# TongtongSong/OpenEAT

Measured on AMD Instinct MI355X. Metric: audio-frames/sec/GPU (train) + RTF (attention-rescoring decode), 12L Conformer, higher is better.
Workload: dtype f32 (storage, accumulate, softmax, norms, losses, optimizer all fp32; every matrix product is the fp32 product to within one fp32 rounding, computed as six exact bf16 x bf16 MFMA products of three-piece operand splits h+m+l = x, dropped terms < 2^-24 |a||b| - tests hold it to the exact-fp32 mode's t; 1 GPU; configs[1]: 12L Conformer d=256 (12+3+3, h=4, ff=1024, K=15, V=3246), B=32/GPU x 10 s 16 kHz wav (T=998 frames), L=30, CTC+attention joint loss, fbank+fwd+bwd+clip+Adam, dropout 0.1; global_batch=32, parallelism=dp1, hip_graph=True

## Files before the change

include/openeat_hip.h:

```cpp
#ifndef OPENEAT_HIP_H
#define OPENEAT_HIP_H

#include <stddef.h>
#include <stdint.h>

#ifdef __cplusplus
extern "C" {
#endif

const char* oe_last_error(void);
int oe_abi_version(void);

int oe_capture_unjoined_streams(void* origin, void* const* sides, int n_sides, int* unjoined_index);

int oe_stamp(long long* buf, int slot, void* stream);

enum { OE_GATHER_NONE = 0, OE_GATHER_A = 1, OE_GATHER_B = 2 };

typedef struct oe_gemm_args {
    const float* a; long lda; int a_kmajor;
    const float* b; long ldb; int b_kmajor;
    float* c; long ldc;
    int m, n, k;
    int split_k;
    float alpha; const float* alpha_dev;
    const float* bias;
    int act;
    float* preact_out; const float* actgrad_in; long ld_aux;
    float drop_p; unsigned long long seed; const unsigned long long* seed_dev;
    const unsigned char* rowmask;
    const float* residual; long ldr; int res_row_mod; float beta;
    int accumulate; int atomic_out;
    int conv_gather; int conv_t1, conv_f1, conv_t2, conv_f2, conv_c;
    float* a_colsum;
    int precision;
    int conv_k, conv_s;
    int conv_kh;
    int out_scatter; int sc_t1, sc_f1, sc_t2, sc_f2, sc_s;
    const void* a_planes; long a_plane_stride;
    const void* b_planes; long b_plane_stride;
    void* c_planes; long c_plane_stride; long ldcp;
    int conv_korder;
    int actgrad_bf16;
    int planes_k_padded;
} oe_gemm_args;

int oe_gemm_f32(const oe_gemm_args* args, void* stream);

int oe_split_planes(const float* x, long ld, long rows, long cols, void* planes, long ldp, long plane_stride, void* stream);
long oe_gemm_pl_launches(void);
long oe_gemm_hyb_launches(void);
int oe_gemm_pl_config(int min_blocks, int tile, int bk, int waves);
int oe_gemm_pl_hybrid(int on);

typedef struct oe_ln_prologue {
    const float* dy; const float* x; const float* stats; const float* gamma; const float* add;
    float* dx; float* g; float* ws;
    float g_alpha, g_p; unsigned long long g_seed; const unsigned char* g_rowmask; const unsigned char* ln_rowmask;
    const float* beta; const float* gamma2; const float* stats2; float* ws2;
} oe_ln_prologue;

typedef struct oe_lnf_prologue {
    const float* x; const float* gamma; const float* beta; float eps;
    float* y; float* stats; const unsigned char* rowmask;
    const float* gamma2; const float* beta2; float eps2; float* u; float* stats2;
} oe_lnf_prologue;

typedef struct oe_ln_epilogue {
    const float* x; const float* stats; const float* gamma; const float* beta; int act;
    float* dx; float* ws;
} oe_ln_epilogue;

typedef struct oe_ffn_args {
    const float* x; long ldx;
    const void* w1p; const float* b1;
    const void* w2p; const float* b2;
    int rows, d, ff, act, precision;
    float drop_in; unsigned long long seed_in;
    float drop_out; unsigned long long seed_out;
    const unsigned long long* seed_dev;
    float* pre_out; float* act_out;
    const float* residual; long ldr; float beta;
    float* y; long ldy;
    oe_ln_prologue ln;
    oe_lnf_prologue lnf;
} oe_ffn_args;
size_t oe_ffn_packed_bytes(int d, int ff, int precision);
int oe_ffn_supported(int d, int ff, int precision, int act);
int oe_ffn_pack_weights(const float* w1, const float* w2, int d, int ff, int precision, void* w1p, void* w2p, void* stream);
int oe_ffn_fwd(const oe_ffn_args* args, void* stream);
int oe_ffn_pack_weights_bwd(const float* w1, const float* w2, int d, int ff, int precision, void* w2t_packed, void* w1t_packed, void* stream);
int oe_ffn_bwd(const oe_ffn_args* a, void* stream);
int oe_ffn_pack_weights_table(const void* table, int n, int max_d, int max_ff, int precision, void* stream);
int oe_ffn6_config(int mode);

typedef struct oe_rowgemm_args {
    const float* x; long ldx;
    const void* wp; const float* bias;
    int rows, k, n;
    float drop_p; unsigned long long seed; const unsigned long long* seed_dev;
    const unsigned char* rowmask;
    const float* residual; long ldr; float beta;
    float* y; long ldy;
    int act; float* preact_out; const float* actgrad_in; long ld_aux;
    oe_ln_prologue ln;
    oe_lnf_prologue lnf;
    oe_ln_epilogue lne;
} oe_rowgemm_args;
int oe_rowgemm6_supported(int k, int n);
int oe_rowgemm6_form(int rows, int k, int n);
int oe_rowgemm6(const oe_rowgemm_args* args, void* stream);
int oe_rowgemm6_pack_table(const void* table, int n, long max_pieces, void* stream);

typedef struct oe_tn_problem {
    const float* a; const float* b; float* c; float* a_colsum; const float* alpha_dev;
    long lda, ldb, ldc;
    int m, n, k;
    float alpha;
    int k_chunk, gx, gy, nz, block_start, reserved;
} oe_tn_problem;
int oe_gemm_tn_grouped_plan(oe_tn_problem* problems_host, int n, int target_blocks);
int oe_gemm_tn_grouped(const oe_tn_problem* problems_dev, int n, int total_blocks, int precision, void* stream);

int oe_colsum_f32(const float* x, long ldx, int m, int n, float alpha, const float* alpha_dev,
                  float* out, int accumulate, void* stream);

int oe_layernorm_fwd_pl(const float* x, const float* gamma, const float* beta, float eps, int rows, int d,
                        const unsigned char* rowmask, int act, float* y, float* stats, void* y_planes, long plane_stride, void* stream);
int oe_layernorm_fwd(const float* x, const float* gamma, const float* beta, float eps, int rows, int d,
                     const unsigned char* rowmask, int act, float* y, float* stats, void* stream);
size_t oe_layernorm_bwd_workspace_floats(int rows, int d);
int oe_layernorm_bwd(const float* dy, const float* x, const float* gamma, const float* beta, int act,
                     const float* stats, int rows, int d, const unsigned char* rowmask, const float* add,
                     float* dx, float* dgamma, float* dbeta, float* workspace, void* stream);
int oe_layernorm_pair_fwd(const float* x, const float* gamma1, const float* beta1, float eps1, const float* gamma2, const float* beta2,
                          float eps2, int rows, int d, float* y1, float* stats1, float* y2, float* stats2, void* stream);
int oe_layernorm_pair_bwd_dx_drop(const float* dy2, const float* x, const float* gamma1, const float* beta1, const float* stats1,
                                  const float* gamma2, const float* stats2, int rows, int d, const float* add, float* dx, float* gout,
                                  float g_alpha, float g_p, unsigned long long g_seed, const unsigned long long* g_seed_dev,
                                  const unsigned char* g_rowmask, float* workspace1, float* workspace2, void* stream);
int oe_layernorm_bwd_dx(const float* dy, const float* x, const float* gamma, const float* beta, int act, const float* stats,
                        int rows, int d, const unsigned char* rowmask, const float* add, float* dx, float* workspace,
                        void* stream);
int oe_layernorm_param_reduce(const float* workspace, int rows, int d, float* dgamma, float* dbeta, void* stream);
int oe_layernorm_param_reduce_table(const long long* table, int n, int max_rows, int max_d, void* stream);
int oe_layernorm_bwd_dx_drop(const float* dy, const float* x, const float* gamma, const float* beta, int act,
                             const float* stats, int rows, int d, const unsigned char* rowmask, const float* add, float* dx,
                             float* gout, float g_alpha, float g_p, unsigned long long g_seed,
                             const unsigned long long* g_seed_dev, const unsigned char* g_rowmask, float* workspace,
                             void* stream);
int oe_layernorm_bwd_dx_drop_pl(const float* dy, const float* x, const float* gamma, const float* beta, int act,
                                const float* stats, int rows, int d, const unsigned char* rowmask, const float* add, float* dx,
                                float* gout, float g_alpha, float g_p, unsigned long long g_seed,
                                const unsigned long long* g_seed_dev, const unsigned char* g_rowmask, float* workspace,
                                void* out_planes, long plane_stride, void* stream);

size_t oe_ctc_workspace_floats(int B, int T, int Lmax);
int oe_ctc_config(int pipe_mode, int chunks);
int oe_ctc_loss_fused_stats(const float* logits, long ldv, int B, int T, int V, const int* hlens, const int* targets,
                            int Lmax, const int* tlens, float grad_scale, const float* utt_weight, float* nll, float* loss_sum,
                            float* dlogits, float* workspace, const float* row_stats, int stats_groups, void* stream);
int oe_ctc_loss_fused(const float* logits, long ldv, int B, int T, int V, const int* hlens, const int* targets,
                      int Lmax, const int* tlens, float grad_scale, const float* utt_weight, float* nll, float* loss_sum,
                      float* dlogits, float* workspace, void* stream);

int oe_ctc_greedy(const float* logits, long ldv, int B, int T, int V, const int* hlens, int eos,
                  int* frame_best, int* out_tokens, int* out_lens, void* stream);

size_t oe_ctc_align_workspace_bytes(int B, int T, int Lmax);
int oe_ctc_align(const float* logits, long ldv, int B, int T, int V, const int* hlens, const int* targets, int Lmax,
                 const int* tlens, int* frames, int* tok_start, int* tok_end, float* tok_logp, float* score, void* workspace,
                 void* stream);

typedef struct oe_attn_args {
    const float* q; long q_bstride, q_rstride;
    const float* k; long k_bstride, k_rstride;
    const float* v; long v_bstride, v_rstride;
    float* out; long o_bstride, o_rstride;
    float* lse;
    const unsigned char* mask; long mask_bstride, mask_rstride;
    const float* keybias;
    int B, H, T1, T2, D;
    float scale;
    float drop_p; unsigned long long seed; const unsigned long long* seed_dev;
    const float* d_out;
    float* dq; float* dk; float* dv;
    float* dkeybias;
    float* delta;
    int precision;
    int causal;
} oe_attn_args;

int oe_attention_fwd(const oe_attn_args* args, void* stream);
int oe_attention_bwd(const oe_attn_args* args, void* stream);

int oe_relpos_prepare(const float* k, long k_bstride, long k_rstride, const float* p, long p_rstride,
                      const float* u, const float* v, int B, int T, int H, int D, float scale, float* kp,
                      float* keybias, void* stream);
int oe_relpos_backward(const float* dkp, const float* dkeybias, const float* k, long k_bstride, long k_rstride,
                       const float* p, long p_rstride, const float* u, const float* v, int B, int T, int H, int D,
                       float scale, float* dk, float* dp, long dp_rstride, float* du, float* dv, void* stream);

int oe_glu_fwd(const float* a, long rows, int d, float* y, void* stream);
int oe_glu_bwd(const float* a, const float* dy, long rows, int d, float* da, void* stream);

// ... 101 lines not shown
```

openeat_amd/csrc/ffn.hip:

```cpp
#include <stdlib.h>
#include "gemm_common.h"
#include "../../include/openeat_hip.h"

typedef __bf16 bf16x8 __attribute__((ext_vector_type(8)));

#define FFN_THREADS 256
#define FFN_ROWS 32

__device__ __forceinline__ int ffn_acc_row(int r, int lk) { return (r & 3) + 8 * (r >> 2) + 4 * lk; }

template <bool TRANSPOSED>
__device__ __forceinline__ void ffn_pack_piece(const float* __restrict__ w1, const float* __restrict__ w2, int d, int ff, int planes,
                                               __bf16* __restrict__ w1p, __bf16* __restrict__ w2p, long piece, int lane) {
    const int KS = d / 16, DT = d / 32, FT = ff / 32;
    const long n1 = (long)FT * KS, n2 = (long)FT * DT * 2;
    float x[8];
    __bf16* dst;
    if (piece < n1) {
        const int ft = (int)(piece / KS), ks = (int)(piece % KS);
        const int row = 32 * ft + (lane & 31), col = 16 * ks + 8 * (lane >> 5);
        if (!TRANSPOSED) {
            const float* src = w1 + (long)row * d + col;
            const float4 a = *reinterpret_cast<const float4*>(src), b = *reinterpret_cast<const float4*>(src + 4);
            x[0] = a.x; x[1] = a.y; x[2] = a.z; x[3] = a.w; x[4] = b.x; x[5] = b.y; x[6] = b.z; x[7] = b.w;
// ... 254 lines not shown
        const int pc = (c4 + 4 * row) & (D - 1);
        float4 v = *reinterpret_cast<const float4*>(&part[row * PART_PITCH + pc]);
#pragma unroll
        for (int w = 1; w < 4; ++w) {
            const float4 u = *reinterpret_cast<const float4*>(&part[w * (FFN_ROWS * PART_PITCH) + row * PART_PITCH + pc]);
            v.x += u.x; v.y += u.y; v.z += u.z; v.w += u.w;
        }
        if (p.b2) { v.x += p.b2[c4]; v.y += p.b2[c4 + 1]; v.z += p.b2[c4 + 2]; v.w += p.b2[c4 + 3]; }
        if (p.p_out > 0.f) {
            const uint2 h = drop_hash4(seed_out, ((unsigned long long)gr * D + c4) >> 2);
            v.x *= drop_field(h.x, 0, dp_out); v.y *= drop_field(h.x, 1, dp_out);
            v.z *= drop_field(h.y, 0, dp_out); v.w *= drop_field(h.y, 1, dp_out);
        }
        float4 res = make_float4(0.f, 0.f, 0.f, 0.f);
        if (p.residual) res = *reinterpret_cast<const float4*>(p.residual + gr * p.ldr + c4);
        v = make_float4(res.x + p.beta * v.x, res.y + p.beta * v.y, res.z + p.beta * v.z, res.w + p.beta * v.w);
        *reinterpret_cast<float4*>(p.y + gr * p.ldy + c4) = v;
    }
}

int oe_ffn6_supported(int d, int ff);
int oe_ffn6_run(const oe_ffn_args* a, bool bwd, void* stream);
static int ffn_planes(int precision) { return precision == 6 ? 3 : precision == 3 ? 2 : 1; }

extern "C" size_t oe_ffn_packed_bytes(int d, int ff, int precision) {
    return (size_t)d * ff * 2 * ffn_planes(precision);
}

extern "C" int oe_ffn_supported(int d, int ff, int precision, int act) {
    if (!(act == OE_ACT_NONE || act == OE_ACT_RELU || act == OE_ACT_SWISH)) return 0;
    if (precision == 6) return oe_ffn6_supported(d, ff);
    return (d == 128 || d == 256) && ff > 0 && ff % 128 == 0 && ff <= 8192 && (precision == 1 || precision == 3);
}

static int ffn_pack(const float* w1, const float* w2, int d, int ff, int precision, void* w1p, void* w2p, bool transposed, void* stream) {
    OE_REQUIRE(w1 && w2 && w1p && w2p, "oe_ffn_pack_weights: null pointer");
    OE_REQUIRE(oe_ffn_supported(d, ff, precision, 0), "oe_ffn_pack_weights: unsupported shape d=%d ff=%d precision=%d", d, ff, precision);
    OE_REQUIRE(((((uintptr_t)w1) | ((uintptr_t)w2) | ((uintptr_t)w1p) | ((uintptr_t)w2p)) & 15) == 0, "oe_ffn_pack_weights: 16-byte alignment required");
    const long pieces = (long)(ff / 32) * (d / 16) + (long)(ff / 32) * (d / 32) * 2;
    if (transposed)
        hipLaunchKernelGGL(ffn_pack_kernel<true>, dim3(oe_cdiv(pieces, 4)), dim3(256), 0, (hipStream_t)stream, w1, w2, d, ff,
                           ffn_planes(precision), (__bf16*)w1p, (__bf16*)w2p);
    else
        hipLaunchKernelGGL(ffn_pack_kernel<false>, dim3(oe_cdiv(pieces, 4)), dim3(256), 0, (hipStream_t)stream, w1, w2, d, ff,
                           ffn_planes(precision), (__bf16*)w1p, (__bf16*)w2p);
    OE_LAUNCH_CHECK("oe_ffn_pack_weights");
    return 0;
}
extern "C" int oe_ffn_pack_weights_table(const void* table, int n, int max_d, int max_ff, int precision, void* stream) {
    OE_REQUIRE(table && n > 0, "oe_ffn_pack_weights_table: empty table");
    OE_REQUIRE(max_d >= 32 && max_d % 32 == 0 && max_ff >= 32 && max_ff % 32 == 0 && (precision == 1 || precision == 3 || precision == 6),
               "oe_ffn_pack_weights_table: bad launch geometry d=%d ff=%d precision=%d", max_d, max_ff, precision);
    const long pieces = (long)(max_ff / 32) * (max_d / 16) + (long)(max_ff / 32) * (max_d / 32) * 2;
    hipLaunchKernelGGL(ffn_pack_table_kernel, dim3(oe_cdiv(pieces, 4), n, 2), dim3(256), 0, (hipStream_t)stream, (const long long*)table);
    OE_LAUNCH_CHECK("oe_ffn_pack_weights_table");
    return 0;
}
extern "C" int oe_ffn_pack_weights(const float* w1, const float* w2, int d, int ff, int precision, void* w1p, void* w2p, void* stream) {
    return ffn_pack(w1, w2, d, ff, precision, w1p, w2p, false, stream);
}
extern "C" int oe_ffn_pack_weights_bwd(const float* w1, const float* w2, int d, int ff, int precision, void* w2tp, void* w1tp, void* stream) {
    return ffn_pack(w1, w2, d, ff, precision, w2tp, w1tp, true, stream);
}

template <int D, int TERMS>
static int ffn_launch(const FfnParams& p, int nout, hipStream_t st) {
    const dim3 grid(oe_cdiv(p.rows, FFN_ROWS)), block(FFN_THREADS);
    const size_t dyn = (size_t)p.ff * sizeof(float);
    if (nout == 2) hipLaunchKernelGGL((ffn_fwd_kernel<D, TERMS, 2>), grid, block, dyn, st, p);
    else if (nout == 1) hipLaunchKernelGGL((ffn_fwd_kernel<D, TERMS, 1>), grid, block, dyn, st, p);
    else hipLaunchKernelGGL((ffn_fwd_kernel<D, TERMS, 0>), grid, block, dyn, st, p);
    OE_LAUNCH_CHECK("oe_ffn_fwd");
    return 0;
}

extern "C" int oe_ffn_fwd(const oe_ffn_args* a, void* stream) {
    OE_REQUIRE(a && a->x && a->w1p && a->w2p && a->y, "oe_ffn_fwd: null pointer");
    OE_REQUIRE(oe_ffn_supported(a->d, a->ff, a->precision, a->act), "oe_ffn_fwd: unsupported d=%d ff=%d precision=%d act=%d", a->d, a->ff,
               a->precision, a->act);
    OE_REQUIRE(a->rows > 0 && a->ldx % 4 == 0 && a->ldy % 4 == 0 && (!a->residual || a->ldr % 4 == 0), "oe_ffn_fwd: bad rows / strides");
    OE_REQUIRE(((((uintptr_t)a->x) | ((uintptr_t)a->y) | ((uintptr_t)a->residual) | ((uintptr_t)a->pre_out) | ((uintptr_t)a->act_out) |
                 ((uintptr_t)a->w1p) | ((uintptr_t)a->w2p)) & 15) == 0, "oe_ffn_fwd: 16-byte alignment required");
    OE_REQUIRE(a->drop_in >= 0.f && a->drop_in < 1.f && a->drop_out >= 0.f && a->drop_out < 1.f, "oe_ffn_fwd: dropout rate out of range");
    OE_REQUIRE(!(a->act_out && !a->pre_out), "oe_ffn_fwd: act_out needs pre_out (the store count is a compile-time constant)");
    if (a->precision == 6) return oe_ffn6_run(a, false, stream);
    FfnParams p{};
    p.x = a->x; p.ldx = a->ldx; p.w1p = (const __bf16*)a->w1p; p.b1 = a->b1; p.w2p = (const __bf16*)a->w2p; p.b2 = a->b2;
    p.pre = a->pre_out; p.act_out = a->act_out; p.residual = a->residual; p.ldr = a->ldr; p.beta = a->beta; p.y = a->y; p.ldy = a->ldy;
    p.rows = a->rows; p.ff = a->ff; p.act = a->act; p.p_in = a->drop_in; p.seed_in = a->seed_in; p.p_out = a->drop_out; p.seed_out = a->seed_out;
    p.seed_dev = a->seed_dev;
    const int nout = a->act_out ? 2 : a->pre_out ? 1 : 0;
    hipStream_t st = (hipStream_t)stream;
    if (a->d == 256) return a->precision == 3 ? ffn_launch<256, 3>(p, nout, st) : ffn_launch<256, 1>(p, nout, st);
    return a->precision == 3 ? ffn_launch<128, 3>(p, nout, st) : ffn_launch<128, 1>(p, nout, st);
}

extern "C" int oe_ffn_bwd(const oe_ffn_args* a, void* stream) {
    OE_REQUIRE(a && (a->x || a->ln.dy) && a->w1p && a->w2p && a->y && a->pre_out && a->act_out, "oe_ffn_bwd: null pointer");
    OE_REQUIRE(!a->ln.dy || a->precision == 6, "oe_ffn_bwd: the LayerNorm-backward prologue exists in precision 6 only");
    OE_REQUIRE(oe_ffn_supported(a->d, a->ff, a->precision, a->act), "oe_ffn_bwd: unsupported d=%d ff=%d precision=%d act=%d", a->d, a->ff,
               a->precision, a->act);
    OE_REQUIRE(!a->b1 && !a->b2 && !a->residual && a->drop_out == 0.f && a->beta == 1.f, "oe_ffn_bwd: bias / residual / output dropout do not apply");
    OE_REQUIRE(a->rows > 0 && a->ldx % 4 == 0 && a->ldy % 4 == 0, "oe_ffn_bwd: bad rows / strides");
    OE_REQUIRE(((((uintptr_t)a->x) | ((uintptr_t)a->y) | ((uintptr_t)a->pre_out) | ((uintptr_t)a->act_out) | ((uintptr_t)a->w1p) |
                 ((uintptr_t)a->w2p)) & 15) == 0, "oe_ffn_bwd: 16-byte alignment required");
    OE_REQUIRE(a->drop_in >= 0.f && a->drop_in < 1.f, "oe_ffn_bwd: dropout rate out of range");
    if (a->precision == 6) return oe_ffn6_run(a, true, stream);
    FfnParams p{};
    p.x = a->x; p.ldx = a->ldx; p.w1p = (const __bf16*)a->w1p; p.w2p = (const __bf16*)a->w2p;
    p.pre = a->pre_out; p.act_out = a->act_out; p.beta = 1.f; p.y = a->y; p.ldy = a->ldy;
    p.rows = a->rows; p.ff = a->ff; p.act = a->act; p.p_in = a->drop_in; p.seed_in = a->seed_in; p.seed_dev = a->seed_dev;
    const dim3 grid(oe_cdiv(p.rows, FFN_ROWS)), block(FFN_THREADS);
    const size_t dyn = (size_t)p.ff * sizeof(float);
    hipStream_t st = (hipStream_t)stream;
    if (a->d == 256) {
        if (a->precision == 3) hipLaunchKernelGGL((ffn_fwd_kernel<256, 3, 1, true>), grid, block, dyn, st, p);
        else hipLaunchKernelGGL((ffn_fwd_kernel<256, 1, 1, true>), grid, block, dyn, st, p);
    } else {
        if (a->precision == 3) hipLaunchKernelGGL((ffn_fwd_kernel<128, 3, 1, true>), grid, block, dyn, st, p);
        else hipLaunchKernelGGL((ffn_fwd_kernel<128, 1, 1, true>), grid, block, dyn, st, p);
    }
    OE_LAUNCH_CHECK("oe_ffn_bwd");
    return 0;
}
```

openeat_amd/csrc/ffn6.hip:

```cpp
#include <stdlib.h>
#include "gemm_common.h"
#include "../../include/openeat_hip.h"

#ifndef OE_F6_NSET
#define OE_F6_NSET 4
#endif
#ifndef OE_F6_FR
#define OE_F6_FR 1
#endif

typedef __bf16 bf16x8 __attribute__((ext_vector_type(8)));
typedef __bf16 bf16x4 __attribute__((ext_vector_type(4)));

struct LnPro {
    const float* dy; const float* x; const float* stats; const float* gamma; const float* add;
    float* dx; float* g; float* ws;
    float g_alpha, g_p; unsigned long long g_seed; const unsigned char* g_rowmask; const unsigned char* ln_rowmask;
    const float* beta; const float* gamma2; const float* stats2; float* ws2;
};
static LnPro ln_pro_of(const oe_ln_prologue& a) {
    LnPro q;
    q.dy = a.dy; q.x = a.x; q.stats = a.stats; q.gamma = a.gamma; q.add = a.add; q.dx = a.dx; q.g = a.g; q.ws = a.ws;
    q.g_alpha = a.g_alpha; q.g_p = a.g_p; q.g_seed = a.g_seed; q.g_rowmask = a.g_rowmask; q.ln_rowmask = a.ln_rowmask;
    q.beta = a.beta; q.gamma2 = a.gamma2; q.stats2 = a.stats2; q.ws2 = a.ws2;
    return q;
}
static const char* ln_pro_check(const oe_ln_prologue& a) {
    if (!(a.x && a.stats && a.gamma && a.dx && a.g && a.ws)) return "null pointer";
    if (((((uintptr_t)a.dy) | ((uintptr_t)a.x) | ((uintptr_t)a.gamma) | ((uintptr_t)a.add) | ((uintptr_t)a.dx) | ((uintptr_t)a.g)) & 15) != 0) return "16-byte alignment required";
    if (!(a.g_p >= 0.f && a.g_p < 1.f)) return "dropout rate out of range";
    if (a.gamma2 && !(a.beta && a.stats2 && a.ws2 && !a.ln_rowmask)) return "pair: beta / stats2 / ws2 missing (and no row mask)";
    if (((((uintptr_t)a.beta) | ((uintptr_t)a.gamma2)) & 15) != 0) return "16-byte alignment required";
    return nullptr;
}

struct LnfPro {
    const float* x; const float* gamma; const float* beta; float eps; float* y; float* stats; const unsigned char* rowmask;
    const float* gamma2; const float* beta2; float eps2; float* u; float* stats2;
};
static LnfPro lnf_pro_of(const oe_lnf_prologue& a) {
    LnfPro q;
    q.x = a.x; q.gamma = a.gamma; q.beta = a.beta; q.eps = a.eps; q.y = a.y; q.stats = a.stats; q.rowmask = a.rowmask;
    q.gamma2 = a.gamma2; q.beta2 = a.beta2; q.eps2 = a.eps2; q.u = a.u; q.stats2 = a.stats2;
    return q;
}
static const char* lnf_pro_check(const oe_lnf_prologue& a) {
    if (!(a.gamma && a.beta && a.y && a.stats)) return "null pointer";
    if (((((uintptr_t)a.x) | ((uintptr_t)a.gamma) | ((uintptr_t)a.beta) | ((uintptr_t)a.y)) & 15) != 0) return "16-byte alignment required";
    if (a.gamma2 && !(a.beta2 && a.stats2 && !a.rowmask)) return "pair: beta2 / stats2 missing (and no row mask)";
    if (((((uintptr_t)a.gamma2) | ((uintptr_t)a.beta2) | ((uintptr_t)a.u)) & 15) != 0) return "16-byte alignment required";
    return nullptr;
}

struct Ffn6Params {
    const float* x; long ldx;
    const unsigned char* w1p; const float* b1;
    const unsigned char* w2p; const float* b2;
    float* pre; float* act_out;
    const float* residual; long ldr; float beta;
    float* y; long ldy;
    int rows, ff, act;
    float p_in; unsigned long long seed_in;
    float p_out; unsigned long long seed_out;
    const unsigned long long* seed_dev;
    LnPro ln;
    LnfPro lnf;
};

__device__ __forceinline__ float f6_act_bwd(int act, float x) {
    const float s = sigmoidf_(x);
    const float sw = s * (1.f + x * (1.f - s));
    return act == OE_ACT_SWISH ? sw : (act == OE_ACT_RELU ? (x > 0.f ? 1.f : 0.f) : 1.f);
}
struct F6 { bf16x8 p[3]; };

#ifdef OE_GEMM_STAMPS
static __device__ unsigned long long* f6_stamp_buf = nullptr;
extern "C" int oe_ffn6_set_stamps(void* buf) {
    return (int)hipMemcpyToSymbol(HIP_SYMBOL(f6_stamp_buf), &buf, sizeof(buf));
}
#define F6_STAMP(slot)                                                                                                   \
    do {                                                                                                                 \
        __builtin_amdgcn_sched_barrier(0);                                                                               \
        unsigned long long t_;                                                                                           \
        asm volatile("s_memtime %0\n\ts_waitcnt lgkmcnt(0)" : "=s"(t_) :: "memory");                                    \
        __builtin_amdgcn_sched_barrier(0);                                                                               \
        if (f6_stamp_buf && (blockIdx.x == 0 || blockIdx.x == gridDim.x - 1) && (threadIdx.x & 63) == 0 && (slot) < 128)     \
            f6_stamp_buf[(blockIdx.x == 0 ? 0 : 1024) + (threadIdx.x >> 6) * 128 + (slot)] = t_;                        \
    } while (0)
#else
#define F6_STAMP(slot) do { } while (0)
#endif
__device__ __forceinline__ int f6_acc_row(int r, int lk) { return (r & 3) + 8 * (r >> 2) + 4 * lk; }
__device__ __forceinline__ void f6_lds_barrier() { asm volatile("s_waitcnt lgkmcnt(0)\n\ts_barrier" ::: "memory"); }
__device__ __forceinline__ void f6_wave_sync() {
    asm volatile("s_waitcnt lgkmcnt(0)" ::: "memory");
    __builtin_amdgcn_wave_barrier();
}

template <bool BWD, int NOUT>
__device__ __forceinline__ void f6_epilogue1(const Ffn6Params& p, const f32x16& hacc, float4 q0, float4 q1, float4 q2, float4 q3, long mrow, int ft,
                                             int lane, float* patch, unsigned long long seed_in, const DropParams& dp_in, float (&hv)[16]) {
    const int lq = lane & 31, lk = lane >> 5;
    auto store_tile = [&](float* out) {
        f6_wave_sync();
#pragma unroll
        for (int r = 0; r < 16; ++r) patch[lq * 36 + f6_acc_row(r, lk)] = hv[r];
        f6_wave_sync();
#pragma unroll
        for (int ps = 0; ps < 4; ++ps) {
            const int row = ps * 8 + (lane >> 3), c4 = (lane & 7) * 4;
            if (mrow + row < p.rows)
                *reinterpret_cast<float4*>(out + (mrow + row) * p.ff + ft * 32 + c4) = *reinterpret_cast<const float4*>(&patch[row * 36 + c4]);
        }
    };
    if (!BWD) {
        hv[0] = hacc[0] + q0.x; hv[1] = hacc[1] + q0.y; hv[2] = hacc[2] + q0.z; hv[3] = hacc[3] + q0.w;
        hv[4] = hacc[4] + q1.x; hv[5] = hacc[5] + q1.y; hv[6] = hacc[6] + q1.z; hv[7] = hacc[7] + q1.w;
        hv[8] = hacc[8] + q2.x; hv[9] = hacc[9] + q2.y; hv[10] = hacc[10] + q2.z; hv[11] = hacc[11] + q2.w;
        hv[12] = hacc[12] + q3.x; hv[13] = hacc[13] + q3.y; hv[14] = hacc[14] + q3.z; hv[15] = hacc[15] + q3.w;
        if (NOUT >= 1 && p.pre) store_tile(p.pre);
        if (p.act == OE_ACT_SWISH) {
#pragma unroll
            for (int r = 0; r < 16; ++r) hv[r] *= sigmoidf_(hv[r]);
        } else if (p.act == OE_ACT_RELU) {
#pragma unroll
            for (int r = 0; r < 16; ++r) hv[r] = fmaxf(hv[r], 0.f);
        }
    } else {
        f6_wave_sync();
        float* pr = &patch[(lane >> 3) * 36 + (lane & 7) * 4];
        *reinterpret_cast<float4*>(pr) = q0;
        *reinterpret_cast<float4*>(pr + 8 * 36) = q1;
        *reinterpret_cast<float4*>(pr + 16 * 36) = q2;
        *reinterpret_cast<float4*>(pr + 24 * 36) = q3;
        f6_wave_sync();
#pragma unroll
        for (int r = 0; r < 16; ++r) hv[r] = hacc[r] * f6_act_bwd(p.act, patch[lq * 36 + f6_acc_row(r, lk)]);
    }
    if (p.p_in > 0.f) {
        const unsigned long long e0 = (unsigned long long)(mrow + lq) * p.ff + ft * 32 + 4 * lk;
#pragma unroll
        for (int g4 = 0; g4 < 4; ++g4) {
            const uint2 h = drop_hash4(seed_in, (e0 + 8 * g4) >> 2);
            hv[4 * g4] *= drop_field(h.x, 0, dp_in); hv[4 * g4 + 1] *= drop_field(h.x, 1, dp_in);
            hv[4 * g4 + 2] *= drop_field(h.y, 0, dp_in); hv[4 * g4 + 3] *= drop_field(h.y, 1, dp_in);
        }
    }
    if ((BWD || NOUT == 2) && p.act_out) store_tile(p.act_out);
}
__device__ __forceinline__ void f6_write_planes(const float (&hv)[16], unsigned char* hdst, int s_stride, int lane) {
#pragma unroll
    for (int s = 0; s < 2; ++s) {
        float v[8];
#pragma unroll
        for (int e = 0; e < 8; ++e) v[e] = hv[8 * s + e];
        oe_bf16x8 pl[3];
        oe_split8<3>(v, pl);
#pragma unroll
        for (int pn = 0; pn < 3; ++pn) *reinterpret_cast<oe_bf16x8*>(hdst + s * s_stride + pn * 1024 + lane * 16) = pl[pn];
    }
}

template <int D, bool PAIR>
__device__ __forceinline__ void ln_fwd_rows_to_planes(const LnfPro& q, int rows, long m0, int wv, int lane, unsigned char* xs) {
    static_assert(D == 256, "one float4 per lane and row");
    constexpr int BM = 32, XP = D + 8;
    const float4 g = reinterpret_cast<const float4*>(q.gamma)[lane], bb = reinterpret_cast<const float4*>(q.beta)[lane];
    float4 g2 = g, bb2 = bb;
    if (PAIR) { g2 = reinterpret_cast<const float4*>(q.gamma2)[lane]; bb2 = reinterpret_cast<const float4*>(q.beta2)[lane]; }
    float4 v[4];
#pragma unroll
    for (int k = 0; k < 4; ++k) v[k] = reinterpret_cast<const float4*>(q.x + min(m0 + wv + 8 * k, (long)rows - 1) * D)[lane];
#pragma unroll
    for (int k = 0; k < 4; ++k) {
        const int row = wv + 8 * k;
        const long grow = m0 + row;
        const bool valid = grow < rows;
        const float mean = wave_sum(v[k].x + v[k].y + v[k].z + v[k].w) / D;
        const float a = v[k].x - mean, b = v[k].y - mean, c = v[k].z - mean, e = v[k].w - mean;
        const float rstd = rsqrtf(wave_sum(a * a + b * b + c * c + e * e) / D + q.eps);
        float4 o = make_float4(0.f, 0.f, 0.f, 0.f);
        if (!(valid && q.rowmask && !q.rowmask[grow]))
            o = make_float4((v[k].x - mean) * rstd * g.x + bb.x, (v[k].y - mean) * rstd * g.y + bb.y,
                            (v[k].z - mean) * rstd * g.z + bb.z, (v[k].w - mean) * rstd * g.w + bb.w);
        if (valid && lane == 0) { q.stats[grow * 2] = mean; q.stats[grow * 2 + 1] = rstd; }
        if (PAIR) {
            if (valid && q.u) reinterpret_cast<float4*>(q.u + grow * D)[lane] = o;
            const float mean2 = wave_sum(o.x + o.y + o.z + o.w) / D;
            const float a2 = o.x - mean2, b2 = o.y - mean2, c2 = o.z - mean2, e2 = o.w - mean2;
            const float rstd2 = rsqrtf(wave_sum(a2 * a2 + b2 * b2 + c2 * c2 + e2 * e2) / D + q.eps2);
            if (valid && lane == 0) { q.stats2[grow * 2] = mean2; q.stats2[grow * 2 + 1] = rstd2; }
            o = make_float4((o.x - mean2) * rstd2 * g2.x + bb2.x, (o.y - mean2) * rstd2 * g2.y + bb2.y,
                            (o.z - mean2) * rstd2 * g2.z + bb2.z, (o.w - mean2) * rstd2 * g2.w + bb2.w);
        }
        if (valid) reinterpret_cast<float4*>(q.y + grow * D)[lane] = o;
        const float xq[4] = {o.x, o.y, o.z, o.w};
        oe_bf16x4v pl[3];
        oe_split4<3>(xq, pl);
#pragma unroll
        for (int n = 0; n < 3; ++n) *reinterpret_cast<oe_bf16x4v*>(xs + ((size_t)(n * BM + row) * XP + 4 * lane) * 2) = pl[n];
    }
}

template <int D, bool PAIR>
__device__ __forceinline__ void ln_bwd_rows_to_planes(const LnPro& q, const unsigned long long* seed_dev, int rows, long m0, int wv, int lane,
                                                      unsigned char* xs, float* red) {
    static_assert(D == 256, "one float4 per lane and row");
    constexpr int BM = 32, XP = D + 8;
    constexpr int NV = D / 256;
    const float4* g4 = reinterpret_cast<const float4*>(q.gamma);
    float4 gam[NV], dg[2][NV], db[2][NV];
    float4 bet[PAIR ? NV : 1], gam2[PAIR ? NV : 1], dg2[2][PAIR ? NV : 1], db2[2][PAIR ? NV : 1];
#pragma unroll
    for (int j = 0; j < NV; ++j) {
        gam[j] = g4[lane + 64 * j];
        dg[0][j] = dg[1][j] = db[0][j] = db[1][j] = make_float4(0.f, 0.f, 0.f, 0.f);
        if (PAIR) {
            bet[j] = reinterpret_cast<const float4*>(q.beta)[lane + 64 * j];
            gam2[j] = reinterpret_cast<const float4*>(q.gamma2)[lane + 64 * j];
            dg2[0][j] = dg2[1][j] = db2[0][j] = db2[1][j] = make_float4(0.f, 0.f, 0.f, 0.f);
        }
    }
    const DropParams g_dpar = drop_params(q.g_p);
    const unsigned long long g_seed_eff = q.g_seed + (seed_dev ? *seed_dev * 0x9E3779B97F4A7C15ull : 0ull);
    float4 dyv[4][NV], xv[4][NV], av[4][NV];
    float mean[4], rstd[4];
#pragma unroll
    for (int k = 0; k < 4; ++k) {
        const long rc = min(m0 + wv + 8 * k, (long)rows - 1);
        mean[k] = q.stats[rc * 2];
        rstd[k] = q.stats[rc * 2 + 1];
// ... 60 lines not shown
            dgs.x += t.x * xh[j].x; dgs.y += t.y * xh[j].y; dgs.z += t.z * xh[j].z; dgs.w += t.w * xh[j].w;
            dbs.x += t.x; dbs.y += t.y; dbs.z += t.z; dbs.w += t.w;
        }
        const float c1 = wave_sum(s1) / D, c2 = wave_sum(s2) / D;
#pragma unroll
        for (int j = 0; j < NV; ++j) {
            const int i = lane + 64 * j;
            float4 o = av[k][j];
            if (live) {
                o.x += rstd[k] * (g[j].x - c1 - xh[j].x * c2);
                o.y += rstd[k] * (g[j].y - c1 - xh[j].y * c2);
                o.z += rstd[k] * (g[j].z - c1 - xh[j].z * c2);
                o.w += rstd[k] * (g[j].w - c1 - xh[j].w * c2);
            }
            float4 gq = make_float4(o.x * q.g_alpha, o.y * q.g_alpha, o.z * q.g_alpha, o.w * q.g_alpha);
            const unsigned long long e0 = (unsigned long long)grow * D + 4 * i;
            if (q.g_p > 0.f) {
                const uint4 r = drop_words8(g_seed_eff, e0 >> 3);
                const bool hi = (e0 >> 2) & 1;
                const unsigned wa = hi ? r.z : r.x, wb = hi ? r.w : r.y;
                gq.x *= drop_field(wa, 0, g_dpar); gq.y *= drop_field(wa, 1, g_dpar);
                gq.z *= drop_field(wb, 0, g_dpar); gq.w *= drop_field(wb, 1, g_dpar);
            }
            if (valid && q.g_rowmask && !q.g_rowmask[grow]) gq = make_float4(0.f, 0.f, 0.f, 0.f);
            if (valid) {
                reinterpret_cast<float4*>(q.dx + grow * D)[i] = o;
                reinterpret_cast<float4*>(q.g + grow * D)[i] = gq;
            }
            const float xq[4] = {gq.x, gq.y, gq.z, gq.w};
            oe_bf16x4v pl[3];
            oe_split4<3>(xq, pl);
#pragma unroll
            for (int n = 0; n < 3; ++n) *reinterpret_cast<oe_bf16x4v*>(xs + ((size_t)(n * BM + row) * XP + 4 * i) * 2) = pl[n];
        }
    }
#pragma unroll
    for (int sl = 0; sl < 2; ++sl)
#pragma unroll
        for (int j = 0; j < NV; ++j) {
            reinterpret_cast<float4*>(red + ((wv * 2 + sl) * 2 + 0) * D)[lane + 64 * j] = dg[sl][j];
            reinterpret_cast<float4*>(red + ((wv * 2 + sl) * 2 + 1) * D)[lane + 64 * j] = db[sl][j];
        }
    __syncthreads();
    for (int c = threadIdx.x; c < 4 * D; c += 512) {
        float sum = 0.f;
#pragma unroll
        for (int w = 0; w < 8; ++w) sum += red[w * 4 * D + c];
        const long slot = 2 * (long)blockIdx.x + c / (2 * D);
        if (slot * 16 < rows) q.ws[slot * 2 * D + (c % (2 * D))] = sum;
    }
    if (PAIR) {
        __syncthreads();
#pragma unroll
        for (int sl = 0; sl < 2; ++sl)
#pragma unroll
            for (int j = 0; j < NV; ++j) {
                reinterpret_cast<float4*>(red + ((wv * 2 + sl) * 2 + 0) * D)[lane + 64 * j] = dg2[sl][j];
                reinterpret_cast<float4*>(red + ((wv * 2 + sl) * 2 + 1) * D)[lane + 64 * j] = db2[sl][j];
            }
        __syncthreads();
        for (int c = threadIdx.x; c < 4 * D; c += 512) {
            float sum = 0.f;
#pragma unroll
            for (int w = 0; w < 8; ++w) sum += red[w * 4 * D + c];
            const long slot = 2 * (long)blockIdx.x + c / (2 * D);
            if (slot * 16 < rows) q.ws2[slot * 2 * D + (c % (2 * D))] = sum;
        }
    }
}

template <int D, int RT, bool BWD, int NOUT, int NG, int LNP = 0>
__global__ __launch_bounds__(256 * NG, (NG == 2 || (RT == 1 && D <= 256)) ? 2 : 1) void ffn6_kernel(Ffn6Params p) {
    static_assert(NG == 1 || (NG == 2 && RT == 1), "two wave groups: 32-row blocks");
    static_assert(LNP == 0 || (D == 256 && RT == 1 && NG == 2 && BWD == (LNP == 1)), "LayerNorm prologues: the eight-wave 32-row kernels at d = 256");
    constexpr int BM = 32 * RT;
    constexpr int KS = D / 16, DT = D / 32, DPW = DT / 4;
    constexpr int FR = OE_F6_FR, NSET = OE_F6_NSET;
    constexpr int NS1 = KS / FR, NS2 = DPW * 8 / FR, NSTG = NS1 + NS2;
    static_assert(DT % 4 == 0 && KS % FR == 0 && NSTG % NSET == 0, "stage split");
    constexpr int XP = D + 8;
    constexpr int X_BYTES = 3 * BM * XP * 2;
    constexpr int H_WAVE = 2 * RT * 3 * 1024;
    constexpr int H_BYTES = 4 * H_WAVE;
    static_assert(H_WAVE >= 32 * 36 * 4, "the wave's h region doubles as its 32 x 36 fp32 patch");
    constexpr int PIECE = 3 * 1024;
    constexpr int NT = RT * DPW;
    static_assert(NG == 1 || (NT % 2 == 0 && 8 * (NT / 2) * 4096 <= X_BYTES), "the groups' exchange buffer reuses the x planes");
    __shared__ __attribute__((aligned(1024))) unsigned char lds[X_BYTES + NG * H_BYTES];
    unsigned char* xs = lds;

    const int lane = threadIdx.x & 63;
    const int wv = __builtin_amdgcn_readfirstlane(threadIdx.x >> 6);
    const int grp = NG == 2 ? (wv >> 2) : 0;
    const int wave = wv & 3;
    unsigned char* hs = lds + X_BYTES + grp * H_BYTES;
    const int lq = lane & 31, lk = lane >> 5;
    const long m0 = (long)blockIdx.x * BM;
    const int nchunks = p.ff / 128;
    const int rot = blockIdx.x % nchunks;

    if constexpr (LNP == 2) {
        if (p.lnf.gamma2) ln_fwd_rows_to_planes<D, true>(p.lnf, p.rows, m0, wv, lane, xs);
        else ln_fwd_rows_to_planes<D, false>(p.lnf, p.rows, m0, wv, lane, xs);
    } else if constexpr (LNP == 1) {
        static_assert(LNP != 1 || 8 * 2 * 2 * D * 4 <= NG * H_BYTES, "the prologue's partial sums reuse the h regions");
        if (p.ln.gamma2) ln_bwd_rows_to_planes<D, true>(p.ln, p.seed_dev, p.rows, m0, wv, lane, xs, reinterpret_cast<float*>(lds + X_BYTES));
        else ln_bwd_rows_to_planes<D, false>(p.ln, p.seed_dev, p.rows, m0, wv, lane, xs, reinterpret_cast<float*>(lds + X_BYTES));
    } else {
        constexpr int C4 = D / 4;
        for (int i = threadIdx.x; i < BM * C4; i += 256 * NG) {
            const int row = i / C4, c4 = (i - row * C4) * 4;
            const long gr = min(m0 + row, (long)p.rows - 1);
            const float4 v = *reinterpret_cast<const float4*>(p.x + gr * p.ldx + c4);
            const float xv[4] = {v.x, v.y, v.z, v.w};
            oe_bf16x4v pl[3];
            oe_split4<3>(xv, pl);
#pragma unroll
            for (int n = 0; n < 3; ++n) *reinterpret_cast<oe_bf16x4v*>(xs + ((size_t)(n * BM + row) * XP + c4) * 2) = pl[n];
        }
    }

    const unsigned char* w1l = p.w1p + lane * 16 + (long)wave * KS * PIECE;
    const unsigned char* w2l = p.w2p + lane * 16 + (long)wave * DPW * 2 * PIECE;
    constexpr long W1_CHUNK = 4L * KS * PIECE, W2_CHUNK = 4L * DT * 2 * PIECE;
    auto load_stage = [&](auto w_c, int c, F6 (&f)[FR]) {
        constexpr int w = decltype(w_c)::value;
        const unsigned char* b1p = w1l + c * W1_CHUNK;
        const unsigned char* b2p = w2l + c * W2_CHUNK;
#pragma unroll
        for (int j = 0; j < FR; ++j) {
            const unsigned char* src;
            if constexpr (w < NS1) {
                src = b1p + (long)(w * FR + j) * PIECE;
            } else {
                const int fidx = (w - NS1) * FR + j;
                const int dtl = fidx >> 3, ftl = (fidx >> 1) & 3, s = fidx & 1;
                src = b2p + (long)(((ftl * DT + dtl) * 2) + s) * PIECE;
            }
            f[j].p[0] = *reinterpret_cast<const bf16x8*>(src); f[j].p[1] = *reinterpret_cast<const bf16x8*>(src + 1024);
            f[j].p[2] = *reinterpret_cast<const bf16x8*>(src + 2048);
        }
    };
    auto chunk_at = [&](int ci) {
        int c = min(ci, nchunks - 1) + rot;
        return c >= nchunks ? c - nchunks : c;
    };
    F6 fr[NSET][FR];
    {
        const int c0 = chunk_at(grp);
        static_for<0, NSET - 1>([&](auto k_c) { load_stage(k_c, c0, fr[decltype(k_c)::value]); });
    }

    f32x16 yacc[RT][DPW];
#pragma unroll
    for (int a = 0; a < RT; ++a)
#pragma unroll
        for (int t = 0; t < DPW; ++t)
#pragma unroll
            for (int r = 0; r < 16; ++r) yacc[a][t][r] = 0.f;
    const unsigned long long sd = p.seed_dev ? *p.seed_dev * 0x9E3779B97F4A7C15ull : 0ull;
    const unsigned long long seed_in = p.seed_in + sd, seed_out = p.seed_out + sd;
    const DropParams dp_in = drop_params(p.p_in), dp_out = drop_params(p.p_out);
    unsigned char* hmine = hs + wave * H_WAVE;
    float* patch = reinterpret_cast<float*>(hmine);

    auto x_frag = [&](int rt, int ks, F6& f) {
        const unsigned char* a = xs + ((size_t)(rt * 32 + lq) * XP + 16 * ks + 8 * lk) * 2;
// ... 671 lines not shown
    OE_REQUIRE(!has_act || !(a->preact_out || a->actgrad_in) || (a->ld_aux % 2 == 0 && ((((uintptr_t)a->preact_out) | ((uintptr_t)a->actgrad_in)) & 7) == 0),
               "oe_rowgemm6: pre-activation / act-grad source must be 8-byte aligned with an even row stride");
    OE_REQUIRE(a->rows > 0 && a->ldx % 4 == 0 && a->ldy % 4 == 0 && (!a->residual || a->ldr % 4 == 0), "oe_rowgemm6: bad rows / strides");
    if (a->ln.dy) {
        OE_REQUIRE(form == 1 && a->k == 256, "oe_rowgemm6: the LayerNorm-backward prologue exists in the row-block form at k = 256 only");
        const char* why = ln_pro_check(a->ln);
        OE_REQUIRE(why == nullptr, "oe_rowgemm6: LayerNorm prologue: %s", why);
    }
    if (a->lnf.x) {
        OE_REQUIRE(form == 1 && a->k == 256 && !a->ln.dy && !a->lnf.gamma2, "oe_rowgemm6: the (single) LayerNorm-forward prologue exists in the row-block form at k = 256 only");
        const char* why = lnf_pro_check(a->lnf);
        OE_REQUIRE(why == nullptr, "oe_rowgemm6: LayerNorm-forward prologue: %s", why);
    }
    OE_REQUIRE(((((uintptr_t)a->x) | ((uintptr_t)a->y) | ((uintptr_t)a->residual) | ((uintptr_t)a->wp) | ((uintptr_t)a->bias)) & 15) == 0,
               "oe_rowgemm6: 16-byte alignment required");
    OE_REQUIRE(a->drop_p >= 0.f && a->drop_p < 1.f, "oe_rowgemm6: dropout rate out of range");
    Row6Params p{};
    p.x = a->x; p.ldx = a->ldx; p.wp = (const unsigned char*)a->wp; p.bias = a->bias; p.residual = a->residual; p.ldr = a->ldr; p.beta = a->beta;
    p.rowmask = a->rowmask; p.y = a->y; p.ldy = a->ldy; p.rows = a->rows; p.no = a->n; p.p_out = a->drop_p; p.seed_out = a->seed; p.seed_dev = a->seed_dev;
    p.k = a->k; p.act = a->act; p.preact_out = a->preact_out; p.actgrad_in = a->actgrad_in; p.ld_aux = a->ld_aux;
    p.ln = ln_pro_of(a->ln);
    p.lnf = lnf_pro_of(a->lnf);
    if (a->lne.dx) {
        OE_REQUIRE(form == 1 && a->k == 256 && a->n == 256 && !a->lnf.x, "oe_rowgemm6: the LayerNorm-backward epilogue exists for 256 <- 256 in the row-block form only");
        OE_REQUIRE(a->lne.x && a->lne.stats && a->lne.gamma && a->lne.beta && a->lne.ws, "oe_rowgemm6: LayerNorm epilogue: null pointer");
        OE_REQUIRE(!a->bias && a->drop_p == 0.f && !a->rowmask && !a->residual && a->beta == 1.f, "oe_rowgemm6: LayerNorm epilogue: no other epilogue feature applies");
        OE_REQUIRE(a->lne.act == OE_ACT_NONE || a->lne.act == OE_ACT_RELU || a->lne.act == OE_ACT_SWISH, "oe_rowgemm6: LayerNorm epilogue: activation %d", a->lne.act);
        OE_REQUIRE(((((uintptr_t)a->lne.x) | ((uintptr_t)a->lne.gamma) | ((uintptr_t)a->lne.beta) | ((uintptr_t)a->lne.dx) | ((uintptr_t)a->lne.ws)) & 15) == 0,
                   "oe_rowgemm6: LayerNorm epilogue: 16-byte alignment required");
        p.le_x = a->lne.x; p.le_stats = a->lne.stats; p.le_gamma = a->lne.gamma; p.le_beta = a->lne.beta; p.le_act = a->lne.act;
        p.le_dx = a->lne.dx; p.le_ws = a->lne.ws;
    }
    if (form == 2) {
        const dim3 tgrid(oe_cdiv(a->rows, 32), a->n / 32), tblock(512);
        hipStream_t st = (hipStream_t)stream;
        switch (a->k / 128) {
            case 2: hipLaunchKernelGGL((rowtile6_kernel<2>), tgrid, tblock, 0, st, p); break;
            case 4: hipLaunchKernelGGL((rowtile6_kernel<4>), tgrid, tblock, 0, st, p); break;
            case 6: hipLaunchKernelGGL((rowtile6_kernel<6>), tgrid, tblock, 0, st, p); break;
            default: hipLaunchKernelGGL((rowtile6_kernel<8>), tgrid, tblock, 0, st, p); break;
        }
        OE_LAUNCH_CHECK("oe_rowgemm6 (tile form)");
        return 0;
    }
    const dim3 grid(oe_cdiv(a->rows, 32)), block(512);
    if (a->k > 512) hipLaunchKernelGGL(rowgemm6p_kernel, grid, block, 0, (hipStream_t)stream, p);
    else if (a->lne.dx && a->ln.dy) hipLaunchKernelGGL((rowgemm6_kernel<256, 1, true>), grid, block, 0, (hipStream_t)stream, p);
    else if (a->lne.dx) hipLaunchKernelGGL((rowgemm6_kernel<256, 0, true>), grid, block, 0, (hipStream_t)stream, p);
    else if (a->ln.dy) hipLaunchKernelGGL((rowgemm6_kernel<256, 1>), grid, block, 0, (hipStream_t)stream, p);
    else if (a->lnf.x) hipLaunchKernelGGL((rowgemm6_kernel<256, 2>), grid, block, 0, (hipStream_t)stream, p);
    else if (a->k == 512) hipLaunchKernelGGL((rowgemm6_kernel<512>), grid, block, 0, (hipStream_t)stream, p);
    else hipLaunchKernelGGL((rowgemm6_kernel<256>), grid, block, 0, (hipStream_t)stream, p);
    OE_LAUNCH_CHECK("oe_rowgemm6");
    return 0;
}

template <int D, int RT, int NG>
static int ffn6_launch(const Ffn6Params& p, bool bwd, int nout, hipStream_t st) {
    const dim3 grid(oe_cdiv(p.rows, 32 * RT)), block(256 * NG);
    if constexpr (D == 256 && RT == 1 && NG == 2) {
        if (bwd && p.ln.dy) {
            hipLaunchKernelGGL((ffn6_kernel<D, RT, true, 1, NG, 1>), grid, block, 0, st, p);
            OE_LAUNCH_CHECK("oe_ffn_bwd (precision 6, LayerNorm-backward prologue)");
            return 0;
        }
        if (!bwd && p.lnf.x) {
            if (nout == 2) hipLaunchKernelGGL((ffn6_kernel<D, RT, false, 2, NG, 2>), grid, block, 0, st, p);
            else if (nout == 1) hipLaunchKernelGGL((ffn6_kernel<D, RT, false, 1, NG, 2>), grid, block, 0, st, p);
            else hipLaunchKernelGGL((ffn6_kernel<D, RT, false, 0, NG, 2>), grid, block, 0, st, p);
            OE_LAUNCH_CHECK("oe_ffn_fwd (precision 6, LayerNorm prologue)");
            return 0;
        }
    }
    OE_REQUIRE(!p.ln.dy && !p.lnf.x, "oe_ffn: the LayerNorm prologues exist at d = 256 in the two-group block shape only");
    if (bwd) hipLaunchKernelGGL((ffn6_kernel<D, RT, true, 1, NG>), grid, block, 0, st, p);
    else if (nout == 2) hipLaunchKernelGGL((ffn6_kernel<D, RT, false, 2, NG>), grid, block, 0, st, p);
    else if (nout == 1) hipLaunchKernelGGL((ffn6_kernel<D, RT, false, 1, NG>), grid, block, 0, st, p);
    else hipLaunchKernelGGL((ffn6_kernel<D, RT, false, 0, NG>), grid, block, 0, st, p);
    OE_LAUNCH_CHECK(bwd ? "oe_ffn_bwd (precision 6)" : "oe_ffn_fwd (precision 6)");
    return 0;
}

int oe_ffn6_supported(int d, int ff) { return (d == 128 || d == 256 || d == 512) && ff > 0 && ff % 128 == 0 && ff <= 8192; }

static int ffn6_mode_v = getenv("OE_FFN6_MODE") ? atoi(getenv("OE_FFN6_MODE")) : 0;
static int ffn6_mode() { return ffn6_mode_v; }
extern "C" int oe_ffn6_config(int mode) {
    if (mode >= 0) ffn6_mode_v = mode;
    return ffn6_mode_v;
}

int oe_ffn6_run(const oe_ffn_args* a, bool bwd, void* stream) {
    Ffn6Params p{};
    p.x = a->x; p.ldx = a->ldx; p.w1p = (const unsigned char*)a->w1p; p.b1 = a->b1; p.w2p = (const unsigned char*)a->w2p; p.b2 = a->b2;
    p.pre = a->pre_out; p.act_out = a->act_out; p.residual = a->residual; p.ldr = a->ldr; p.beta = a->beta; p.y = a->y; p.ldy = a->ldy;
    p.rows = a->rows; p.ff = a->ff; p.act = a->act; p.p_in = a->drop_in; p.seed_in = a->seed_in; p.p_out = a->drop_out; p.seed_out = a->seed_out;
    p.seed_dev = a->seed_dev;
    if (a->ln.dy) {
        const char* why = ln_pro_check(a->ln);
        OE_REQUIRE(bwd && why == nullptr, "oe_ffn: LayerNorm prologue: %s", bwd ? why : "backward only");
        p.ln = ln_pro_of(a->ln);
    }
    if (a->lnf.x) {
        const char* why = lnf_pro_check(a->lnf);
        OE_REQUIRE(!bwd && why == nullptr, "oe_ffn: LayerNorm-forward prologue: %s", bwd ? "forward only" : why);
        p.lnf = lnf_pro_of(a->lnf);
    }
    const int nout = a->act_out ? 2 : a->pre_out ? 1 : 0;
    hipStream_t st = (hipStream_t)stream;
    const int mode = ffn6_mode();
    const bool two_groups = (a->ff % 256 == 0) && mode != 1 && mode != 2;
    if (a->d == 512) return two_groups ? ffn6_launch<512, 1, 2>(p, bwd, nout, st) : ffn6_launch<512, 1, 1>(p, bwd, nout, st);
    if (a->d == 256) {
        if (two_groups) return ffn6_launch<256, 1, 2>(p, bwd, nout, st);
        return mode == 2 ? ffn6_launch<256, 1, 1>(p, bwd, nout, st) : ffn6_launch<256, 2, 1>(p, bwd, nout, st);
    }
    return ffn6_launch<128, 2, 1>(p, bwd, nout, st);
}
```

openeat_amd/csrc/gemm.hip:

```cpp
#include <stdlib.h>
#include "gemm_common.h"
#include "../../include/openeat_hip.h"


#define BK 16
#define LDS_PAD 4

template <int TM, int TN, bool A_KMAJOR, bool B_KMAJOR, bool GATHER_A, bool GATHER_B>
__global__ __launch_bounds__(256) void gemm_f32_kernel(OperandDesc A, OperandDesc B, float* __restrict__ C, long ldc,
                                                        int M, int N, int K, int k_chunk, int gx, int gy, EpiParams ep) {
    int tile_x, tile_y, tile_z;
    {
        const int nblk = gridDim.x, id = blockIdx.x;
        const int q = nblk >> 3, r = nblk & 7, xcd = id & 7, j = id >> 3;
        const int swz = (xcd < r ? xcd * (q + 1) : r * (q + 1) + (xcd - r) * q) + j;
        tile_x = swz % gx;
        tile_y = (swz / gx) % gy;
        tile_z = swz / (gx * gy);
    }
    constexpr int BM = 64 * TM, BN = 64 * TN;
    constexpr int LDA = BM + LDS_PAD, LDB = BN + LDS_PAD;
    constexpr int LDS_FLOATS = (2 * BK * (LDA + LDB) > 4 * 32 * 36) ? 2 * BK * (LDA + LDB) : 4 * 32 * 36;
    __shared__ __attribute__((aligned(16))) float lds[LDS_FLOATS];
    auto As = [&](int buf) -> float* { return lds + buf * (BK * LDA); };
// ... 60 lines not shown
#pragma unroll
        for (int s = 0; s < A_SLOTS; ++s) {
            int slot = tid + s * 256;
            if (!A_KMAJOR) {
                int row = slot / 4, kq = (slot & 3) * 4;
                float* d = As(buf) + kq * LDA + row;
                d[0] = a_reg[s].x; d[LDA] = a_reg[s].y; d[2 * LDA] = a_reg[s].z; d[3 * LDA] = a_reg[s].w;
            } else {
                int k = slot / (BM / 4), rq = (slot % (BM / 4)) * 4;
                *reinterpret_cast<float4*>(As(buf) + k * LDA + rq) = a_reg[s];
            }
        }
#pragma unroll
        for (int s = 0; s < B_SLOTS; ++s) {
            int slot = tid + s * 256;
            if (!B_KMAJOR) {
                int row = slot / 4, kq = (slot & 3) * 4;
                float* d = Bs(buf) + kq * LDB + row;
                d[0] = b_reg[s].x; d[LDB] = b_reg[s].y; d[2 * LDB] = b_reg[s].z; d[3 * LDB] = b_reg[s].w;
            } else {
                int k = slot / (BN / 4), rq = (slot % (BN / 4)) * 4;
                *reinterpret_cast<float4*>(Bs(buf) + k * LDB + rq) = b_reg[s];
            }
        }
    };

    f32x16 acc[TM][TN];
#pragma unroll
    for (int i = 0; i < TM; ++i)
#pragma unroll
        for (int j = 0; j < TN; ++j)
#pragma unroll
            for (int r = 0; r < 16; ++r) acc[i][j][r] = 0.f;

    if (nk > 0) {
        load_tiles(0);
        store_tiles(0);
    }
    __syncthreads();

    const int lrow = lane & 31, lk = lane >> 5;
    for (int kt = 0; kt < nk; ++kt) {
        const int buf = kt & 1;
        if (kt + 1 < nk) load_tiles(kt + 1);
        const float* as = As(buf) + wm * (32 * TM) + lrow;
        const float* bs = Bs(buf) + wn * (32 * TN) + lrow;
#pragma unroll
        for (int kk = 0; kk < BK / 2; ++kk) {
            float a[TM], b[TN];
#pragma unroll
            for (int i = 0; i < TM; ++i) a[i] = as[(kk * 2 + lk) * LDA + i * 32];
#pragma unroll
            for (int j = 0; j < TN; ++j) b[j] = bs[(kk * 2 + lk) * LDB + j * 32];
#pragma unroll
            for (int i = 0; i < TM; ++i)
#pragma unroll
                for (int j = 0; j < TN; ++j)
                    acc[i][j] = __builtin_amdgcn_mfma_f32_32x32x2f32(a[i], b[j], acc[i][j], 0, 0, 0);
        }
        if (kt + 1 < nk) store_tiles(buf ^ 1);
        __syncthreads();
    }

    gemm_epilogue<TM, TN>(acc, lds, C, ldc, M, N, m0, n0, ep, tile_z);
}

template <int TM, int TN, bool AK, bool BKM, bool GA, bool GB>
static int launch(const OperandDesc& A, const OperandDesc& B, float* C, long ldc, int M, int N, int K, int splitk,
                  const EpiParams& ep, hipStream_t st) {
    constexpr int BM = 64 * TM, BN = 64 * TN;
    int kc = oe_cdiv(oe_cdiv(K, splitk), BK) * BK;
    if (kc <= 0) kc = BK;
    int nz = oe_cdiv(K, kc);
    if (nz < 1) nz = 1;
    const int gx = oe_cdiv(N, BN), gy = oe_cdiv(M, BM);
    hipLaunchKernelGGL((gemm_f32_kernel<TM, TN, AK, BKM, GA, GB>), dim3(gx * gy * nz), dim3(256), 0, st, A, B, C, ldc, M, N, K, kc, gx, gy, ep);
    OE_LAUNCH_CHECK("oe_gemm_f32");
    return 0;
}

static bool vec_ok(const void* p, long ld) { return ((uintptr_t)p % 16 == 0) && (ld % 4 == 0); }

extern "C" int oe_gemm_f32(const oe_gemm_args* g, void* stream) {
    OE_REQUIRE(g && g->c && (g->a || (g->a_planes && g->b_planes && g->precision == 6)) && (g->b || (g->a_planes && g->b_planes && g->precision == 6)),
               "oe_gemm_f32: null operand");
    OE_REQUIRE(g->m > 0 && g->n > 0 && g->k >= 0, "oe_gemm_f32: bad shape m=%d n=%d k=%d", g->m, g->n, g->k);
    OE_REQUIRE(g->split_k >= 1, "oe_gemm_f32: split_k must be >= 1");
    OE_REQUIRE(!(g->split_k > 1 && !g->atomic_out), "oe_gemm_f32: split_k > 1 needs atomic_out");
    OE_REQUIRE(!(g->atomic_out && (g->act || g->residual || g->preact_out || g->actgrad_in || g->drop_p > 0.f || g->beta != 1.f)),
               "oe_gemm_f32: atomic_out supports only alpha/bias epilogues");
    OE_REQUIRE(g->drop_p >= 0.f && g->drop_p < 1.f, "oe_gemm_f32: drop_p out of range");
    OE_REQUIRE(g->act == OE_ACT_NONE || g->act == OE_ACT_RELU || g->act == OE_ACT_SWISH,
               "oe_gemm_f32: only relu (1) and swish (2) are fused into the epilogue; apply act %d with oe_act_fwd / oe_act_grad", g->act);
    hipStream_t st = (hipStream_t)stream;
    OperandDesc A{}, B{};
    A.p = g->a; A.ld = g->lda; A.vec_ok = vec_ok(g->a, g->lda);
    B.p = g->b; B.ld = g->ldb; B.vec_ok = vec_ok(g->b, g->ldb);
    const bool ga = g->conv_gather == OE_GATHER_A, gb = g->conv_gather == OE_GATHER_B;
    if (ga || gb) {
        OperandDesc& X = ga ? A : B;
        X.T1 = g->conv_t1; X.F1 = g->conv_f1; X.T2 = g->conv_t2; X.F2 = g->conv_f2; X.C = g->conv_c;
        X.KS = g->conv_k > 0 ? g->conv_k : 3;
        X.S = g->conv_s > 0 ? g->conv_s : 2;
        OE_REQUIRE(X.C > 0 && X.C % 4 == 0, "oe_gemm_f32: conv gather needs C %% 4 == 0");
        const int KH = g->conv_kh > 0 ? g->conv_kh : X.KS;
        OE_REQUIRE(X.T1 >= KH && X.F1 >= X.KS && X.T2 >= 1 && X.F2 >= 1 && X.T2 <= (X.T1 - KH) / X.S + 1 && X.F2 <= (X.F1 - X.KS) / X.S + 1,
                   "oe_gemm_f32: conv gather dims inconsistent");
        OE_REQUIRE(g->conv_kh <= 0 || ga, "oe_gemm_f32: conv_kh is for a gather on A");
        OE_REQUIRE(gb ? (X.T2 == (X.T1 - KH) / X.S + 1 && X.F2 == (X.F1 - X.KS) / X.S + 1) : true, "oe_gemm_f32: conv gather dims inconsistent");
        X.vec_ok = ((uintptr_t)X.p % 16 == 0);
        OE_REQUIRE(ga ? (!g->a_kmajor && g->k == KH * X.KS * X.C) : (g->b_kmajor && g->n == X.KS * X.KS * X.C),
                   "oe_gemm_f32: conv gather layout mismatch");
    }
    EpiParams ep{};
    ep.alpha = g->alpha; ep.alpha_dev = g->alpha_dev; ep.bias = g->bias; ep.act = g->act;
    ep.preact_out = g->preact_out; ep.actgrad_in = g->actgrad_in; ep.ld_aux = g->ld_aux ? g->ld_aux : g->ldc;
    ep.actgrad_bf16 = g->actgrad_bf16;
    OE_REQUIRE(!g->actgrad_bf16 || (g->actgrad_in && g->act == OE_ACT_RELU && !g->preact_out),
               "oe_gemm_f32: actgrad_bf16 is for the ReLU mask (only the sign of the source is read), without preact_out");
    ep.drop_p = g->drop_p; ep.seed = g->seed; ep.seed_dev = g->seed_dev; ep.rowmask = g->rowmask;
    ep.residual = g->residual; ep.ldr = g->ldr ? g->ldr : g->ldc; ep.beta = g->beta; ep.res_row_mod = g->res_row_mod;
    ep.accumulate = g->accumulate; ep.atomic = g->atomic_out; ep.a_colsum = g->a_colsum;
    ep.scatter = g->out_scatter; ep.sc_t1 = g->sc_t1; ep.sc_f1 = g->sc_f1; ep.sc_t2 = g->sc_t2; ep.sc_f2 = g->sc_f2; ep.sc_s = g->sc_s;
    ep.c_planes = (__bf16*)g->c_planes; ep.c_pstride = g->c_plane_stride; ep.ld_cp = g->ldcp ? g->ldcp : g->ldc;
    OE_REQUIRE(!g->c_planes || (!g->atomic_out && !g->accumulate && !g->out_scatter && ep.ld_cp % 4 == 0 && g->c_plane_stride % 4 == 0 &&
                                (((uintptr_t)g->c_planes) & 7) == 0),
               "oe_gemm_f32: c_planes needs a plain (non-atomic, non-scattered) output, 8-byte aligned planes and strides of whole 4-element groups");
    if (g->out_scatter) {
        OE_REQUIRE(!g->atomic_out && !g->accumulate && !g->preact_out && !g->residual && !g->rowmask && g->drop_p <= 0.f,
                   "oe_gemm_f32: out_scatter supports alpha / bias / activation / act-grad epilogues only");
        OE_REQUIRE(g->sc_t2 >= 1 && g->sc_f2 >= 1 && g->sc_s >= 1 && (long)(g->sc_t2 - 1) * g->sc_s < g->sc_t1 && (long)(g->sc_f2 - 1) * g->sc_s < g->sc_f1 &&
                   g->m % ((long)g->sc_t2 * g->sc_f2) == 0, "oe_gemm_f32: out_scatter dims inconsistent");
    }
    OE_REQUIRE(!g->a_colsum || (g->precision != 0 && g->a_kmajor && g->conv_gather != OE_GATHER_A), "oe_gemm_f32: a_colsum needs the bf16 path and a k-major A");
    const int M = g->m, N = g->n, K = g->k, sk = g->split_k;
    OE_REQUIRE(g->precision == 0 || g->precision == 1 || g->precision == 3 || g->precision == 6,
               "oe_gemm_f32: precision must be 0 (fp32), 1 (bf16), 3 (bf16x3) or 6 (bf16x6)");
    OE_REQUIRE(g->conv_korder == 0 || (g->conv_korder == 1 && ga && g->precision == 6 && g->a_planes && g->b_planes && sk <= 1 && A.C % 32 == 0),
               "oe_gemm_f32: conv_korder 1 needs a gather on A, precision 6, pre-split operands, no split of the reduction and C %% 32 == 0");
    if (g->precision == 6 && g->a_planes && g->b_planes) {
        const int r = oe_gemm_pl_try(A, B, g->a_planes, g->a_plane_stride, g->b_planes, g->b_plane_stride, g->c, g->ldc, M, N, K, sk, ep,
                                     g->a_kmajor, g->b_kmajor, ga, gb, st, g->conv_korder, g->planes_k_padded != 0);
        if (r != 1) return r;
        OE_REQUIRE(g->conv_korder == 0, "oe_gemm_f32: conv_korder 1, but the pre-split kernel does not take this problem (M=%d N=%d K=%d) - "
                                        "B is laid out for it alone", M, N, K);
    }
    if (g->precision == 6 && g->b_planes && !g->a_planes && g->a && !ga && !gb && !g->a_kmajor) {
        const int r = oe_gemm_hyb_try(A, B, g->b_planes, g->b_plane_stride, g->c, g->ldc, M, N, K, sk, ep, g->b_kmajor, st);
        if (r != 1) return r;
    }
    OE_REQUIRE(g->a && g->b, "oe_gemm_f32: an operand exists as bf16 planes only, but the pre-split kernel does not take this problem "
                             "(M=%d N=%d K=%d, a_kmajor=%d b_kmajor=%d gather=%d)", M, N, K, g->a_kmajor, g->b_kmajor, g->conv_gather);
    if (g->precision) return oe_gemm_bf16_dispatch(A, B, g->c, g->ldc, M, N, K, sk, ep, g->a_kmajor, g->b_kmajor, ga, gb, g->precision, st);
    const long b22 = (long)oe_cdiv(M, 128) * oe_cdiv(N, 128) * sk, b12 = (long)oe_cdiv(M, 64) * oe_cdiv(N, 128) * sk;
    const int tile = (b22 >= 200 && M >= 128 && N >= 128) ? 22 : (b12 >= 160 && N >= 128) ? 12 : 11;
#define OE_DISPATCH(AK, BKM, GA, GB)                                                                       \
    do {                                                                                                   \
        if (tile == 22) return launch<2, 2, AK, BKM, GA, GB>(A, B, g->c, g->ldc, M, N, K, sk, ep, st);     \
        if (tile == 12) return launch<1, 2, AK, BKM, GA, GB>(A, B, g->c, g->ldc, M, N, K, sk, ep, st);     \
        return launch<1, 1, AK, BKM, GA, GB>(A, B, g->c, g->ldc, M, N, K, sk, ep, st);                     \
    } while (0)
    if (!g->a_kmajor && !g->b_kmajor) { if (ga) { OE_DISPATCH(false, false, true, false); } else { OE_DISPATCH(false, false, false, false); } }
    if (!g->a_kmajor && g->b_kmajor) { OE_DISPATCH(false, true, false, false); }
    if (g->a_kmajor && g->b_kmajor) { if (gb) { OE_DISPATCH(true, true, false, true); } else { OE_DISPATCH(true, true, false, false); } }
    OE_REQUIRE(false, "oe_gemm_f32: layout a_kmajor=1,b_kmajor=0 is not supported");
#undef OE_DISPATCH
}
```

openeat_amd/csrc/gemm_common.h:

```cpp
#pragma once
#include "oe_common.h"

#include <type_traits>

typedef float f32x16 __attribute__((ext_vector_type(16)));

template <int I, int N, class F>
__device__ __forceinline__ void static_for(F&& f) {
    if constexpr (I < N) {
        f(std::integral_constant<int, I>{});
        static_for<I + 1, N>(f);
    }
}


#ifdef OE_GEMM_STAMPS
static __device__ unsigned long long* oe_stamp_buf = nullptr;
#define OE_STAMP(slot)                                                                                     \
    do {                                                                                                   \
        __builtin_amdgcn_sched_barrier(0);                                                                 \
        unsigned long long t_;                                                                             \
        asm volatile("s_memtime %0\n\ts_waitcnt lgkmcnt(0)" : "=s"(t_) :: "memory");                       \
        __builtin_amdgcn_sched_barrier(0);                                                                 \
        if (oe_stamp_buf && threadIdx.x == 0 && blockIdx.x < 4096) oe_stamp_buf[blockIdx.x * 8 + (slot)] = t_; \
// ... 18 lines not shown
    long b = q / d.T2;
    return ((b * d.T1 + d.S * t) * (long)d.F1 + d.S * f) * d.C;
}
template <bool GATHER>
__device__ __forceinline__ long addr_col(const OperandDesc& d, long c) {
    if (!GATHER) return c;
    int seg = d.KS * d.C;
    int kh = (int)(c / seg);
    return (long)kh * d.F1 * d.C + (c - (long)kh * seg);
}

__device__ __forceinline__ float4 load4(const float* p, int n_valid, bool vec_ok) {
    float4 v = make_float4(0.f, 0.f, 0.f, 0.f);
    if (n_valid >= 4 && vec_ok) {
        v = *reinterpret_cast<const float4*>(p);
    } else {
        if (n_valid > 0) v.x = p[0];
        if (n_valid > 1) v.y = p[1];
        if (n_valid > 2) v.z = p[2];
        if (n_valid > 3) v.w = p[3];
    }
    return v;
}

struct EpiParams {
    float alpha;
    const float* alpha_dev;
    const float* bias;
    int act;
    float* preact_out;
    const float* actgrad_in;
    long ld_aux;
    float drop_p;
    unsigned long long seed;
    const unsigned long long* seed_dev;
    const unsigned char* rowmask;
    const float* residual;
    long ldr;
    int res_row_mod;
    float beta;
    int accumulate;
    int atomic;
    float* a_colsum;
    int scatter, sc_t1, sc_f1, sc_t2, sc_f2, sc_s;
    int actgrad_bf16;
    __bf16* c_planes;
    long c_pstride;
    long ld_cp;
};

__device__ __forceinline__ long scatter_row(const EpiParams& ep, long r) {
    const int f = (int)(r % ep.sc_f2);
    const long q = r / ep.sc_f2;
    const int t = (int)(q % ep.sc_t2);
    const long b = q / ep.sc_t2;
    return (b * ep.sc_t1 + (long)ep.sc_s * t) * ep.sc_f1 + (long)ep.sc_s * f;
}
__device__ __forceinline__ void pass_rows(const EpiParams& ep, long row0, long (&ro)[4]) {
    if (!ep.scatter) {
#pragma unroll
        for (int p = 0; p < 4; ++p) ro[p] = row0 + 8 * p;
        return;
    }
    int f = (int)(row0 % ep.sc_f2);
    long q = row0 / ep.sc_f2;
    int t = (int)(q % ep.sc_t2);
    long b = q / ep.sc_t2;
#pragma unroll
    for (int p = 0; p < 4; ++p) {
        ro[p] = (b * ep.sc_t1 + (long)ep.sc_s * t) * ep.sc_f1 + (long)ep.sc_s * f;
        f += 8;
        while (f >= ep.sc_f2) {
            f -= ep.sc_f2;
            if (++t == ep.sc_t2) { t = 0; ++b; }
        }
    }
}


int oe_gemm_bf16_dispatch(const OperandDesc& A, const OperandDesc& B, float* C, long ldc, int M, int N, int K, int sk,
                          const EpiParams& ep, bool a_kmajor, bool b_kmajor, bool ga, bool gb, int terms, hipStream_t st);

int oe_gemm_tn_planes_try(const OperandDesc& A, const OperandDesc& B, float* C, long ldc, int M, int N, int K, int sk, const EpiParams& ep,
                          int terms, hipStream_t st);
int oe_gemm_dma_try(const OperandDesc& A, const OperandDesc& B, float* C, long ldc, int M, int N, int K, int sk, const EpiParams& ep,
                    bool a_kmajor, bool b_kmajor, bool gather_b, int terms, int tile, hipStream_t st);
int oe_gemm_hyb_try(const OperandDesc& A, const OperandDesc& B, const void* Bp, long b_pstride, float* C, long ldc, int M, int N, int K, int sk,
                    const EpiParams& ep, bool b_kmajor, hipStream_t st);
int oe_gemm_pl_try(const OperandDesc& A, const OperandDesc& B, const void* Ap, long a_pstride, const void* Bp, long b_pstride, float* C, long ldc,
                   int M, int N, int K, int sk, const EpiParams& ep, bool a_kmajor, bool b_kmajor, bool ga, bool gb, hipStream_t st, int korder = 0,
                   bool k_padded = false);

__device__ __forceinline__ float epi_value(const EpiParams& ep, float v, float alpha, float bias, float aux, float dm, bool row_dead,
                                           float res, float& pre) {
    float x = v * alpha + bias;
    pre = x;
    if (ep.actgrad_in) x *= (ep.act == OE_ACT_RELU) ? (aux > 0.f ? 1.f : 0.f) : (ep.act == OE_ACT_SWISH) ? act_bwd(OE_ACT_SWISH, aux) : 1.f;
    else x = (ep.act == OE_ACT_RELU) ? fmaxf(x, 0.f) : (ep.act == OE_ACT_SWISH) ? x * sigmoidf_(x) : x;
    x *= dm;
    if (row_dead) x = 0.f;
    return res + ep.beta * x;
}

__device__ __forceinline__ float4 load_aux4(const EpiParams& ep, long off) {
    if (!ep.actgrad_bf16) return *reinterpret_cast<const float4*>(ep.actgrad_in + off);
    const oe_bf16x4 h = *reinterpret_cast<const oe_bf16x4*>(reinterpret_cast<const __bf16*>(ep.actgrad_in) + off);
    return make_float4((float)h[0], (float)h[1], (float)h[2], (float)h[3]);
}
__device__ __forceinline__ float load_aux1(const EpiParams& ep, long off) {
    return ep.actgrad_bf16 ? (float)reinterpret_cast<const __bf16*>(ep.actgrad_in)[off] : ep.actgrad_in[off];
}
template <int TM, int TN, int WM = 2>
__device__ __forceinline__ void gemm_epilogue(f32x16 (&acc)[TM][TN], float* lds, float* __restrict__ C, long ldc, int M, int N,
                                              long m0, long n0, const EpiParams& ep, int tile_z) {
    const int lane = threadIdx.x & 63, wave = threadIdx.x >> 6;
    const int wm = wave >> 1, wn = wave & 1;
    const int lrow = lane & 31, lk = lane >> 5;
    float alpha = ep.alpha;
    if (ep.alpha_dev) alpha *= *ep.alpha_dev;
    const DropParams dpar = drop_params(ep.drop_p);
    const unsigned long long seed = ep.seed + (ep.seed_dev ? *ep.seed_dev * 0x9E3779B97F4A7C15ull : 0ull);
    const bool first_split = (tile_z == 0);
    const bool interior = (m0 + 32 * TM * WM <= M) && (n0 + 64 * TN <= N);
    constexpr int EP_LD = 36;
    if (ep.atomic) {
#pragma unroll
        for (int i = 0; i < TM; ++i)
#pragma unroll
            for (int j = 0; j < TN; ++j) {
                const long col = n0 + wn * (32 * TN) + j * 32 + lrow;
                float bias = (col < N && ep.bias && first_split) ? ep.bias[col] : 0.f;
                asm volatile("" : "+v"(bias));
                float* base = C + (m0 + wm * (32 * TM) + i * 32 + 4 * lk) * ldc + col;
                if (interior) {
#pragma unroll
                    for (int r = 0; r < 16; ++r) atomicAdd(base + ((r & 3) + 8 * (r >> 2)) * ldc, acc[i][j][r] * alpha + bias);
                } else {
#pragma unroll
                    for (int r = 0; r < 16; ++r) {
                        const long row = m0 + wm * (32 * TM) + i * 32 + (r & 3) + 8 * (r >> 2) + 4 * lk;
                        if (row < M && col < N) atomicAdd(C + row * ldc + col, acc[i][j][r] * alpha + bias);
                    }
                }
            }
        return;
    }
    if (interior && !ep.scatter && !ep.accumulate && !ep.actgrad_in && !ep.residual && !ep.rowmask && ep.drop_p <= 0.f && ep.beta == 1.f && !ep.c_planes) {
        static_for<0, TM * TN>([&](auto tile_idx) {
            constexpr int i = decltype(tile_idx)::value / TN, j = decltype(tile_idx)::value % TN;
            const long col = n0 + wn * (32 * TN) + j * 32 + lrow;
            const float bias = (ep.bias && first_split) ? ep.bias[col] : 0.f;
            const long rbase = m0 + wm * (32 * TM) + i * 32 + 4 * lk;
            float* cbase = C + rbase * ldc + col;
            float v[16];
#pragma unroll
            for (int r = 0; r < 16; ++r) v[r] = acc[i][j][r] * alpha + bias;
            if (ep.preact_out) {
                float* pbase = ep.preact_out + rbase * ep.ld_aux + col;
#pragma unroll
                for (int r = 0; r < 16; ++r) pbase[((r & 3) + 8 * (r >> 2)) * ep.ld_aux] = v[r];
            }
            if (ep.act == OE_ACT_SWISH) {
#pragma unroll
                for (int r = 0; r < 16; ++r) v[r] *= sigmoidf_(v[r]);
            } else if (ep.act == OE_ACT_RELU) {
#pragma unroll
                for (int r = 0; r < 16; ++r) v[r] = fmaxf(v[r], 0.f);
// ... 219 lines not shown
```

openeat_amd/csrc/gemm_tn.hip:

```cpp
#include <stdlib.h>
#include "gemm_common.h"
#include "../../include/openeat_hip.h"

typedef __bf16 bf16x8 __attribute__((ext_vector_type(8)));
typedef __bf16 bf16x4 __attribute__((ext_vector_type(4)));
typedef short s16x4 __attribute__((ext_vector_type(4)));

#define TN_KROWS 32
#define TN_COLS 128
#define TN_PITCH (TN_COLS + 16)
#define TN_PLANE (TN_KROWS * TN_PITCH)
#define TN_THREADS 512

#ifdef OE_GEMM_STAMPS
static __device__ unsigned long long* tn_stamp_buf = nullptr;
extern "C" int oe_debug_set_tn_stamp_buffer(void* p) { return (int)hipMemcpyToSymbol(HIP_SYMBOL(tn_stamp_buf), &p, sizeof(p)); }
#define TN_NOW(var)                                                                          \
    do {                                                                                     \
        __builtin_amdgcn_sched_barrier(0);                                                   \
        asm volatile("s_memtime %0\n\ts_waitcnt lgkmcnt(0)" : "=s"(var) :: "memory");        \
        __builtin_amdgcn_sched_barrier(0);                                                   \
    } while (0)
#define TN_ACC(slot) do { unsigned long long t1_; TN_NOW(t1_); tn_acc[slot] += t1_ - tn_t; tn_t = t1_; } while (0)
#else
#define TN_NOW(var) do { } while (0)
#define TN_ACC(slot) do { } while (0)
#endif

template <int TERMS> struct TFrag { bf16x8 p[oe_npl<TERMS>::N]; };

template <int TERMS>
__device__ __forceinline__ void tn_frag(const __bf16* img, int col32, int s, int lane, TFrag<TERMS>& f) {
    const int i = lane & 15, grp = lane >> 4;
    const __bf16* p = img + (16 * s + 4 * (grp >> 1) + (i >> 2)) * TN_PITCH + col32 + 16 * (grp & 1) + 4 * (i & 3);
    typedef __attribute__((address_space(3))) s16x4 lds_s16x4;
#pragma unroll
    for (int n = 0; n < oe_npl<TERMS>::N; ++n) {
        union { s16x4 h[2]; bf16x8 v; } u;
        u.h[0] = __builtin_amdgcn_ds_read_tr16_b64_v4i16((lds_s16x4*)(p + n * TN_PLANE));
        u.h[1] = __builtin_amdgcn_ds_read_tr16_b64_v4i16((lds_s16x4*)(p + n * TN_PLANE + 8 * TN_PITCH));
        f.p[n] = u.v;
    }
}

template <int TERMS>
__device__ __forceinline__ f32x16 tn_mma(const TFrag<TERMS>& a, const TFrag<TERMS>& b, f32x16 c) {
    return oe_mma_terms<TERMS>(a, b, c);
}

struct TnRegs { float4 v[2]; };
__device__ __forceinline__ void tn_load(TnRegs& t, const float* base, long ld, int k0, int k_last) {
#pragma unroll
    for (int i = 0; i < 2; ++i) {
        const int k = min(k0 + (int)(threadIdx.x >> 5) + 16 * i, k_last);
        t.v[i] = *reinterpret_cast<const float4*>(base + (long)k * ld);
    }
}
template <int TERMS>
__device__ __forceinline__ void tn_store(const TnRegs& t, __bf16* img, int k0, int k_end) {
#pragma unroll
    for (int i = 0; i < 2; ++i) {
        const int row = (int)(threadIdx.x >> 5) + 16 * i;
        const bool live = k0 + row < k_end;
        const float x[4] = {live ? t.v[i].x : 0.f, live ? t.v[i].y : 0.f, live ? t.v[i].z : 0.f, live ? t.v[i].w : 0.f};
        constexpr int NPL = oe_npl<TERMS>::N;
        bf16x4 pl[NPL];
#pragma unroll
        for (int e = 0; e < 4; ++e) {
            __bf16 q[NPL];
            oe_split_bf16<NPL>(x[e], q);
#pragma unroll
            for (int n = 0; n < NPL; ++n) pl[n][e] = q[n];
        }
        __bf16* d = img + row * TN_PITCH + 4 * (threadIdx.x & 31);
#pragma unroll
        for (int n = 0; n < NPL; ++n) *reinterpret_cast<bf16x4*>(d + n * TN_PLANE) = pl[n];
    }
}

template <int TERMS>
__device__ __forceinline__ void tn_block(const float* __restrict__ Ap, long lda, const float* __restrict__ Bp, long ldb,
                                         float* __restrict__ C, long ldc, int M, int N, int Mr, int Nr, int K, int k_chunk,
                                         int tile_x, int tile_y, int tile_z, const EpiParams& ep) {
    constexpr int NPL = oe_npl<TERMS>::N;
    constexpr int OP_ELEMS = NPL * TN_PLANE;
    constexpr int BUF_ELEMS = 2 * OP_ELEMS;
    constexpr int XCH_BYTES = 4 * 2 * 32 * 64 * 4;
    constexpr int IMG_ELEMS = (2 * BUF_ELEMS * 2 >= XCH_BYTES) ? 2 * BUF_ELEMS : XCH_BYTES / 2;
    __shared__ __attribute__((aligned(16))) __bf16 img[IMG_ELEMS];
    __shared__ float csum_s[TN_COLS];

    const int lane = threadIdx.x & 63;
    const int wave = __builtin_amdgcn_readfirstlane(threadIdx.x >> 6);
    const int grp = wave >> 2, wm = (wave >> 1) & 1, wn = wave & 1;
    const long m0 = (long)tile_y * TN_COLS, n0 = (long)tile_x * TN_COLS;
    const int k_begin = tile_z * k_chunk;
    const int k_end = min(K, k_begin + k_chunk);
    const int nchunks = (k_end - k_begin + TN_KROWS - 1) / TN_KROWS;

    const int c4 = 4 * (threadIdx.x & 31);
    const float* a_src = Ap + min(m0 + c4, (long)Mr - 4);
    const float* b_src = Bp + min(n0 + c4, (long)Nr - 4);
    const bool do_csum = ep.a_colsum != nullptr && tile_x == 0;
    float cs[4] = {0.f, 0.f, 0.f, 0.f};

    f32x16 acc[2][2];
#pragma unroll
    for (int i = 0; i < 2; ++i)
#pragma unroll
        for (int j = 0; j < 2; ++j)
#pragma unroll
            for (int r = 0; r < 16; ++r) acc[i][j][r] = 0.f;

#ifdef OE_GEMM_STAMPS
    unsigned long long tn_acc[8] = {0, 0, 0, 0, 0, 0, 0, 0}, tn_t, tn_t0;
    TN_NOW(tn_t);
    tn_t0 = tn_t;
#endif
    TnRegs ra, rb;
    if (nchunks > 0) {
        tn_load(ra, a_src, lda, k_begin, k_end - 1);
        tn_load(rb, b_src, ldb, k_begin, k_end - 1);
        if (do_csum) {
#pragma unroll
            for (int i = 0; i < 2; ++i)
                if (k_begin + (int)(threadIdx.x >> 5) + 16 * i < k_end) { cs[0] += ra.v[i].x; cs[1] += ra.v[i].y; cs[2] += ra.v[i].z; cs[3] += ra.v[i].w; }
        }
        tn_store<TERMS>(ra, img, k_begin, k_end);
        tn_store<TERMS>(rb, img + OP_ELEMS, k_begin, k_end);
    }
    __syncthreads();
    TN_ACC(0);
    for (int c = 0; c < nchunks; ++c) {
        const int kn = k_begin + (c + 1) * TN_KROWS;
        const bool more = c + 1 < nchunks;
        if (more) {
            tn_load(ra, a_src, lda, kn, k_end - 1);
            tn_load(rb, b_src, ldb, kn, k_end - 1);
        }
        TN_ACC(1);
        const __bf16* ia = img + (c & 1) * BUF_ELEMS;
        const __bf16* ib = ia + OP_ELEMS;
        TFrag<TERMS> fa[2], fb[2];
        tn_frag<TERMS>(ia, wm * 64, grp, lane, fa[0]);
        tn_frag<TERMS>(ia, wm * 64 + 32, grp, lane, fa[1]);
        tn_frag<TERMS>(ib, wn * 64, grp, lane, fb[0]);
        tn_frag<TERMS>(ib, wn * 64 + 32, grp, lane, fb[1]);
#pragma unroll
        for (int i = 0; i < 2; ++i)
#pragma unroll
            for (int j = 0; j < 2; ++j) acc[i][j] = tn_mma<TERMS>(fa[i], fb[j], acc[i][j]);
        TN_ACC(2);
#ifdef OE_GEMM_STAMPS
        asm volatile("s_waitcnt vmcnt(0)" ::: "memory");
        TN_ACC(3);
#endif
        if (more) {
            if (do_csum) {
#pragma unroll
                for (int i = 0; i < 2; ++i)
                    if (kn + (int)(threadIdx.x >> 5) + 16 * i < k_end) { cs[0] += ra.v[i].x; cs[1] += ra.v[i].y; cs[2] += ra.v[i].z; cs[3] += ra.v[i].w; }
            }
            __bf16* nx = img + ((c + 1) & 1) * BUF_ELEMS;
            tn_store<TERMS>(ra, nx, kn, k_end);
            tn_store<TERMS>(rb, nx + OP_ELEMS, kn, k_end);
        }
        TN_ACC(4);
        __syncthreads();
        TN_ACC(5);
    }

    float alpha = ep.alpha;
    if (ep.alpha_dev) alpha *= *ep.alpha_dev;

    if (do_csum) {
        if (threadIdx.x < TN_COLS) csum_s[threadIdx.x] = 0.f;
        __syncthreads();
#pragma unroll
        for (int e = 0; e < 4; ++e) {
            const float v = cs[e] + __shfl_xor(cs[e], 32, 64);
            if (lane < 32) atomicAdd(&csum_s[4 * lane + e], v);
        }
        __syncthreads();
        if (threadIdx.x < TN_COLS && m0 + threadIdx.x < M) atomicAdd(ep.a_colsum + m0 + threadIdx.x, csum_s[threadIdx.x] * alpha);
    }

    float* xch = reinterpret_cast<float*>(img);
    const int q = wave & 3;
    {
        float* mine = xch + ((q * 2 + grp) * 32) * 64 + lane;
#pragma unroll
        for (int j = 0; j < 2; ++j)
#pragma unroll
            for (int r = 0; r < 16; ++r) mine[(j * 16 + r) * 64] = grp == 0 ? acc[1][j][r] : acc[0][j][r];
    }
    __syncthreads();
    f32x16 fin[2];
    {
        const float* theirs = xch + ((q * 2 + (1 - grp)) * 32) * 64 + lane;
#pragma unroll
        for (int j = 0; j < 2; ++j)
#pragma unroll
            for (int r = 0; r < 16; ++r) fin[j][r] = (grp == 0 ? acc[0][j][r] : acc[1][j][r]) + theirs[(j * 16 + r) * 64];
    }
    const int lrow = lane & 31, lk = lane >> 5;
    const bool interior = (m0 + TN_COLS <= M) && (n0 + TN_COLS <= N);
#pragma unroll
    for (int j = 0; j < 2; ++j) {
        const long col = n0 + wn * 64 + j * 32 + lrow;
        const long row0 = m0 + wm * 64 + grp * 32 + 4 * lk;
        float* base = C + row0 * ldc + col;
#pragma unroll
        for (int r = 0; r < 16; ++r) {
            const int dr = (r & 3) + 8 * (r >> 2);
            if (!interior && !(row0 + dr < M && col < N)) continue;
            const float v = fin[j][r] * alpha;
            if (ep.atomic) atomicAdd(base + dr * ldc, v);
            else if (ep.accumulate) base[dr * ldc] += v;
            else base[dr * ldc] = v;
        }
    }
#ifdef OE_GEMM_STAMPS
    TN_ACC(6);
    if (tn_stamp_buf && threadIdx.x == 0 && blockIdx.x < 2048) {
        for (int i = 0; i < 7; ++i) tn_stamp_buf[blockIdx.x * 8 + i] = tn_acc[i];
        tn_stamp_buf[blockIdx.x * 8 + 7] = tn_t - tn_t0;
    }
#endif
}

__device__ __forceinline__ int tn_swizzle(int id, int nblk) {
    const int q = nblk >> 3, r = nblk & 7, xcd = id & 7, j = id >> 3;
    return (xcd < r ? xcd * (q + 1) : r * (q + 1) + (xcd - r) * q) + j;
}

template <int TERMS>
__global__ __launch_bounds__(TN_THREADS) void gemm_tn_planes_kernel(const float* __restrict__ Ap, long lda, const float* __restrict__ Bp, long ldb,
                                                                   float* __restrict__ C, long ldc, int M, int N, int Mr, int Nr, int K, int k_chunk,
                                                                   int gx, int gy, EpiParams ep) {
    const int swz = tn_swizzle(blockIdx.x, gridDim.x);
    tn_block<TERMS>(Ap, lda, Bp, ldb, C, ldc, M, N, Mr, Nr, K, k_chunk, swz % gx, (swz / gx) % gy, swz / (gx * gy), ep);
}

template <int TERMS>
__global__ __launch_bounds__(TN_THREADS) void gemm_tn_grouped_kernel(const oe_tn_problem* __restrict__ tab, int n_problems) {
    const int swz = tn_swizzle(blockIdx.x, gridDim.x);
    int p = 0;
    while (p + 1 < n_problems && tab[p + 1].block_start <= swz) ++p;
    const oe_tn_problem pr = tab[p];
    const int local = swz - pr.block_start;
    EpiParams ep{};
    ep.alpha = pr.alpha; ep.alpha_dev = pr.alpha_dev; ep.beta = 1.f; ep.atomic = 1; ep.a_colsum = pr.a_colsum;
    tn_block<TERMS>(pr.a, pr.lda, pr.b, pr.ldb, pr.c, pr.ldc, pr.m, pr.n, (pr.m + 3) / 4 * 4, (pr.n + 3) / 4 * 4, pr.k, pr.k_chunk,
                    local % pr.gx, (local / pr.gx) % pr.gy, local / (pr.gx * pr.gy), ep);
}

extern "C" int oe_gemm_tn_grouped_plan(oe_tn_problem* problems, int n, int target_blocks) {
    OE_REQUIRE(problems && n > 0 && target_blocks > 0, "oe_gemm_tn_grouped_plan: bad arguments");
    long tiles = 0;
    for (int i = 0; i < n; ++i) {
        oe_tn_problem& p = problems[i];
        OE_REQUIRE(p.a && p.b && p.c && p.m >= 4 && p.n >= 4 && p.k >= 1, "oe_gemm_tn_grouped_plan: problem %d: bad shape / null pointer", i);
        OE_REQUIRE((((uintptr_t)p.a | (uintptr_t)p.b) & 15) == 0 && p.lda % 4 == 0 && p.ldb % 4 == 0 && p.lda >= (p.m + 3) / 4 * 4 &&
                       p.ldb >= (p.n + 3) / 4 * 4 && p.ldc >= p.n,
                   "oe_gemm_tn_grouped_plan: problem %d: operands not 16-byte aligned / leading dimensions too short", i);
        p.gx = oe_cdiv(p.n, TN_COLS);
        p.gy = oe_cdiv(p.m, TN_COLS);
        tiles += (long)p.gx * p.gy;
    }
    const int split = (int)min(16L, max(1L, (target_blocks + tiles / 2) / tiles));
    int blocks = 0;
    for (int i = 0; i < n; ++i) {
        oe_tn_problem& p = problems[i];
        int nz = min(split, max(1, p.k / 128));
        p.k_chunk = oe_cdiv(oe_cdiv(p.k, nz), TN_KROWS) * TN_KROWS;
        p.nz = oe_cdiv(p.k, p.k_chunk);
        p.block_start = blocks;
        blocks += p.gx * p.gy * p.nz;
    }
    return blocks;
}

extern "C" int oe_gemm_tn_grouped(const oe_tn_problem* problems_dev, int n, int total_blocks, int precision, void* stream) {
    OE_REQUIRE(problems_dev && n > 0 && total_blocks > 0, "oe_gemm_tn_grouped: bad arguments");
    OE_REQUIRE(precision == 1 || precision == 3 || precision == 6, "oe_gemm_tn_grouped: precision must be 1 (bf16), 3 (bf16x3) or 6 (bf16x6)");
    if (precision == 6)
        hipLaunchKernelGGL((gemm_tn_grouped_kernel<6>), dim3(total_blocks), dim3(TN_THREADS), 0, (hipStream_t)stream, problems_dev, n);
    else if (precision == 3)
        hipLaunchKernelGGL((gemm_tn_grouped_kernel<3>), dim3(total_blocks), dim3(TN_THREADS), 0, (hipStream_t)stream, problems_dev, n);
    else
        hipLaunchKernelGGL((gemm_tn_grouped_kernel<1>), dim3(total_blocks), dim3(TN_THREADS), 0, (hipStream_t)stream, problems_dev, n);
    OE_LAUNCH_CHECK("oe_gemm_tn_grouped");
    return 0;
}

int oe_gemm_tn_planes_try(const OperandDesc& A, const OperandDesc& B, float* C, long ldc, int M, int N, int K, int sk, const EpiParams& ep,
                          int terms, hipStream_t st) {
    static const int mode = getenv("OE_GEMM_TN_PLANES") ? atoi(getenv("OE_GEMM_TN_PLANES")) : 1;
    if (!mode) return 1;
    const int Mr = (M + 3) / 4 * 4, Nr = (N + 3) / 4 * 4;
    if (!A.vec_ok || !B.vec_ok || A.ld < Mr || B.ld < Nr || M < 4 || N < 4 || K < 1) return 1;
    if (ep.bias || ep.act || ep.preact_out || ep.actgrad_in || ep.residual || ep.rowmask || ep.drop_p > 0.f || ep.beta != 1.f || ep.scatter) return 1;
    if (sk > 1 && !ep.atomic) return 1;
    const int gx = oe_cdiv(N, TN_COLS), gy = oe_cdiv(M, TN_COLS);
    if (mode == 1 && (gx * gy < 12 || K < 2048)) return 1;
    int nz = 1;
    static const int blocks_target = getenv("OE_TN_BLOCKS") ? atoi(getenv("OE_TN_BLOCKS")) : 256;
    if (ep.atomic) {
        nz = max(1, blocks_target / (gx * gy));
        nz = min(nz, max(1, K / 128));
    }
    int kc = oe_cdiv(oe_cdiv(K, nz), TN_KROWS) * TN_KROWS;
    nz = oe_cdiv(K, kc);
    if (terms == 6)
        hipLaunchKernelGGL((gemm_tn_planes_kernel<6>), dim3(gx * gy * nz), dim3(TN_THREADS), 0, st, A.p, A.ld, B.p, B.ld, C, ldc, M, N, Mr, Nr, K, kc, gx, gy, ep);
    else if (terms == 3)
        hipLaunchKernelGGL((gemm_tn_planes_kernel<3>), dim3(gx * gy * nz), dim3(TN_THREADS), 0, st, A.p, A.ld, B.p, B.ld, C, ldc, M, N, Mr, Nr, K, kc, gx, gy, ep);
    else
        hipLaunchKernelGGL((gemm_tn_planes_kernel<1>), dim3(gx * gy * nz), dim3(TN_THREADS), 0, st, A.p, A.ld, B.p, B.ld, C, ldc, M, N, Mr, Nr, K, kc, gx, gy, ep);
    OE_LAUNCH_CHECK("oe_gemm (bf16 mfma, k-major planes)");
    return 0;
}
```

openeat_amd/hip.py:

```python
from __future__ import annotations

import ctypes as C
import os
from typing import Optional

import torch

PROFILE = None

GEMM_PRECISION = int(os.environ.get("OE_GEMM_PRECISION", "0"))

_LIB_PATH = os.environ.get("OE_HIP_LIB") or os.path.join(os.path.dirname(os.path.abspath(__file__)), "lib", "libopeneat_hip.so")
_lib = None

ACT = {"none": 0, None: 0, "relu": 1, "swish": 2, "tanh": 3, "hardtanh": 4, "selu": 5, "gelu": 6}
GATHER_NONE, GATHER_A, GATHER_B = 0, 1, 2

c_fp = C.c_void_p


class GemmArgs(C.Structure):
    _fields_ = [
        ("a", c_fp), ("lda", C.c_long), ("a_kmajor", C.c_int),
        ("b", c_fp), ("ldb", C.c_long), ("b_kmajor", C.c_int),
# ... 1 lines not shown
        ("m", C.c_int), ("n", C.c_int), ("k", C.c_int),
        ("split_k", C.c_int),
        ("alpha", C.c_float), ("alpha_dev", c_fp),
        ("bias", c_fp),
        ("act", C.c_int),
        ("preact_out", c_fp), ("actgrad_in", c_fp), ("ld_aux", C.c_long),
        ("drop_p", C.c_float), ("seed", C.c_ulonglong), ("seed_dev", c_fp),
        ("rowmask", c_fp),
        ("residual", c_fp), ("ldr", C.c_long), ("res_row_mod", C.c_int), ("beta", C.c_float),
        ("accumulate", C.c_int), ("atomic_out", C.c_int),
        ("conv_gather", C.c_int), ("conv_t1", C.c_int), ("conv_f1", C.c_int), ("conv_t2", C.c_int),
        ("conv_f2", C.c_int), ("conv_c", C.c_int),
        ("a_colsum", c_fp),
        ("precision", C.c_int),
        ("conv_k", C.c_int), ("conv_s", C.c_int),
        ("conv_kh", C.c_int),
        ("out_scatter", C.c_int), ("sc_t1", C.c_int), ("sc_f1", C.c_int), ("sc_t2", C.c_int), ("sc_f2", C.c_int), ("sc_s", C.c_int),
        ("a_planes", c_fp), ("a_plane_stride", C.c_long), ("b_planes", c_fp), ("b_plane_stride", C.c_long),
        ("c_planes", c_fp), ("c_plane_stride", C.c_long), ("ldcp", C.c_long),
        ("conv_korder", C.c_int),
        ("actgrad_bf16", C.c_int),
        ("planes_k_padded", C.c_int),
    ]


class AttnArgs(C.Structure):
    _fields_ = [
        ("q", c_fp), ("q_bstride", C.c_long), ("q_rstride", C.c_long),
        ("k", c_fp), ("k_bstride", C.c_long), ("k_rstride", C.c_long),
        ("v", c_fp), ("v_bstride", C.c_long), ("v_rstride", C.c_long),
        ("out", c_fp), ("o_bstride", C.c_long), ("o_rstride", C.c_long),
        ("lse", c_fp),
        ("mask", c_fp), ("mask_bstride", C.c_long), ("mask_rstride", C.c_long),
        ("keybias", c_fp),
        ("B", C.c_int), ("H", C.c_int), ("T1", C.c_int), ("T2", C.c_int), ("D", C.c_int),
        ("scale", C.c_float),
        ("drop_p", C.c_float), ("seed", C.c_ulonglong), ("seed_dev", c_fp),
        ("d_out", c_fp), ("dq", c_fp), ("dk", c_fp), ("dv", c_fp), ("dkeybias", c_fp), ("delta", c_fp),
        ("precision", C.c_int), ("causal", C.c_int),
    ]


class LnPrologue(C.Structure):
    _fields_ = [
        ("dy", c_fp), ("x", c_fp), ("stats", c_fp), ("gamma", c_fp), ("add", c_fp),
        ("dx", c_fp), ("g", c_fp), ("ws", c_fp),
        ("g_alpha", C.c_float), ("g_p", C.c_float), ("g_seed", C.c_ulonglong), ("g_rowmask", c_fp), ("ln_rowmask", c_fp),
        ("beta", c_fp), ("gamma2", c_fp), ("stats2", c_fp), ("ws2", c_fp),
    ]

    def fill(self, ln):
        dp = lambda t: None if t is None else t.data_ptr()
        self.dy, self.x, self.stats, self.gamma, self.add = dp(ln["dy"]), dp(ln["x"]), dp(ln["stats"]), dp(ln["gamma"]), dp(ln.get("add"))
        self.dx, self.g, self.ws = dp(ln["dx"]), dp(ln["g"]), dp(ln["ws"])
        self.g_alpha, self.g_p, self.g_seed = ln["alpha"], ln["p"], ln["seed"]
        self.g_rowmask, self.ln_rowmask = dp(ln.get("rowmask")), dp(ln.get("ln_rowmask"))
        self.beta, self.gamma2, self.stats2, self.ws2 = dp(ln.get("beta")), dp(ln.get("gamma2")), dp(ln.get("stats2")), dp(ln.get("ws2"))


class LnfPrologue(C.Structure):
    _fields_ = [("x", c_fp), ("gamma", c_fp), ("beta", c_fp), ("eps", C.c_float), ("y", c_fp), ("stats", c_fp), ("rowmask", c_fp),
                ("gamma2", c_fp), ("beta2", c_fp), ("eps2", C.c_float), ("u", c_fp), ("stats2", c_fp)]

    def fill(self, q):
        dp = lambda t: None if t is None else t.data_ptr()
        self.x, self.gamma, self.beta, self.eps = dp(q["x"]), dp(q["gamma"]), dp(q["beta"]), float(q["eps"])
        self.y, self.stats, self.rowmask = dp(q["y"]), dp(q["stats"]), dp(q.get("rowmask"))
        self.gamma2, self.beta2, self.eps2 = dp(q.get("gamma2")), dp(q.get("beta2")), float(q.get("eps2") or 0.0)
        self.u, self.stats2 = dp(q.get("u")), dp(q.get("stats2"))


class LnEpilogue(C.Structure):
    _fields_ = [("x", c_fp), ("stats", c_fp), ("gamma", c_fp), ("beta", c_fp), ("act", C.c_int), ("dx", c_fp), ("ws", c_fp)]


class FfnArgs(C.Structure):
    _fields_ = [
        ("x", c_fp), ("ldx", C.c_long),
        ("w1p", c_fp), ("b1", c_fp), ("w2p", c_fp), ("b2", c_fp),
        ("rows", C.c_int), ("d", C.c_int), ("ff", C.c_int), ("act", C.c_int), ("precision", C.c_int),
        ("drop_in", C.c_float), ("seed_in", C.c_ulonglong), ("drop_out", C.c_float), ("seed_out", C.c_ulonglong),
        ("seed_dev", c_fp),
        ("pre_out", c_fp), ("act_out", c_fp),
        ("residual", c_fp), ("ldr", C.c_long), ("beta", C.c_float),
        ("y", c_fp), ("ldy", C.c_long),
        ("ln", LnPrologue), ("lnf", LnfPrologue),
    ]


class RowGemmArgs(C.Structure):
    _fields_ = [
        ("x", c_fp), ("ldx", C.c_long),
        ("wp", c_fp), ("bias", c_fp),
        ("rows", C.c_int), ("k", C.c_int), ("n", C.c_int),
        ("drop_p", C.c_float), ("seed", C.c_ulonglong), ("seed_dev", c_fp),
        ("rowmask", c_fp),
        ("residual", c_fp), ("ldr", C.c_long), ("beta", C.c_float),
        ("y", c_fp), ("ldy", C.c_long),
        ("act", C.c_int), ("preact_out", c_fp), ("actgrad_in", c_fp), ("ld_aux", C.c_long),
        ("ln", LnPrologue), ("lnf", LnfPrologue), ("lne", LnEpilogue),
    ]


class HipLibraryMissing(RuntimeError):
    pass


def lib():
    global _lib
    if _lib is None:
        if not os.path.exists(_LIB_PATH):
            raise HipLibraryMissing(
                f"{_LIB_PATH} not found - build it with `python -c 'import __graft_entry__ as g; g.build()'` "
                "(openeat_amd has no CPU fallback)")
        _lib = C.CDLL(_LIB_PATH)
        _declare(_lib)
    return _lib


def exported_symbols():
    return list(_SIGNATURES)


class TnProblem(C.Structure):
    _fields_ = [("a", C.c_void_p), ("b", C.c_void_p), ("c", C.c_void_p), ("a_colsum", C.c_void_p), ("alpha_dev", C.c_void_p),
                ("lda", C.c_long), ("ldb", C.c_long), ("ldc", C.c_long), ("m", C.c_int), ("n", C.c_int), ("k", C.c_int),
                ("alpha", C.c_float), ("k_chunk", C.c_int), ("gx", C.c_int), ("gy", C.c_int), ("nz", C.c_int),
                ("block_start", C.c_int), ("reserved", C.c_int)]


I, L, F, P, U64, SZ = C.c_int, C.c_long, C.c_float, c_fp, C.c_ulonglong, C.c_size_t
_SIGNATURES = {
    "oe_last_error": (C.c_char_p, []),
    "oe_abi_version": (I, []),
    "oe_capture_unjoined_streams": (I, [P, C.POINTER(C.c_void_p), I, C.POINTER(I)]),
    "oe_stamp": (I, [P, I, P]),
    "oe_gemm_f32": (I, [C.POINTER(GemmArgs), P]),
    "oe_split_planes": (I, [P, L, L, L, P, L, L, P]),
    "oe_gemm_pl_launches": (L, []),
    "oe_gemm_hyb_launches": (L, []),
    "oe_gemm_pl_config": (I, [I, I, I, I]),
    "oe_gemm_pl_hybrid": (I, [I]),
    "oe_gemm_tn_grouped_plan": (I, [C.POINTER(TnProblem), I, I]),
    "oe_gemm_tn_grouped": (I, [P, I, I, I, P]),
    "oe_ffn_packed_bytes": (SZ, [I, I, I]),
    "oe_ffn_supported": (I, [I, I, I, I]),
    "oe_ffn_pack_weights": (I, [P, P, I, I, I, P, P, P]),
    "oe_ffn_pack_weights_bwd": (I, [P, P, I, I, I, P, P, P]),
    "oe_ffn_pack_weights_table": (I, [P, I, I, I, I, P]),
    "oe_ffn_fwd": (I, [C.POINTER(FfnArgs), P]),
    "oe_ffn_bwd": (I, [C.POINTER(FfnArgs), P]),
    "oe_ffn6_config": (I, [I]),
    "oe_rowgemm6_supported": (I, [I, I]),
    "oe_rowgemm6": (I, [C.POINTER(RowGemmArgs), P]),
    "oe_rowgemm6_pack_table": (I, [P, I, L, P]),
    "oe_rowgemm6_form": (I, [I, I, I]),
    "oe_colsum_f32": (I, [P, L, I, I, F, P, P, I, P]),
    "oe_layernorm_fwd": (I, [P, P, P, F, I, I, P, I, P, P, P]),
    "oe_layernorm_fwd_pl": (I, [P, P, P, F, I, I, P, I, P, P, P, L, P]),
    "oe_layernorm_bwd_workspace_floats": (SZ, [I, I]),
    "oe_layernorm_pair_fwd": (I, [P, P, P, F, P, P, F, I, I, P, P, P, P, P]),
    "oe_layernorm_pair_bwd_dx_drop": (I, [P, P, P, P, P, P, P, I, I, P, P, P, F, F, U64, P, P, P, P, P]),
    "oe_layernorm_bwd": (I, [P, P, P, P, I, P, I, I, P, P, P, P, P, P, P]),
    "oe_layernorm_bwd_dx": (I, [P, P, P, P, I, P, I, I, P, P, P, P, P]),
    "oe_layernorm_param_reduce": (I, [P, I, I, P, P, P]),
    "oe_layernorm_param_reduce_table": (I, [P, I, I, I, P]),
    "oe_layernorm_bwd_dx_drop": (I, [P, P, P, P, I, P, I, I, P, P, P, P, F, F, U64, P, P, P, P]),
    "oe_layernorm_bwd_dx_drop_pl": (I, [P, P, P, P, I, P, I, I, P, P, P, P, F, F, U64, P, P, P, P, L, P]),
    "oe_ctc_workspace_floats": (SZ, [I, I, I]),
    "oe_ctc_config": (I, [I, I]),
    "oe_ctc_loss_fused": (I, [P, L, I, I, I, P, P, I, P, F, P, P, P, P, P, P]),
    "oe_ctc_loss_fused_stats": (I, [P, L, I, I, I, P, P, I, P, F, P, P, P, P, P, P, I, P]),
    "oe_ctc_greedy": (I, [P, L, I, I, I, P, I, P, P, P, P]),
    "oe_ctc_align_workspace_bytes": (SZ, [I, I, I]),
    "oe_ctc_align": (I, [P, L, I, I, I, P, P, I, P, P, P, P, P, P, P, P]),
    "oe_attention_fwd": (I, [C.POINTER(AttnArgs), P]),
    "oe_attention_bwd": (I, [C.POINTER(AttnArgs), P]),
    "oe_relpos_prepare": (I, [P, L, L, P, L, P, P, I, I, I, I, F, P, P, P]),
    "oe_relpos_backward": (I, [P, P, P, L, L, P, L, P, P, I, I, I, I, F, P, P, L, P, P, P]),
    "oe_glu_fwd": (I, [P, L, I, P, P]),
    "oe_glu_bwd": (I, [P, P, L, I, P, P]),
    "oe_dropout_scale": (I, [P, L, I, F, F, U64, P, P, P, P]),
    "oe_embed_fwd": (I, [P, P, P, L, I, I, I, F, P, P]),
    "oe_embed_bwd": (I, [P, P, L, I, I, F, P, P]),
    "oe_swap_last2": (I, [P, L, I, I, P, I, P]),
    "oe_pad1_nhwc": (I, [P, I, I, I, I, P, P]),
    "oe_pad1_nhwc_planes": (I, [P, I, I, I, I, P, P, L, P]),
    "oe_conv_dgrad_k3s2_weights": (I, [P, I, P, P]),
    "oe_axpby": (I, [P, P, L, F, F, P, P, P]),
    "oe_loss_combine": (I, [P, P, P, F, F, F, P, P]),
    "oe_loss_combine_bwd": (I, [P, F, F, F, P, P, P, P]),
    "oe_act_fwd": (I, [P, L, I, P, P]),
    "oe_act_grad": (I, [P, P, L, I, P, P]),
    "oe_log_softmax": (I, [P, L, I, P, P]),
    "oe_topk_rows": (I, [P, L, I, I, I, P, P, P]),
    "oe_logprob_gather": (I, [P, L, I, P, I, P, P, P]),
    "oe_att_inputs": (I, [P, P, I, I, I, I, I, P, P, P, P, P, P]),
    "oe_masked_softmax_fwd": (I, [P, P, L, L, I, I, I, I, F, U64, P, P, P, P]),
    "oe_masked_softmax_bwd": (I, [P, P, L, I, F, U64, P, P, P]),
    "oe_global_cmvn": (I, [P, P, P, L, I, P, P]),
    "oe_conv1_fwd": (I, [P, P, P, I, I, I, I, P, P]),
    "oe_conv1_fwd_pl": (I, [P, P, P, I, I, I, I, P, P, L, P]),
    "oe_conv1_wgrad": (I, [P, P, I, I, I, I, P, P, P]),
    "oe_col2im_relu": (I, [P, P, I, I, I, I, P, P]),
    "oe_col2im_relu_ks": (I, [P, P, I, I, I, I, I, I, P, P]),
    "oe_dwconv_glu_fwd": (I, [P, P, P, P, I, I, I, I, I, P, P]),
    "oe_dwconv_glu_ln_fwd": (I, [P, P, P, P, I, I, I, I, I, P, P, P, F, I, P, P, P]),
    "oe_dwconv_glu_bwd_workspace_floats": (SZ, [I, I, I, I]),
    "oe_dwconv_glu_bwd": (I, [P, P, P, P, I, I, I, I, I, P, P, P, P, P, P]),
    "oe_lsm_workspace_bytes": (SZ, [L]),
    "oe_lsm_loss_fused": (I, [P, L, L, I, P, I, F, I, F, F, I, P, P, P]),
    "oe_fbank": (I, [P, P, I, L, I, I, I, I, F, F, P, P, P, P, P, F, P, P, P, P]),
    "oe_fbank_dither": (I, [P, P, I, L, I, I, I, I, F, F, P, P, P, P, P, F, P, P, F, U64, P, P]),
    "oe_utt_normalize": (I, [P, P, I, I, I, P]),
    "oe_spec_augment": (I, [P, P, I, I, I, P, I, P, I, F, P]),
    "oe_spec_substitute": (I, [P, I, I, I, P, I, I, P]),
    "oe_feature_dither": (I, [P, P, I, I, I, F, U64, P]),
    "oe_speed_perturb": (I, [P, L, P, P, I, I, P, L, P, P]),
    "oe_ctc_prefix_beam_workspace_bytes": (SZ, [I, I, I]),
    "oe_ctc_prefix_beam": (I, [P, P, I, I, P, I, I, P, P, P, P, P]),
    "oe_ctc_prefix_beam_host": (I, [P, P, I, I, I, P, P, P]),
    "oe_ctc_prefix_beam_host_batch": (I, [P, P, I, I, P, I, I, P, P, P, I]),
    "oe_ngram_score": (I, [P, I, P, L, I, I, I, I, I, P, I, P, L, P, I, I, I, P, P, P, P]),
    "oe_grad_norm_workspace_floats": (SZ, []),
    "oe_grad_norm": (I, [P, L, P, P, P]),
    "oe_adam_step": (I, [P, P, P, P, L, P, F, F, F, F, F, P, P, P]),
}


def _declare(l):
    for name, (res, args) in _SIGNATURES.items():
        fn = getattr(l, name)
        fn.restype = res
        fn.argtypes = args


def check(rc: int, what: str):
    if rc != 0:
        msg = lib().oe_last_error().decode("utf-8", "replace")
        raise RuntimeError(f"{what} failed (rc={rc}): {msg}")


def capture_unjoined_streams(origin: "torch.cuda.Stream", sides):
    sides = [s for s in sides if s is not None]
    arr = (C.c_void_p * max(len(sides), 1))(*[s.cuda_stream for s in sides])
    first = I(-1)
    n = lib().oe_capture_unjoined_streams(C.c_void_p(origin.cuda_stream), arr, len(sides), C.byref(first))
    if n < 0:
        check(n, "oe_capture_unjoined_streams")
    return n, (sides[first.value] if n > 0 else None)


def ptr(t: Optional[torch.Tensor]):
    return None if t is None else C.c_void_p(t.data_ptr())


def stream():
    return C.c_void_p(torch.cuda.current_stream().cuda_stream)


def _dev_f32(t: torch.Tensor, name: str):
    if not (t.is_cuda and t.dtype == torch.float32):
        raise TypeError(f"{name}: expected a float32 CUDA tensor, got {t.dtype} on {t.device}")


def gemm(a, b, c, m, n, k, *, lda, ldb, ldc, a_kmajor=False, b_kmajor=False, split_k=1, alpha=1.0, alpha_dev=None,
         bias=None, act=0, preact_out=None, actgrad_in=None, ld_aux=0, drop_p=0.0, seed=0, seed_dev=None, rowmask=None,
         residual=None, ldr=0, res_row_mod=0, beta=1.0, accumulate=False, atomic_out=False, conv=None, conv_gather=GATHER_NONE, precision=None, a_colsum=None,
         conv_kh=0, scatter=None, a_planes=None, b_planes=None, c_planes=None, conv_korder=0, actgrad_bf16=False):
    g = GemmArgs()
    g.a, g.lda, g.a_kmajor = (None if a is None else a.data_ptr()), lda, int(a_kmajor)
    g.b, g.ldb, g.b_kmajor = (None if b is None else b.data_ptr()), ldb, int(b_kmajor)
    g.c, g.ldc = c.data_ptr(), ldc
    g.m, g.n, g.k, g.split_k = m, n, k, split_k
    g.alpha = alpha
    g.alpha_dev = None if alpha_dev is None else alpha_dev.data_ptr()
    g.bias = None if bias is None else bias.data_ptr()
    g.act = act
    g.preact_out = None if preact_out is None else preact_out.data_ptr()
    g.actgrad_in = None if actgrad_in is None else actgrad_in.data_ptr()
    g.actgrad_bf16 = int(actgrad_bf16)
    g.ld_aux = ld_aux
    g.drop_p, g.seed = drop_p, seed
    g.seed_dev = None if seed_dev is None else seed_dev.data_ptr()
    g.rowmask = None if rowmask is None else rowmask.data_ptr()
    g.residual = None if residual is None else residual.data_ptr()
    g.ldr, g.beta, g.res_row_mod = ldr, beta, res_row_mod
    g.accumulate, g.atomic_out = int(accumulate), int(atomic_out)
    g.conv_gather = conv_gather
    g.precision = GEMM_PRECISION if precision is None else precision
    g.a_colsum = None if (a_colsum is None or g.precision == 0) else a_colsum.data_ptr()
    g.conv_kh = conv_kh
    g.conv_korder = conv_korder
    if g.precision == 6:
        if a_planes is not None and b_planes is not None:
            g.a_planes, g.a_plane_stride = a_planes.ptr, a_planes.stride
            g.b_planes, g.b_plane_stride = b_planes.ptr, b_planes.stride
            g.planes_k_padded = int(a_kmajor and b_kmajor and getattr(a_planes, "kpad", False) and getattr(b_planes, "kpad", False))
        elif b_planes is not None and a is not None:
            g.b_planes, g.b_plane_stride = b_planes.ptr, b_planes.stride
        if c_planes is not None:
            g.c_planes, g.c_plane_stride, g.ldcp = c_planes.ptr, c_planes.stride, c_planes.ld
    if scatter is not None:
        g.out_scatter = 1
        g.sc_t1, g.sc_f1, g.sc_t2, g.sc_f2, g.sc_s = scatter
    if conv is not None:
        g.conv_t1, g.conv_f1, g.conv_t2, g.conv_f2, g.conv_c = conv[:5]
        g.conv_k, g.conv_s = (conv[5], conv[6]) if len(conv) > 5 else (0, 0)
    if PROFILE is not None:
        e0, e1 = torch.cuda.Event(enable_timing=True), torch.cuda.Event(enable_timing=True)
        e0.record()
        check(lib().oe_gemm_f32(C.byref(g), stream()), "oe_gemm_f32")
        e1.record()
        PROFILE.append((e0, e1, 2.0 * m * n * k, (m, n, k, int(a_kmajor), int(b_kmajor), int(conv_gather), int(split_k))))
        return
    check(lib().oe_gemm_f32(C.byref(g), stream()), "oe_gemm_f32")


def tn_grouped_plan(problems, target_blocks: int = 384):
    n = len(problems)
    arr = (TnProblem * n)()
    dp = lambda t: None if t is None else t.data_ptr()
    for i, q in enumerate(problems):
        dy, x, out = q["dy"], q["x"], q["out"]
        p = arr[i]
        p.a, p.b, p.c, p.a_colsum, p.alpha_dev = dy.data_ptr(), x.data_ptr(), out.data_ptr(), dp(q.get("bias_out")), dp(q.get("alpha_dev"))
        p.lda, p.ldb, p.ldc = dy.stride(0), x.stride(0), out.stride(0)
        p.m, p.n, p.k, p.alpha = dy.shape[1], x.shape[1], dy.shape[0], float(q.get("alpha", 1.0))
    total = lib().oe_gemm_tn_grouped_plan(arr, n, int(target_blocks))
    if total < 0:
        return None
    return bytes(arr), total


def tn_grouped_launch(table_dev: torch.Tensor, n: int, total_blocks: int, precision=None, flops: float = 0.0):
    if PROFILE is not None:
        e0, e1 = torch.cuda.Event(enable_timing=True), torch.cuda.Event(enable_timing=True)
        e0.record()
        check(lib().oe_gemm_tn_grouped(C.c_void_p(table_dev.data_ptr()), n, total_blocks, GEMM_PRECISION if precision is None else precision,
                                       stream()), "oe_gemm_tn_grouped")
        e1.record()
        PROFILE.append((e0, e1, flops, ("tn_grouped", n, total_blocks, 0, 1, 1, 0)))
        return
    check(lib().oe_gemm_tn_grouped(C.c_void_p(table_dev.data_ptr()), n, total_blocks, GEMM_PRECISION if precision is None else precision,
                                   stream()), "oe_gemm_tn_grouped")


def ffn_fwd(x2, w1p, b1, w2p, b2, rows, d, ff, act, *, drop_in=0.0, seed_in=0, drop_out=0.0, seed_out=0, seed_dev=None, pre_out=None,
            act_out=None, residual=None, ldr=0, beta=1.0, y=None, precision=None, lnf=None):
    a = FfnArgs()
    dp = lambda t: None if t is None else t.data_ptr()
    a.x, a.ldx = x2.data_ptr(), x2.stride(0)
    if lnf is not None:
        a.lnf.fill(lnf)
    a.w1p, a.b1, a.w2p, a.b2 = w1p.data_ptr(), dp(b1), w2p.data_ptr(), dp(b2)
    a.rows, a.d, a.ff, a.act = rows, d, ff, act
    a.precision = GEMM_PRECISION if precision is None else precision
    a.drop_in, a.seed_in, a.drop_out, a.seed_out, a.seed_dev = drop_in, seed_in, drop_out, seed_out, dp(seed_dev)
    a.pre_out, a.act_out, a.residual, a.ldr, a.beta = dp(pre_out), dp(act_out), dp(residual), ldr, beta
    a.y, a.ldy = y.data_ptr(), y.stride(0)
    if PROFILE is not None:
        e0, e1 = torch.cuda.Event(enable_timing=True), torch.cuda.Event(enable_timing=True)
        e0.record()
        check(lib().oe_ffn_fwd(C.byref(a), stream()), "oe_ffn_fwd")
        e1.record()
        PROFILE.append((e0, e1, 4.0 * rows * d * ff, ("ffn_fwd", rows, d, ff, 0, 0, 1)))
        return
    check(lib().oe_ffn_fwd(C.byref(a), stream()), "oe_ffn_fwd")


def ffn_bwd(dy2, w2tp, w1tp, rows, d, ff, act, *, drop_in=0.0, seed_in=0, seed_dev=None, pre=None, dh=None, dx=None, precision=None, ln=None):
    a = FfnArgs()
    dp = lambda t: None if t is None else t.data_ptr()
    a.x, a.ldx = dy2.data_ptr(), dy2.stride(0)
    if ln is not None:
        a.ln.fill(ln)
    a.w1p, a.b1, a.w2p, a.b2 = w2tp.data_ptr(), None, w1tp.data_ptr(), None
    a.rows, a.d, a.ff, a.act = rows, d, ff, act
    a.precision = GEMM_PRECISION if precision is None else precision
    a.drop_in, a.seed_in, a.drop_out, a.seed_out, a.seed_dev = drop_in, seed_in, 0.0, 0, dp(seed_dev)
    a.pre_out, a.act_out, a.residual, a.ldr, a.beta = pre.data_ptr(), dh.data_ptr(), None, 0, 1.0
    a.y, a.ldy = dx.data_ptr(), dx.stride(0)
    if PROFILE is not None:
        e0, e1 = torch.cuda.Event(enable_timing=True), torch.cuda.Event(enable_timing=True)
        e0.record()
        check(lib().oe_ffn_bwd(C.byref(a), stream()), "oe_ffn_bwd")
        e1.record()
        PROFILE.append((e0, e1, 4.0 * rows * d * ff, ("ffn_bwd", rows, d, ff, 0, 0, 1)))
        return
    check(lib().oe_ffn_bwd(C.byref(a), stream()), "oe_ffn_bwd")


def rowgemm6(x, wp, y, rows, k, n, *, bias=None, drop_p=0.0, seed=0, seed_dev=None, rowmask=None, residual=None, ldr=0, beta=1.0,
             act=0, preact_out=None, actgrad_in=None, ld_aux=0, ln=None, lnf=None, lne=None):
    a = RowGemmArgs()
    dp = lambda t: None if t is None else t.data_ptr()
    a.x, a.ldx, a.wp, a.bias = (0 if x is None else x.data_ptr()), (k if x is None else x.stride(0)), wp.data_ptr(), dp(bias)
    a.rows, a.k, a.n = rows, k, n
    a.drop_p, a.seed, a.seed_dev, a.rowmask = drop_p, seed, dp(seed_dev), dp(rowmask)
    a.residual, a.ldr, a.beta = dp(residual), ldr, beta
    a.y, a.ldy = y.data_ptr(), y.stride(0)
    a.act, a.preact_out, a.actgrad_in, a.ld_aux = act, dp(preact_out), dp(actgrad_in), ld_aux
    if ln is not None:
        a.ln.fill(ln)
    if lnf is not None:
        a.lnf.fill(lnf)
    if lne is not None:
        a.lne.x, a.lne.stats, a.lne.gamma, a.lne.beta = dp(lne["x"]), dp(lne["stats"]), dp(lne["gamma"]), dp(lne["beta"])
        a.lne.act, a.lne.dx, a.lne.ws = int(lne["act"]), dp(lne["dx"]), dp(lne["ws"])
    if PROFILE is not None:
        e0, e1 = torch.cuda.Event(enable_timing=True), torch.cuda.Event(enable_timing=True)
        e0.record()
        check(lib().oe_rowgemm6(C.byref(a), stream()), "oe_rowgemm6")
        e1.record()
        PROFILE.append((e0, e1, 2.0 * rows * k * n, ("rowgemm6", rows, n, k, 0, 0, 1)))
        return
    check(lib().oe_rowgemm6(C.byref(a), stream()), "oe_rowgemm6")


def call(name, *args):
    conv = []
    for a in args:
        if isinstance(a, torch.Tensor):
            conv.append(C.c_void_p(a.data_ptr()))
        else:
            conv.append(a)
    check(getattr(lib(), name)(*conv, stream()), name)


def attn_args(q, k, v, out, lse, B, H, T1, T2, D, scale, *, q_strides, k_strides, v_strides, o_strides, mask=None,
              mask_strides=(0, 0), keybias=None, drop_p=0.0, seed=0, seed_dev=None, d_out=None, dq=None, dk=None, dv=None,
              dkeybias=None, delta=None, precision=None, causal=False):
    a = AttnArgs()
    a.precision = GEMM_PRECISION if precision is None else precision
    dp = lambda t: None if t is None else t.data_ptr()
    a.q, (a.q_bstride, a.q_rstride) = dp(q), q_strides
    a.k, (a.k_bstride, a.k_rstride) = dp(k), k_strides
    a.v, (a.v_bstride, a.v_rstride) = dp(v), v_strides
    a.out, (a.o_bstride, a.o_rstride) = dp(out), o_strides
    a.lse = dp(lse)
    a.mask, (a.mask_bstride, a.mask_rstride) = dp(mask), mask_strides
    a.keybias = dp(keybias)
    a.B, a.H, a.T1, a.T2, a.D = B, H, T1, T2, D
    a.scale, a.drop_p, a.seed = scale, drop_p, seed
    a.seed_dev = dp(seed_dev)
    a.d_out, a.dq, a.dk, a.dv, a.dkeybias, a.delta = dp(d_out), dp(dq), dp(dk), dp(dv), dp(dkeybias), dp(delta)
    a.causal = int(bool(causal))
    return a


def attention_fwd(a: AttnArgs):
    check(lib().oe_attention_fwd(C.byref(a), stream()), "oe_attention_fwd")


def attention_bwd(a: AttnArgs):
    check(lib().oe_attention_bwd(C.byref(a), stream()), "oe_attention_bwd")


def ctc_prefix_beam_device(top_logp: torch.Tensor, top_idx: torch.Tensor, lens: Optional[torch.Tensor], beam: int, raw: bool = False):
    if not (top_logp.is_cuda and top_idx.is_cuda and top_logp.dtype == torch.float32 and top_idx.dtype == torch.int64):
        raise TypeError("ctc_prefix_beam_device: float32 / int64 CUDA tensors required")
    top_logp, top_idx = top_logp.contiguous(), top_idx.contiguous()
    B, T = top_logp.shape[0], top_logp.shape[1]
    ml = max(T, 1)
# ... 47 lines not shown
```

openeat_amd/ops.py:

```python
from __future__ import annotations

import itertools
import os
import math
import weakref
from typing import Optional

import torch

from . import hip
from . import arena as _arena
from . import planes as _planes

ACT_NONE, ACT_RELU, ACT_SWISH, ACT_TANH, ACT_HARDTANH, ACT_SELU, ACT_GELU = 0, 1, 2, 3, 4, 5, 6
ACT_IDS = {"relu": ACT_RELU, "swish": ACT_SWISH, "tanh": ACT_TANH, "hardtanh": ACT_HARDTANH, "selu": ACT_SELU, "gelu": ACT_GELU,
           "none": ACT_NONE}
GEMM_FUSED_ACTS = (ACT_NONE, ACT_RELU, ACT_SWISH)


_seed_counter = itertools.count(0x5EED0001)
_seed_dev: Optional[torch.Tensor] = None


def next_seed() -> int:
# ... 438 lines not shown


def join_side_stream():
    flush_wgrads()
    if _side_stream is not None:
        torch.cuda.current_stream().wait_stream(_side_stream)
    if _decoder_stream is not None:
        torch.cuda.current_stream().wait_stream(_decoder_stream)
    if _ctc_stream is not None:
        torch.cuda.current_stream().wait_stream(_ctc_stream)


PARALLEL_DECODERS = False
_decoder_stream = None


_ctc_stream = None


def ctc_stream():
    global _ctc_stream
    if _ctc_stream is None:
        _ctc_stream = torch.cuda.Stream()
    return _ctc_stream


def decoder_stream():
    global _decoder_stream
    if _decoder_stream is None:
        _decoder_stream = torch.cuda.Stream()
    return _decoder_stream


class _Side:

    def __init__(self, *tensors):
        self.tensors = [t for t in tensors if isinstance(t, torch.Tensor)]

    def __enter__(self):
        side = side_stream()
        side.wait_stream(torch.cuda.current_stream())
        self.cm = torch.cuda.stream(side)
        self.cm.__enter__()

    def __exit__(self, *exc):
        self.cm.__exit__(*exc)
        for t in self.tensors:
            t.record_stream(_side_stream)
        return False


class _Inline:
    def __enter__(self):
        return None

    def __exit__(self, *exc):
        return False


def _wgrad_ctx(to_arena: bool, *tensors):
    return _Side(*tensors) if (ASYNC_WGRAD and to_arena) else _Inline()


WGRAD_DEFER = 0
_deferred = []


def _run_wgrad(to_arena: bool, tensors, fn, desc=None):
    if WGRAD_DEFER > 0 and to_arena:
        _deferred.append((fn, [t for t in tensors if isinstance(t, torch.Tensor)], torch.cuda.current_stream(), desc))
        if len(_deferred) >= WGRAD_DEFER:
            flush_wgrads()
        return
    with _wgrad_ctx(to_arena, *tensors):
        fn()


WGRAD_GROUPED = os.environ.get("OE_WGRAD_GROUPED", "1") == "1"
WGRAD_GROUP_MAX_TILES = int(os.environ.get("OE_WGRAD_GROUP_MAX_TILES", "12"))
WGRAD_GROUP_BLOCKS = int(os.environ.get("OE_WGRAD_GROUP_BLOCKS", "512"))
_TN_TABLES = []


def _group_wgrads(descs):
    if hip.GEMM_PRECISION == 0:
        return set()
    idx = []
    for i, d in enumerate(descs):
        if d is None:
            continue
        dy, x, out = d["dy"], d["x"], d["out"]
        tiles = -(-dy.shape[1] // 128) * -(-x.shape[1] // 128)
        ok = (dy.dim() == 2 and x.dim() == 2 and out.dim() == 2 and dy.stride(1) == 1 and x.stride(1) == 1 and out.stride(1) == 1 and
              dy.shape[0] == x.shape[0] and dy.shape[0] >= 128 and tiles <= WGRAD_GROUP_MAX_TILES and dy.shape[1] >= 4 and x.shape[1] >= 4 and
              dy.stride(0) % 4 == 0 and x.stride(0) % 4 == 0 and dy.data_ptr() % 16 == 0 and x.data_ptr() % 16 == 0 and
              dy.stride(0) >= -(-dy.shape[1] // 4) * 4 and x.stride(0) >= -(-x.shape[1] // 4) * 4)
        if ok:
            idx.append(i)
    if len(idx) < 2:
        return set()
    plan = hip.tn_grouped_plan([descs[i] for i in idx], WGRAD_GROUP_BLOCKS)
    if plan is None:
        return set()
    host, total = plan
    table = torch.empty(len(host), dtype=torch.uint8, device=descs[idx[0]]["dy"].device)
    if LN_TABLE is not None and not LN_TABLE.eager:
        LN_TABLE.uploads.append((table, host))
    else:
        pinned = torch.frombuffer(bytearray(host), dtype=torch.uint8).pin_memory()
        table.copy_(pinned, non_blocking=True)
        _TN_TABLES.append((table, pinned))
        del _TN_TABLES[:-64]
    hip.tn_grouped_launch(table, len(idx), total,
                          flops=sum(2.0 * descs[i]["dy"].shape[0] * descs[i]["dy"].shape[1] * descs[i]["x"].shape[1] for i in idx))
    return set(idx)


def drop_deferred():
    global _deferred
    _deferred = []


WGRAD_FLUSH_INLINE = False


def flush_wgrads():
    global _deferred
    if not _deferred:
        return
    if WGRAD_FLUSH_INLINE:
        grouped = _group_wgrads([d for _, _, _, d in _deferred]) if WGRAD_GROUPED else set()
        for i, (fn, _, _, _) in enumerate(_deferred):
            if i not in grouped:
                fn()
        _deferred = []
        return
    side = side_stream()
    origins = []
    for _, _, st, _ in _deferred:
        if all(st != o for o in origins):
            origins.append(st)
    for st in origins:
        side.wait_stream(st)
    with torch.cuda.stream(side):
        grouped = _group_wgrads([d for _, _, _, d in _deferred]) if WGRAD_GROUPED else set()
        for i, (fn, _, _, _) in enumerate(_deferred):
            if i not in grouped:
                fn()
    for _, ts, _, _ in _deferred:
        for t in ts:
            t.record_stream(side)
    _deferred = []


def wgrad(param, dy, x, alpha=1.0, alpha_dev=None):
    tgt = _arena.grad_target(param)
    if tgt is None:
        return gemm_tn(dy, x, alpha=alpha, alpha_dev=alpha_dev).view(param.shape)
    out = tgt.view(dy.shape[1], x.shape[1])
    pl = wgrad_planes(dy, x)
    _run_wgrad(True, (dy, x, alpha_dev) + _pl_tensors(pl), lambda: gemm_tn(dy, x, out=out, alpha=alpha, alpha_dev=alpha_dev, planes=pl),
               desc=dict(dy=dy, x=x, out=out, alpha=alpha, alpha_dev=alpha_dev, bias_out=None))
    return None


def _pl_tensors(pl):
    return tuple(q.t for q in pl if q is not None) if pl is not None else ()


def _sink_swapped(param, src, A, Bd, Cd):
    tgt = _arena.grad_target(param)
    if tgt is None:
        out = torch.empty_like(param)
        hip.call("oe_swap_last2", src, A, Bd, Cd, out, 0)
        return out
    hip.call("oe_swap_last2", src, A, Bd, Cd, tgt, 1)
    return None


def wgrad_bias(w, b, dy, x, alpha=1.0, alpha_dev=None):
    if b is None:
        return wgrad(w, dy, x, alpha, alpha_dev), None
    N, K = dy.shape[1], x.shape[1]
    tw, tb = _arena.grad_target(w), _arena.grad_target(b)
    ow = tw.view(N, K) if tw is not None else _new(N, K, like=dy, zero=True)
    ob = tb if tb is not None else _new(N, like=dy, zero=True)
    pl = wgrad_planes(dy, x)
    _run_wgrad(tw is not None and tb is not None, (dy, x, alpha_dev) + _pl_tensors(pl),
               lambda: gemm_tn(dy, x, out=ow, alpha=alpha, alpha_dev=alpha_dev, bias_out=ob, planes=pl),
               desc=dict(dy=dy, x=x, out=ow, alpha=alpha, alpha_dev=alpha_dev, bias_out=ob))
    return (None if tw is not None else ow.view(w.shape)), (None if tb is not None else ob)


def bgrad(param, dy, alpha=1.0, alpha_dev=None, n=None):
    if param is None:
        return None
    tgt = _arena.grad_target(param)
    if tgt is None:
        return colsum(dy, alpha, alpha_dev, n)
    colsum(dy, alpha, alpha_dev, n, out=tgt)
    return None


def grad_sink(param):
    tgt = _arena.grad_target(param)
    if tgt is None:
        z = torch.zeros_like(param)
        return z, z
    return tgt.view(param.shape), None


def _fused_rows(parts, cat_dim0=True):
    a = _arena.active()
    if a is not None and a.enabled and a.adjacent(*parts):
        rows = sum(p.shape[0] for p in parts)
        return torch.as_strided(parts[0], (rows,) + tuple(parts[0].shape[1:]), parts[0].stride()), True
    return torch.cat(list(parts), 0), False


def dropout_scale(x, alpha=1.0, p=0.0, seed=0, rowmask=None, cols=None):
    out = torch.empty_like(x)
    cols = x.shape[-1] if cols is None else cols
    hip.call("oe_dropout_scale", x, x.numel(), cols, alpha, p, seed, _seed_dev, rowmask, out)
    return out


def _ln_ws(like, rows, d):
    return _new(hip.lib().oe_layernorm_bwd_workspace_floats(rows, d), like=like)


def _ln_fwd(x, gamma, beta, eps, rows, d, rowmask, act, y, stats, planes_out=True):
    pl = _planes.new_output(y.view(rows, d)) if (planes_out and _planes.active() and rows * d >= _planes.MIN_SPLIT_ELEMS) else None
    if pl is None:
        hip.call("oe_layernorm_fwd", x, gamma, beta, eps, rows, d, rowmask, act, y, stats)
    else:
        hip.call("oe_layernorm_fwd_pl", x, gamma, beta, eps, rows, d, rowmask, act, y, stats, pl.t, pl.stride)


LN_TABLE_CAPACITY = 512


class _LnTable:
    __slots__ = ("dev", "eager", "entries", "keep", "max_rows", "max_d", "launched", "uploads")

    def __init__(self, dev, eager):
        self.dev, self.eager, self.entries, self.keep, self.uploads = dev, eager, [], [], []
        self.max_rows, self.max_d, self.launched = 1, 4, 0

    def add(self, ws, rows, d, dg, db):
        self.entries.append((ws.data_ptr(), rows, d, dg.data_ptr(), db.data_ptr()))
        self.keep.append(ws)
        self.max_rows, self.max_d = max(self.max_rows, rows), max(self.max_d, d)


LN_TABLE = None
LN_EAGER_TABLE = os.environ.get("OE_LN_EAGER_TABLE", "1") == "1"
_LN_EAGER_DEV = {}
_LN_EAGER_PINNED = []


def ln_table_begin(device, eager=False):
    global LN_TABLE
    if eager:
        dev = _LN_EAGER_DEV.get(device)
        if dev is None:
            dev = _LN_EAGER_DEV[device] = torch.zeros(LN_TABLE_CAPACITY, 5, dtype=torch.int64, device=device)
    else:
        dev = torch.zeros(LN_TABLE_CAPACITY, 5, dtype=torch.int64, device=device)
    LN_TABLE = _LnTable(dev, eager)
    return LN_TABLE


def ln_table_flush():
    t = LN_TABLE
# ... 379 lines not shown
    def forward(ctx, x, y):
        x, y = _chk(x, "add"), _chk(y, "add")
        out = torch.empty_like(x)
        hip.call("oe_axpby", x, y, x.numel(), 1.0, 1.0, None, out)
        return out

    @staticmethod
    def backward(ctx, d):
        return d, d


def add(x, y):
    return AddFn.apply(x, y)


class LossCombineFn(torch.autograd.Function):

    @staticmethod
    def forward(ctx, loss_att, loss_att_r, loss_ctc, ctc_weight, reverse_weight):
        f = lambda t: None if t is None else _chk(t.reshape(1), "loss")
        la, lr, lc = f(loss_att), f(loss_att_r), f(loss_ctc)
        out = _new(1, like=la)
        hip.call("oe_loss_combine", lc, la, lr, float(ctc_weight), float(reverse_weight), 1.0, out)
        ctx.cfg = (float(ctc_weight), float(reverse_weight), lr is not None, lc is not None)
        return out.view(())

    @staticmethod
    def backward(ctx, g):
        wc, r, has_r, has_c = ctx.cfg
        g = g.contiguous().reshape(1)
        d = _new(3, like=g)
        hip.call("oe_loss_combine_bwd", g, wc, r, 1.0, d[0:1] if has_c else None, d[1:2], d[2:3] if has_r else None)
        return d[1].view(()), (d[2].view(()) if has_r else None), (d[0].view(()) if has_c else None), None, None


def combine_losses(loss_att, loss_att_r=None, loss_ctc=None, ctc_weight=0.0, reverse_weight=0.0):
    return LossCombineFn.apply(loss_att, loss_att_r, loss_ctc, ctc_weight, reverse_weight)


class CmvnFn(torch.autograd.Function):
    @staticmethod
    def forward(ctx, x, mean, istd):
        x = _chk(x, "cmvn")
        y = torch.empty_like(x)
        hip.call("oe_global_cmvn", x, mean, istd, x.numel(), x.shape[-1], y)
        return y

    @staticmethod
    def backward(ctx, dy):
        raise NotImplementedError("GlobalCMVN is applied to input features, which carry no gradient")


def global_cmvn(x, mean, istd):
    return CmvnFn.apply(x, mean, istd)


FUSED_FFN = os.environ.get("OE_FUSED_FFN", "1") == "1"
FUSED_FFN_MIN_ROWS = int(os.environ.get("OE_FUSED_FFN_MIN_ROWS", "4096"))
FUSED_FFN_BWD = {"1": True, "0": False}.get(os.environ.get("OE_FUSED_FFN_BWD", ""), None)


def _ffn_bwd_fused() -> bool:
    return (hip.GEMM_PRECISION == 6) if FUSED_FFN_BWD is None else bool(FUSED_FFN_BWD)


def _ffn6_takes_ln(d, ff):
    return hip.GEMM_PRECISION == 6 and d == 256 and ff % 256 == 0 and hip.lib().oe_ffn6_config(-1) in (0, 3)


def _ffn_fused_ok(x2, w1, w2, act, res2):
    d, ff = w1.shape[1], w1.shape[0]
    if hip.GEMM_PRECISION == 0 or x2.shape[0] < FUSED_FFN_MIN_ROWS or not hip.lib().oe_ffn_supported(d, ff, hip.GEMM_PRECISION, act):
        return False
    ok = lambda t: t is None or (t.data_ptr() % 16 == 0 and t.stride(-1) == 1)
    return (w1.is_contiguous() and w2.is_contiguous() and ok(x2) and ok(res2) and x2.stride(0) % 4 == 0 and
            (res2 is None or res2.stride(0) % 4 == 0) and w1.data_ptr() % 16 == 0 and w2.data_ptr() % 16 == 0)



_FFN = _PackTable(9)
FFN_PACK_TABLE = os.environ.get("OE_FFN_PACK_TABLE", "1") == "1"
FFN_FWD_FUSED_LAUNCHES = 0
FFN_BWD_FUSED_LAUNCHES = 0


def _ffn_dead(key, ent):
    w1, w2 = ent["w1"](), ent["w2"]()
    return w1 is None or w2 is None or w1.data_ptr() != key[0] or w2.data_ptr() != key[1]


def ffn_packs_clear():
    _FFN.clear()
    row_packs_clear()


def pack_tables_sweep():
    if torch.cuda.is_available() and not torch.cuda.is_current_stream_capturing():
        _FFN.sweep(_ffn_dead)
        _FFN.upload()
        _ROW.sweep(_row_dead)
        _ROW.upload()


def _ffn_packed(w1, w2, d, ff, bwd=False):
    prec = hip.GEMM_PRECISION
    nbytes = hip.lib().oe_ffn_packed_bytes(d, ff, prec)
    capturing = torch.cuda.is_current_stream_capturing()
    key = (w1.data_ptr(), w2.data_ptr(), prec)
    ent = _FFN.entries.get(key) if FFN_PACK_TABLE else None
    if ent is not None and ((ent["d"], ent["ff"]) != (d, ff) or ent["w1"]() is not w1 or ent["w2"]() is not w2 or _ffn_dead(key, ent)):
        if capturing:
            ent = False
        else:
            _FFN.drop(key)
            ent = None
    if ent is None and FFN_PACK_TABLE and not capturing and isinstance(w1, torch.nn.Parameter) and isinstance(w2, torch.nn.Parameter):
        bufs = [torch.empty(nbytes, dtype=torch.uint8, device=w1.device) for _ in range(4)]
        ent = dict(w1=weakref.ref(w1), w2=weakref.ref(w2), bufs=bufs, d=d, ff=ff, gen=[-1, -1], ver=[None, None])
        if not _FFN.add(key, [key[0], key[1]] + [b.data_ptr() for b in bufs] + [d, ff, {6: 3, 3: 2}.get(prec, 1)], ent, w1.device):
            ent = None
    if not ent:
        a = torch.empty(nbytes, dtype=torch.uint8, device=w1.device)
        b = torch.empty(nbytes, dtype=torch.uint8, device=w1.device)
        hip.call("oe_ffn_pack_weights_bwd" if bwd else "oe_ffn_pack_weights", w1, w2, d, ff, prec, a, b)
        return a, b
    gen, ver, kind = _planes.weights_generation(), (w1._version, w2._version), int(bwd)
    if ent["gen"][kind] != gen or ent["ver"][kind] != ver:
        if not capturing:
            _FFN.sweep(_ffn_dead)
            _FFN.upload()
        if not _FFN.dirty and len(_FFN.entries) > 1 and ent["gen"][0] != gen and ent["gen"][1] != gen:
            alive = _FFN.entries.values()
            hip.call("oe_ffn_pack_weights_table", _FFN.dev, _FFN.n, max(e["d"] for e in alive), max(e["ff"] for e in alive), prec)
            _pack_done(_FFN)
            for e in alive:
                w1e, w2e = e["w1"](), e["w2"]()
                v = (w1e._version, w2e._version) if (w1e is not None and w2e is not None) else None
                e["gen"], e["ver"] = [gen, gen], [v, v]
        else:
            _pack_wait(_FFN)
            hip.call("oe_ffn_pack_weights_bwd" if bwd else "oe_ffn_pack_weights", w1, w2, d, ff, prec, ent["bufs"][2 * kind], ent["bufs"][2 * kind + 1])
            _pack_done(_FFN)
            ent["gen"][kind], ent["ver"][kind] = gen, ver
    else:
        _pack_wait(_FFN)
    return ent["bufs"][2 * kind], ent["bufs"][2 * kind + 1]


class FeedForwardFn(torch.autograd.Function):

    @staticmethod
    def forward(ctx, x, w1, b1, w2, b2, act, p_in, residual, out_scale, p_out):
        x = _chk(x, "feed_forward", keep_pending=True)
        d = x.shape[-1]
        x2 = x.reshape(-1, d)
        M, ff = x2.shape[0], w1.shape[0]
        s_in, s_out = (next_seed() if p_in > 0 else 0), (next_seed() if p_out > 0 else 0)
        res2 = None if residual is None else _chk(residual, "residual").reshape(-1, w2.shape[0])
        lnf_p = _PENDING_LNF.take(x2)
        fused_now = FUSED_FFN and _ffn_fused_ok(x2, w1, w2, act, res2)
        lnf = None
        if lnf_p is not None:
            if (fused_now and _ffn6_takes_ln(d, ff) and x2.is_contiguous() and M == lnf_p.rows and
                    (lnf_p.gamma2 is None or (res2 is not None and lnf_p.u is not None and res2.data_ptr() == lnf_p.u.data_ptr()))):
                lnf = lnf_p.prologue()
            else:
                lnf_p.resolve()
        if fused_now:
            need = any(ctx.needs_input_grad)
            pre = _new(M, ff, like=x) if need else None
            a = _new(M, ff, like=x) if need else None
            w1p, w2p = _ffn_packed(w1, w2, d, ff)
            y = _new(M, d, like=x)
            hip.ffn_fwd(x2, w1p, b1, w2p, b2, M, d, ff, act, drop_in=p_in, seed_in=s_in, drop_out=p_out, seed_out=s_out,
                        seed_dev=_seed_dev, pre_out=pre, act_out=a, residual=res2, ldr=0 if res2 is None else res2.stride(0),
                        beta=out_scale, y=y, lnf=lnf)
            global FFN_FWD_FUSED_LAUNCHES
            FFN_FWD_FUSED_LAUNCHES += 1
            if lnf is not None:
                lnf_p.fused()
            ctx.save_for_backward(x2, w1, w2, pre, a)
            ctx.biases = (b1, b2)
            ctx.cfg = (act, p_in, s_in, out_scale, p_out, s_out, residual is not None, x.shape)
            ctx.fused = True
            ln_fuse = LN_BWD_FUSE and FUSE_OUT_DROP and _ln_rows_fusable(M, d) and _ffn_bwd_fused() and _ffn6_takes_ln(d, ff)
            return _tag_out_drop(y.view(*x.shape[:-1], w2.shape[0]), out_scale, p_out, s_out, ln_fuse=ln_fuse)
        ctx.fused = False
        pre = _new(M, ff, like=x)
        if act in GEMM_FUSED_ACTS:
            a = gemm_nt(x2, w1, b1, act=act, preact_out=pre, ld_aux=ff, drop_p=p_in, seed=s_in, seed_dev=_seed_dev, out_planes=True)
        else:
            gemm_nt(x2, w1, b1, out=pre)
            a = torch.empty_like(pre)
            hip.call("oe_act_fwd", pre, pre.numel(), act, a)
            if p_in > 0:
                a = dropout_scale(a, 1.0, p_in, s_in)
        y = gemm_nt(a, w2, b2, drop_p=p_out, seed=s_out, seed_dev=_seed_dev, residual=res2,
                    ldr=0 if res2 is None else res2.stride(0), beta=out_scale)
        ctx.save_for_backward(x2, w1, w2, pre, a)
        ctx.biases = (b1, b2)
        ctx.cfg = (act, p_in, s_in, out_scale, p_out, s_out, residual is not None, x.shape)
        return _tag_out_drop(y.view(*x.shape[:-1], w2.shape[0]), out_scale, p_out, s_out)

    @staticmethod
    def backward(ctx, dy):
        x2, w1, w2, pre, a = ctx.saved_tensors
        act, p_in, s_in, out_scale, p_out, s_out, has_res, in_shape = ctx.cfg
        dy = dy.contiguous()
        dy2 = dy.view(-1, w2.shape[0])
        g2 = dy2 if (p_out == 0 and out_scale == 1.0) else _out_drop_grad(dy2, out_scale, p_out, s_out)
        b1, b2 = ctx.biases
        pend = _PENDING_LN.take(g2)
        if ctx.fused and _ffn_bwd_fused() and g2.stride(0) % 4 == 0:
            M, d, ff = g2.shape[0], w2.shape[0], w1.shape[0]
            w2tp, w1tp = _ffn_packed(w1, w2, d, ff, bwd=True)
            dh, dx = _new(M, ff, like=g2), _new(M, d, like=g2)
            ln = None
            if pend is not None and not pend.done:
                if _ffn6_takes_ln(d, ff) and g2.is_contiguous() and g2.data_ptr() == pend.g.data_ptr() and M == pend.rows:
                    ln = pend.prologue()
                else:
                    pend.resolve()
            hip.ffn_bwd(g2, w2tp, w1tp, M, d, ff, act, drop_in=p_in, seed_in=s_in, seed_dev=_seed_dev, pre=pre, dh=dh, dx=dx, ln=ln)
            global FFN_BWD_FUSED_LAUNCHES
            FFN_BWD_FUSED_LAUNCHES += 1
            if ln is not None:
                pend.fused()
            dw2, db2 = wgrad_bias(w2, b2, g2, a)
            dw1, db1 = wgrad_bias(w1, b1, dh, x2)
            return dx.view(in_shape), dw1, db1, dw2, db2, None, None, (dy if has_res else None), None, None
        if pend is not None:
            pend.resolve()
        dw2, db2 = wgrad_bias(w2, b2, g2, a)
        if act in GEMM_FUSED_ACTS:
            dh = gemm_nn(g2, w2, act=act, actgrad_in=pre, ld_aux=pre.stride(0), drop_p=p_in, seed=s_in, seed_dev=_seed_dev, out_planes=True)
        else:
            dh = gemm_nn(g2, w2)
            if p_in > 0:
                dh = dropout_scale(dh, 1.0, p_in, s_in)
            dh = _act_grad(dh, pre, act)
        dw1, db1 = wgrad_bias(w1, b1, dh, x2)
        dx = gemm_nn(dh, w1).view(in_shape)
        return dx, dw1, db1, dw2, db2, None, None, (dy if has_res else None), None, None


def feed_forward(x, w1, b1, w2, b2, act, p_in=0.0, residual=None, out_scale=1.0, p_out=0.0):
    return FeedForwardFn.apply(x, w1, b1, w2, b2, act, p_in, residual, out_scale, p_out)


def mask_bytes(mask: torch.Tensor) -> torch.Tensor:
    if mask.dtype == torch.bool:
        return mask.contiguous().view(torch.uint8)
    return (mask if mask.dtype == torch.uint8 else mask.to(torch.uint8)).contiguous()


def _mask_u8(mask: Optional[torch.Tensor]):
    if mask is None:
        return None, (0, 0)
    m = mask_bytes(mask)
    assert m.dim() == 3, "mask must be (B, 1|T1, T2)"
    return m, (m.shape[1] * m.shape[2], 0 if m.shape[1] == 1 else m.shape[2])


CAUSAL_SELF_ATTENTION = False


class causal_self_attention:
    def __enter__(self):
        global CAUSAL_SELF_ATTENTION
        self.old, CAUSAL_SELF_ATTENTION = CAUSAL_SELF_ATTENTION, True

    def __exit__(self, *exc):
        global CAUSAL_SELF_ATTENTION
        CAUSAL_SELF_ATTENTION = self.old
        return False


class AttentionFn(torch.autograd.Function):

    @staticmethod
    def forward(ctx, xq, xkv, wq, bq, wk, bk, wv, bv, wo, bo, mask, pos_emb, wpos, pu, pv, H, p_attn, residual, p_out, pp_in=None):
        xq = _chk(xq, "attention query", keep_pending=True)
        self_attn = xkv is None
        B, T1, d = xq.shape
        D = d // H
        scale = 1.0 / math.sqrt(D)
        xq2 = xq.view(-1, d)
        if self_attn:
            T2 = T1
            wqkv, _ = _fused_rows((wq, wk, wv))
            bqkv, _ = _fused_rows((bq, bk, bv))
            qkv = gemm_nt(xq2, wqkv, bqkv)
            q, k, v = qkv[:, :d], qkv[:, d:2 * d], qkv[:, 2 * d:]
            qs = ks = vs = (T1 * 3 * d, 3 * d)
            xkv2 = xq2
        else:
            xkv = _chk(xkv, "attention key/value")
            T2 = xkv.shape[1]
            xkv2 = xkv.view(-1, d)
            q = gemm_nt(xq2, wq, bq)
            wkv, _ = _fused_rows((wk, wv))
            bkv, _ = _fused_rows((bk, bv))
            kv = gemm_nt(xkv2, wkv, bkv)
            k, v = kv[:, :d], kv[:, d:]
            qs, ks, vs = (T1 * d, d), (T2 * 2 * d, 2 * d), (T2 * 2 * d, 2 * d)
            qkv = None
        rel = pos_emb is not None
        kp = keybias = pp = None
        k_att, k_att_s = k, ks
        if rel:
            assert self_attn and pos_emb.shape[-2] == T2
            pe2 = _chk(pos_emb, "pos_emb").reshape(-1, d)
            pp = pp_in if pp_in is not None else gemm_nt(pe2, wpos)
            kp = _new(B, T2, d, like=xq)
            keybias = _new(B, H, T2, like=xq)
# ... 670 lines not shown
```

openeat_amd/planes.py:

```python
from __future__ import annotations

import os
from typing import Optional

import torch

from . import hip

POLICY = os.environ.get("OE_PLANES", "conv")
MIN_SPLIT_ELEMS = int(os.environ.get("OE_PLANES_MIN", str(1 << 19)))


_DEBUG = bool(os.environ.get("OE_PLANES_DEBUG"))


def available() -> bool:
    return POLICY != "0" and hip.GEMM_PRECISION == 6


def active() -> bool:
    return POLICY in ("all", "ln") and hip.GEMM_PRECISION == 6


WEIGHT_PLANES = os.environ.get("OE_WEIGHT_PLANES", "1") == "1"
HYB_MIN_ROWS = int(os.environ.get("OE_HYB_MIN_ROWS", "12288"))


def weights_presplit() -> bool:
    return hip.GEMM_PRECISION == 6 and (POLICY in ("all", "ln") or (WEIGHT_PLANES and POLICY != "0"))


def arena_weight(w2d: torch.Tensor) -> Optional[Planes]:
    if not weights_presplit() or w2d.dim() != 2 or w2d.stride(1) != 1 or w2d.stride(0) % 8 or w2d.shape[1] % 8:
        return None
    from . import arena as _arena
    a = _arena.active()
    if a is None:
        return None
    ptr = w2d.data_ptr()
    off = (ptr - a.flat.data_ptr()) // 4
    if not (0 <= off < a.numel) or ptr % 32:
        return None
    a.step_planes()
    return Planes(a.planes, a.planes.data_ptr() + 2 * off, a.planes_stride, w2d.stride(0), w2d.shape[0], w2d.shape[1])


def split_activations() -> bool:
    return POLICY == "all" and hip.GEMM_PRECISION == 6


class Planes:
    __slots__ = ("t", "ptr", "stride", "ld", "rows", "cols", "kpad")

    def __init__(self, t: torch.Tensor, ptr: int, stride: int, ld: int, rows: int, cols: int, kpad: bool = False):
        self.t, self.ptr, self.stride, self.ld, self.rows, self.cols = t, ptr, stride, ld, rows, cols
        self.kpad = kpad


def alloc(rows: int, cols: int, device) -> Planes:
    rp = (rows + 15) // 16 * 16
    t = torch.empty(3, rp, cols, dtype=torch.bfloat16, device=device)
    if rp != rows:
        t[:, rows:].zero_()
    return Planes(t, t.data_ptr(), rp * cols, cols, rows, cols, kpad=True)


import contextlib
from collections import OrderedDict

_REG: "OrderedDict[int, tuple]" = OrderedDict()
_NO_GRAD_KEEP = 64
_CAPTURE_DEPTH = 0
ISOLATE_CAPTURES = True


def clear():
    _REG.clear()
    new_pass()


def clear_all():
    _WCACHE.clear()
    clear()
    try:
        from . import ops as _ops
        _ops.ffn_packs_clear()
    except ImportError:
        pass


@contextlib.contextmanager
def capture_scope():
    global _REG, _CAPTURE_DEPTH
    if not ISOLATE_CAPTURES:
        yield
        return
    from . import arena as _arena
    a = _arena.active()
    if a is not None and weights_presplit():
        a.alloc_planes()
    outer, _REG = _REG, OrderedDict()
    _CAPTURE_DEPTH += 1
    try:
        yield
    finally:
        _CAPTURE_DEPTH -= 1
        _REG = outer
        bump_generation()
        if a is not None:
            a.mark_step()
        from . import ops as _ops
        _ops.pack_events_forget()


_GEN = 0


def weights_generation() -> int:
    return _GEN


def bump_generation():
    global _GEN
    _GEN += 1


def new_pass():
    bump_generation()
    from . import arena as _arena
    from . import ops as _ops
    _ops.pack_tables_sweep()
    a = _arena.active()
    if a is not None:
        a.mark_step()


def _dense2d(t: torch.Tensor) -> bool:
    return t.dim() == 2 and t.stride(1) == 1 and t.stride(0) == t.shape[1] and t.shape[1] % 8 == 0 and t.data_ptr() % 16 == 0


def register(t2d: torch.Tensor, pl: Planes):
    _REG[t2d.data_ptr()] = (pl, t2d, t2d._version)
    if not torch.is_grad_enabled():
        while len(_REG) > _NO_GRAD_KEEP:
            _REG.popitem(last=False)


# ... 70 lines not shown
```

Baseline: 1.993 million audio-frames/s.

## Emit FFN activation and hidden-gradient as bf16 planes and group weight-gradient GEMMs

The fused FFN forward now writes the activation directly as three bf16 split planes, and the fused backward writes dh the same way, in place of fp32 tensors. The weight-gradient TN GEMMs then read these pre-split planes without re-splitting, and the two FFN weight gradients go out as one grouped launch. This cuts fp32 activation traffic and the split work inside the wgrad kernels, and saves a launch. In exchange it adds plane stores through LDS in the FFN epilogue, 1.5x storage for the saved activation, and a new planes path in the TN kernel.

After: 1.943 million audio-frames/s. 0.975x the previous value.

```diff
diff --git a/include/openeat_hip.h b/include/openeat_hip.h
--- a/include/openeat_hip.h
+++ b/include/openeat_hip.h
@@ -80,6 +80,7 @@
     float drop_out; unsigned long long seed_out;
     const unsigned long long* seed_dev;
     float* pre_out; float* act_out;
+    void* act_planes; long act_plane_stride;
     const float* residual; long ldr; float beta;
     float* y; long ldy;
     oe_ln_prologue ln;
@@ -87,6 +88,7 @@
 } oe_ffn_args;
 size_t oe_ffn_packed_bytes(int d, int ff, int precision);
 int oe_ffn_supported(int d, int ff, int precision, int act);
+int oe_ffn_planes_out_supported(int d, int ff, int precision);
 int oe_ffn_pack_weights(const float* w1, const float* w2, int d, int ff, int precision, void* w1p, void* w2p, void* stream);
 int oe_ffn_fwd(const oe_ffn_args* args, void* stream);
 int oe_ffn_pack_weights_bwd(const float* w1, const float* w2, int d, int ff, int precision, void* w2t_packed, void* w1t_packed, void* stream);
@@ -118,9 +120,12 @@
     int m, n, k;
     float alpha;
     int k_chunk, gx, gy, nz, block_start, reserved;
+    const void* a_planes; long a_plane_stride;
+    const void* b_planes; long b_plane_stride;
 } oe_tn_problem;
 int oe_gemm_tn_grouped_plan(oe_tn_problem* problems_host, int n, int target_blocks);
 int oe_gemm_tn_grouped(const oe_tn_problem* problems_dev, int n, int total_blocks, int precision, void* stream);
+int oe_gemm_tn_grouped_planes(const oe_tn_problem* problems_dev, int n, int total_blocks, void* stream);
 
 int oe_colsum_f32(const float* x, long ldx, int m, int n, float alpha, const float* alpha_dev,
                   float* out, int accumulate, void* stream);
diff --git a/openeat_amd/csrc/ffn.hip b/openeat_amd/csrc/ffn.hip
--- a/openeat_amd/csrc/ffn.hip
+++ b/openeat_amd/csrc/ffn.hip
@@ -360,7 +360,8 @@
     OE_REQUIRE(((((uintptr_t)a->x) | ((uintptr_t)a->y) | ((uintptr_t)a->residual) | ((uintptr_t)a->pre_out) | ((uintptr_t)a->act_out) |
                  ((uintptr_t)a->w1p) | ((uintptr_t)a->w2p)) & 15) == 0, "oe_ffn_fwd: 16-byte alignment required");
     OE_REQUIRE(a->drop_in >= 0.f && a->drop_in < 1.f && a->drop_out >= 0.f && a->drop_out < 1.f, "oe_ffn_fwd: dropout rate out of range");
-    OE_REQUIRE(!(a->act_out && !a->pre_out), "oe_ffn_fwd: act_out needs pre_out (the store count is a compile-time constant)");
+    OE_REQUIRE(!((a->act_out || a->act_planes) && !a->pre_out), "oe_ffn_fwd: act_out needs pre_out (the store count is a compile-time constant)");
+    OE_REQUIRE(!a->act_planes || a->precision == 6, "oe_ffn_fwd: act_planes exists in precision 6 only (oe_ffn_planes_out_supported)");
     if (a->precision == 6) return oe_ffn6_run(a, false, stream);
     FfnParams p{};
     p.x = a->x; p.ldx = a->ldx; p.w1p = (const __bf16*)a->w1p; p.b1 = a->b1; p.w2p = (const __bf16*)a->w2p; p.b2 = a->b2;
@@ -374,7 +375,8 @@
 }
 
 extern "C" int oe_ffn_bwd(const oe_ffn_args* a, void* stream) {
-    OE_REQUIRE(a && (a->x || a->ln.dy) && a->w1p && a->w2p && a->y && a->pre_out && a->act_out, "oe_ffn_bwd: null pointer");
+    OE_REQUIRE(a && (a->x || a->ln.dy) && a->w1p && a->w2p && a->y && a->pre_out && (a->act_out || a->act_planes), "oe_ffn_bwd: null pointer");
+    OE_REQUIRE(!a->act_planes || a->precision == 6, "oe_ffn_bwd: act_planes exists in precision 6 only (oe_ffn_planes_out_supported)");
     OE_REQUIRE(!a->ln.dy || a->precision == 6, "oe_ffn_bwd: the LayerNorm-backward prologue exists in precision 6 only");
     OE_REQUIRE(oe_ffn_supported(a->d, a->ff, a->precision, a->act), "oe_ffn_bwd: unsupported d=%d ff=%d precision=%d act=%d", a->d, a->ff,
                a->precision, a->act);
diff --git a/openeat_amd/csrc/ffn6.hip b/openeat_amd/csrc/ffn6.hip
--- a/openeat_amd/csrc/ffn6.hip
+++ b/openeat_amd/csrc/ffn6.hip
@@ -57,6 +57,7 @@
     const unsigned char* w1p; const float* b1;
     const unsigned char* w2p; const float* b2;
     float* pre; float* act_out;
+    unsigned char* act_planes; long act_pbytes;
     const float* residual; long ldr; float beta;
     float* y; long ldy;
     int rows, ff, act;
@@ -148,6 +149,37 @@
         }
     }
     if ((BWD || NOUT == 2) && p.act_out) store_tile(p.act_out);
+    if ((BWD || NOUT == 2) && p.act_planes && mrow < p.rows) {
+        unsigned char* pp = reinterpret_cast<unsigned char*>(patch);
+        const int sw = (lq >> 2) & 3;
+        f6_wave_sync();
+#pragma unroll
+        for (int s = 0; s < 2; ++s) {
+            float v[8];
+#pragma unroll
+            for (int e = 0; e < 8; ++e) v[e] = hv[8 * s + e];
+            oe_bf16x8 hp[3];
+            oe_split8<3>(v, hp);
+#pragma unroll
+            for (int pn = 0; pn < 3; ++pn) {
+                unsigned char* d = pp + pn * 2048 + lq * 64 + lk * 8;
+                *reinterpret_cast<bf16x4*>(d + ((2 * s) ^ sw) * 16) = __builtin_shufflevector(hp[pn], hp[pn], 0, 1, 2, 3);
+                *reinterpret_cast<bf16x4*>(d + ((2 * s + 1) ^ sw) * 16) = __builtin_shufflevector(hp[pn], hp[pn], 4, 5, 6, 7);
+            }
+        }
+        f6_wave_sync();
+#pragma unroll
+        for (int ps = 0; ps < 2; ++ps) {
+            const int row = ps * 16 + (lane >> 2), j = lane & 3;
+            const bool live = mrow + row < p.rows;
+#pragma unroll
+            for (int pn = 0; pn < 3; ++pn) {
+                uint4 v = *reinterpret_cast<const uint4*>(pp + pn * 2048 + row * 64 + (j ^ ((row >> 2) & 3)) * 16);
+                if (!live) v = make_uint4(0u, 0u, 0u, 0u);
+                *reinterpret_cast<uint4*>(p.act_planes + pn * p.act_pbytes + (((mrow + row) * p.ff + ft * 32 + 8 * j) << 1)) = v;
+            }
+        }
+    }
 }
 __device__ __forceinline__ void f6_write_planes(const float (&hv)[16], unsigned char* hdst, int s_stride, int lane) {
 #pragma unroll
@@ -374,7 +406,7 @@
     constexpr int X_BYTES = 3 * BM * XP * 2;
     constexpr int H_WAVE = 2 * RT * 3 * 1024;
     constexpr int H_BYTES = 4 * H_WAVE;
-    static_assert(H_WAVE >= 32 * 36 * 4, "the wave's h region doubles as its 32 x 36 fp32 patch");
+    static_assert(H_WAVE >= 32 * 36 * 4 && H_WAVE >= 3 * 32 * 64, "the wave's h region doubles as its 32 x 36 fp32 patch / its three 32 x 32 bf16 plane patches");
     constexpr int PIECE = 3 * 1024;
     constexpr int NT = RT * DPW;
     static_assert(NG == 1 || (NT % 2 == 0 && 8 * (NT / 2) * 4096 <= X_BYTES), "the groups' exchange buffer reuses the x planes");
@@ -1212,6 +1244,7 @@
 }
 
 int oe_ffn6_supported(int d, int ff) { return (d == 128 || d == 256 || d == 512) && ff > 0 && ff % 128 == 0 && ff <= 8192; }
+extern "C" int oe_ffn_planes_out_supported(int d, int ff, int precision) { return precision == 6 && oe_ffn6_supported(d, ff); }
 
 static int ffn6_mode_v = getenv("OE_FFN6_MODE") ? atoi(getenv("OE_FFN6_MODE")) : 0;
 static int ffn6_mode() { return ffn6_mode_v; }
@@ -1226,6 +1259,12 @@
     p.pre = a->pre_out; p.act_out = a->act_out; p.residual = a->residual; p.ldr = a->ldr; p.beta = a->beta; p.y = a->y; p.ldy = a->ldy;
     p.rows = a->rows; p.ff = a->ff; p.act = a->act; p.p_in = a->drop_in; p.seed_in = a->seed_in; p.p_out = a->drop_out; p.seed_out = a->seed_out;
     p.seed_dev = a->seed_dev;
+    if (a->act_planes) {
+        OE_REQUIRE((((uintptr_t)a->act_planes) & 15) == 0 && a->act_plane_stride % 8 == 0 &&
+                       a->act_plane_stride >= (long)oe_cdiv(a->rows, 32) * 32 * a->ff,
+                   "oe_ffn: act_planes needs 16-byte alignment and a plane stride of whole 8-element groups that covers ceil(rows / 32) * 32 rows");
+        p.act_planes = (unsigned char*)a->act_planes; p.act_pbytes = a->act_plane_stride * 2;
+    }
     if (a->ln.dy) {
         const char* why = ln_pro_check(a->ln);
         OE_REQUIRE(bwd && why == nullptr, "oe_ffn: LayerNorm prologue: %s", bwd ? why : "backward only");
@@ -1236,7 +1275,7 @@
         OE_REQUIRE(!bwd && why == nullptr, "oe_ffn: LayerNorm-forward prologue: %s", bwd ? "forward only" : why);
         p.lnf = lnf_pro_of(a->lnf);
     }
-    const int nout = a->act_out ? 2 : a->pre_out ? 1 : 0;
+    const int nout = (a->act_out || a->act_planes) ? 2 : a->pre_out ? 1 : 0;
     hipStream_t st = (hipStream_t)stream;
     const int mode = ffn6_mode();
     const bool two_groups = (a->ff % 256 == 0) && mode != 1 && mode != 2;
diff --git a/openeat_amd/csrc/gemm.hip b/openeat_amd/csrc/gemm.hip
--- a/openeat_amd/csrc/gemm.hip
+++ b/openeat_amd/csrc/gemm.hip
@@ -166,7 +166,9 @@
 static bool vec_ok(const void* p, long ld) { return ((uintptr_t)p % 16 == 0) && (ld % 4 == 0); }
 
 extern "C" int oe_gemm_f32(const oe_gemm_args* g, void* stream) {
-    OE_REQUIRE(g && g->c && (g->a || (g->a_planes && g->b_planes && g->precision == 6)) && (g->b || (g->a_planes && g->b_planes && g->precision == 6)),
+    const bool wg_pl = g && g->precision == 6 && g->planes_k_padded == 2 && (g->a_planes || g->b_planes);
+    OE_REQUIRE(g && g->c && (g->a || (g->a_planes && (g->b_planes || wg_pl) && g->precision == 6)) &&
+                   (g->b || (g->b_planes && (g->a_planes || wg_pl) && g->precision == 6)),
                "oe_gemm_f32: null operand");
     OE_REQUIRE(g->m > 0 && g->n > 0 && g->k >= 0, "oe_gemm_f32: bad shape m=%d n=%d k=%d", g->m, g->n, g->k);
     OE_REQUIRE(g->split_k >= 1, "oe_gemm_f32: split_k must be >= 1");
@@ -222,6 +224,11 @@
                "oe_gemm_f32: precision must be 0 (fp32), 1 (bf16), 3 (bf16x3) or 6 (bf16x6)");
     OE_REQUIRE(g->conv_korder == 0 || (g->conv_korder == 1 && ga && g->precision == 6 && g->a_planes && g->b_planes && sk <= 1 && A.C % 32 == 0),
                "oe_gemm_f32: conv_korder 1 needs a gather on A, precision 6, pre-split operands, no split of the reduction and C %% 32 == 0");
+    if (wg_pl) {
+        OE_REQUIRE(g->a_kmajor && g->b_kmajor && !ga && !gb && g->conv_korder == 0 && !g->c_planes,
+                   "oe_gemm_f32: planes_k_padded = 2 is for plain weight gradients (a_kmajor, b_kmajor, no gather, no planes output)");
+        return oe_gemm_tn_planes_try(A, B, g->c, g->ldc, M, N, K, sk, ep, 6, st, g->a_planes, g->a_plane_stride, g->b_planes, g->b_plane_stride);
+    }
     if (g->precision == 6 && g->a_planes && g->b_planes) {
         const int r = oe_gemm_pl_try(A, B, g->a_planes, g->a_plane_stride, g->b_planes, g->b_plane_stride, g->c, g->ldc, M, N, K, sk, ep,
                                      g->a_kmajor, g->b_kmajor, ga, gb, st, g->conv_korder, g->planes_k_padded != 0);
diff --git a/openeat_amd/csrc/gemm_common.h b/openeat_amd/csrc/gemm_common.h
--- a/openeat_amd/csrc/gemm_common.h
+++ b/openeat_amd/csrc/gemm_common.h
@@ -124,7 +124,8 @@
                           const EpiParams& ep, bool a_kmajor, bool b_kmajor, bool ga, bool gb, int terms, hipStream_t st);
 
 int oe_gemm_tn_planes_try(const OperandDesc& A, const OperandDesc& B, float* C, long ldc, int M, int N, int K, int sk, const EpiParams& ep,
-                          int terms, hipStream_t st);
+                          int terms, hipStream_t st, const void* a_planes = nullptr, long a_pstride = 0, const void* b_planes = nullptr,
+                          long b_pstride = 0);
 int oe_gemm_dma_try(const OperandDesc& A, const OperandDesc& B, float* C, long ldc, int M, int N, int K, int sk, const EpiParams& ep,
                     bool a_kmajor, bool b_kmajor, bool gather_b, int terms, int tile, hipStream_t st);
 int oe_gemm_hyb_try(const OperandDesc& A, const OperandDesc& B, const void* Bp, long b_pstride, float* C, long ldc, int M, int N, int K, int sk,
diff --git a/openeat_amd/csrc/gemm_tn.hip b/openeat_amd/csrc/gemm_tn.hip
--- a/openeat_amd/csrc/gemm_tn.hip
+++ b/openeat_amd/csrc/gemm_tn.hip
@@ -78,17 +78,45 @@
     }
 }
 
-template <int TERMS>
-__device__ __forceinline__ void tn_block(const float* __restrict__ Ap, long lda, const float* __restrict__ Bp, long ldb,
-                                         float* __restrict__ C, long ldc, int M, int N, int Mr, int Nr, int K, int k_chunk,
-                                         int tile_x, int tile_y, int tile_z, const EpiParams& ep) {
-    constexpr int NPL = oe_npl<TERMS>::N;
-    constexpr int OP_ELEMS = NPL * TN_PLANE;
-    constexpr int BUF_ELEMS = 2 * OP_ELEMS;
-    constexpr int XCH_BYTES = 4 * 2 * 32 * 64 * 4;
-    constexpr int IMG_ELEMS = (2 * BUF_ELEMS * 2 >= XCH_BYTES) ? 2 * BUF_ELEMS : XCH_BYTES / 2;
-    __shared__ __attribute__((aligned(16))) __bf16 img[IMG_ELEMS];
-    __shared__ float csum_s[TN_COLS];
+typedef unsigned tn_u32x4 __attribute__((ext_vector_type(4)));
+struct TnPlRegs { tn_u32x4 p0, p1, p2; };
+__device__ __forceinline__ void tn_load_pl(TnPlRegs& t, const __bf16* p, long pstride) {
+    t.p0 = *reinterpret_cast<const tn_u32x4*>(p);
+    t.p1 = *reinterpret_cast<const tn_u32x4*>(p + pstride);
+    t.p2 = *reinterpret_cast<const tn_u32x4*>(p + 2 * pstride);
+}
+__device__ __forceinline__ void tn_store_pl(const TnPlRegs& t, __bf16* img) {
+    __bf16* d = img + (int)(threadIdx.x >> 4) * TN_PITCH + 8 * (threadIdx.x & 15);
+    *reinterpret_cast<tn_u32x4*>(d) = t.p0;
+    *reinterpret_cast<tn_u32x4*>(d + TN_PLANE) = t.p1;
+    *reinterpret_cast<tn_u32x4*>(d + 2 * TN_PLANE) = t.p2;
+}
+__device__ __forceinline__ void tn_csum_pl(const TnPlRegs& t, float (&cs)[8]) {
+    const unsigned w0[4] = {t.p0.x, t.p0.y, t.p0.z, t.p0.w}, w1[4] = {t.p1.x, t.p1.y, t.p1.z, t.p1.w}, w2[4] = {t.p2.x, t.p2.y, t.p2.z, t.p2.w};
+#pragma unroll
+    for (int i = 0; i < 4; ++i) {
+        cs[2 * i] += (__uint_as_float(w1[i] << 16) + __uint_as_float(w2[i] << 16)) + __uint_as_float(w0[i] << 16);
+        cs[2 * i + 1] += (__uint_as_float(w1[i] & 0xffff0000u) + __uint_as_float(w2[i] & 0xffff0000u)) + __uint_as_float(w0[i] & 0xffff0000u);
+    }
+}
+
+struct TnOp { const float* f; const __bf16* pl; long ld; long ps; };
+template <bool PL> struct TnStage { TnRegs r; };
+template <> struct TnStage<true> { TnPlRegs r; };
+
+template <int TERMS> struct TnLds {
+    static constexpr int OP_ELEMS = oe_npl<TERMS>::N * TN_PLANE;
+    static constexpr int BUF_ELEMS = 2 * OP_ELEMS;
+    static constexpr int XCH_BYTES = 4 * 2 * 32 * 64 * 4;
+    static constexpr int IMG_ELEMS = (2 * BUF_ELEMS * 2 >= XCH_BYTES) ? 2 * BUF_ELEMS : XCH_BYTES / 2;
+};
+
+template <int TERMS, bool APL, bool BPL>
+__device__ __forceinline__ void tn_block(const TnOp& Ao, const TnOp& Bo, float* __restrict__ C, long ldc, int M, int N, int Mr, int Nr,
+                                         int K, int k_chunk, int tile_x, int tile_y, int tile_z, const EpiParams& ep, __bf16* img, float* csum_s) {
+    static_assert(!(APL || BPL) || TERMS == 6, "planes operands are the three pieces of precision 6");
+    constexpr int OP_ELEMS = TnLds<TERMS>::OP_ELEMS, BUF_ELEMS = TnLds<TERMS>::BUF_ELEMS;
+    constexpr int NCS = APL ? 8 : 4;
 
     const int lane = threadIdx.x & 63;
     const int wave = __builtin_amdgcn_readfirstlane(threadIdx.x >> 6);
@@ -98,11 +126,37 @@
     const int k_end = min(K, k_begin + k_chunk);
     const int nchunks = (k_end - k_begin + TN_KROWS - 1) / TN_KROWS;
 
-    const int c4 = 4 * (threadIdx.x & 31);
-    const float* a_src = Ap + min(m0 + c4, (long)Mr - 4);
-    const float* b_src = Bp + min(n0 + c4, (long)Nr - 4);
+    const int c4 = 4 * (threadIdx.x & 31), c8 = 8 * (threadIdx.x & 15);
+    const float* a_src = APL ? nullptr : Ao.f + min(m0 + c4, (long)Mr - 4);
+    const float* b_src = BPL ? nullptr : Bo.f + min(n0 + c4, (long)Nr - 4);
+    const long lda = Ao.ld, ldb = Bo.ld;
+    const __bf16* a_pl = APL ? Ao.pl + min(m0 + c8, (long)M - 8) + (long)(k_begin + (int)(threadIdx.x >> 4)) * lda : nullptr;
+    const __bf16* b_pl = BPL ? Bo.pl + min(n0 + c8, (long)N - 8) + (long)(k_begin + (int)(threadIdx.x >> 4)) * ldb : nullptr;
     const bool do_csum = ep.a_colsum != nullptr && tile_x == 0;
-    float cs[4] = {0.f, 0.f, 0.f, 0.f};
+    float cs[NCS];
+#pragma unroll
+    for (int e = 0; e < NCS; ++e) cs[e] = 0.f;
+    auto load_a = [&](TnStage<APL>& t, int k0) {
+        if constexpr (APL) { tn_load_pl(t.r, a_pl, Ao.ps); a_pl += TN_KROWS * lda; } else tn_load(t.r, a_src, lda, k0, k_end - 1);
+    };
+    auto load_b = [&](TnStage<BPL>& t, int k0) {
+        if constexpr (BPL) { tn_load_pl(t.r, b_pl, Bo.ps); b_pl += TN_KROWS * ldb; } else tn_load(t.r, b_src, ldb, k0, k_end - 1);
+    };
+    auto store_a = [&](const TnStage<APL>& t, __bf16* dst, int k0) {
+        if constexpr (APL) tn_store_pl(t.r, dst); else tn_store<TERMS>(t.r, dst, k0, k_end);
+    };
+    auto store_b = [&](const TnStage<BPL>& t, __bf16* dst, int k0) {
+        if constexpr (BPL) tn_store_pl(t.r, dst); else tn_store<TERMS>(t.r, dst, k0, k_end);
+    };
+    auto csum_a = [&](const TnStage<APL>& t, int k0) {
+        if constexpr (APL) {
+            tn_csum_pl(t.r, cs);
+        } else {
+#pragma unroll
+            for (int i = 0; i < 2; ++i)
+                if (k0 + (int)(threadIdx.x >> 5) + 16 * i < k_end) { cs[0] += t.r.v[i].x; cs[1] += t.r.v[i].y; cs[2] += t.r.v[i].z; cs[3] += t.r.v[i].w; }
+        }
+    };
 
     f32x16 acc[2][2];
 #pragma unroll
@@ -117,17 +171,14 @@
     TN_NOW(tn_t);
     tn_t0 = tn_t;
 #endif
-    TnRegs ra, rb;
+    TnStage<APL> ra;
+    TnStage<BPL> rb;
     if (nchunks > 0) {
-        tn_load(ra, a_src, lda, k_begin, k_end - 1);
-        tn_load(rb, b_src, ldb, k_begin, k_end - 1);
-        if (do_csum) {
-#pragma unroll
-            for (int i = 0; i < 2; ++i)
-                if (k_begin + (int)(threadIdx.x >> 5) + 16 * i < k_end) { cs[0] += ra.v[i].x; cs[1] += ra.v[i].y; cs[2] += ra.v[i].z; cs[3] += ra.v[i].w; }
-        }
-        tn_store<TERMS>(ra, img, k_begin, k_end);
-        tn_store<TERMS>(rb, img + OP_ELEMS, k_begin, k_end);
+        load_a(ra, k_begin);
+        load_b(rb, k_begin);
+        if (do_csum) csum_a(ra, k_begin);
+        store_a(ra, img, k_begin);
+        store_b(rb, img + OP_ELEMS, k_begin);
     }
     __syncthreads();
     TN_ACC(0);
@@ -135,8 +186,8 @@
         const int kn = k_begin + (c + 1) * TN_KROWS;
         const bool more = c + 1 < nchunks;
         if (more) {
-            tn_load(ra, a_src, lda, kn, k_end - 1);
-            tn_load(rb, b_src, ldb, kn, k_end - 1);
+            load_a(ra, kn);
+            load_b(rb, kn);
         }
         TN_ACC(1);
         const __bf16* ia = img + (c & 1) * BUF_ELEMS;
@@ -156,14 +207,10 @@
         TN_ACC(3);
 #endif
         if (more) {
-            if (do_csum) {
-#pragma unroll
-                for (int i = 0; i < 2; ++i)
-                    if (kn + (int)(threadIdx.x >> 5) + 16 * i < k_end) { cs[0] += ra.v[i].x; cs[1] += ra.v[i].y; cs[2] += ra.v[i].z; cs[3] += ra.v[i].w; }
-            }
+            if (do_csum) csum_a(ra, kn);
             __bf16* nx = img + ((c + 1) & 1) * BUF_ELEMS;
-            tn_store<TERMS>(ra, nx, kn, k_end);
-            tn_store<TERMS>(rb, nx + OP_ELEMS, kn, k_end);
+            store_a(ra, nx, kn);
+            store_b(rb, nx + OP_ELEMS, kn);
         }
         TN_ACC(4);
         __syncthreads();
@@ -176,10 +223,19 @@
     if (do_csum) {
         if (threadIdx.x < TN_COLS) csum_s[threadIdx.x] = 0.f;
         __syncthreads();
-#pragma unroll
-        for (int e = 0; e < 4; ++e) {
-            const float v = cs[e] + __shfl_xor(cs[e], 32, 64);
-            if (lane < 32) atomicAdd(&csum_s[4 * lane + e], v);
+        if constexpr (APL) {
+#pragma unroll
+            for (int e = 0; e < 8; ++e) {
+                float v = cs[e] + __shfl_xor(cs[e], 32, 64);
+                v += __shfl_xor(v, 16, 64);
+                if (lane < 16) atomicAdd(&csum_s[8 * lane + e], v);
+            }
+        } else {
+#pragma unroll
+            for (int e = 0; e < 4; ++e) {
+                const float v = cs[e] + __shfl_xor(cs[e], 32, 64);
+                if (lane < 32) atomicAdd(&csum_s[4 * lane + e], v);
+            }
         }
         __syncthreads();
         if (threadIdx.x < TN_COLS && m0 + threadIdx.x < M) atomicAdd(ep.a_colsum + m0 + threadIdx.x, csum_s[threadIdx.x] * alpha);
@@ -234,16 +290,19 @@
     return (xcd < r ? xcd * (q + 1) : r * (q + 1) + (xcd - r) * q) + j;
 }
 
-template <int TERMS>
-__global__ __launch_bounds__(TN_THREADS) void gemm_tn_planes_kernel(const float* __restrict__ Ap, long lda, const float* __restrict__ Bp, long ldb,
-                                                                   float* __restrict__ C, long ldc, int M, int N, int Mr, int Nr, int K, int k_chunk,
-                                                                   int gx, int gy, EpiParams ep) {
+template <int TERMS, bool APL = false, bool BPL = false>
+__global__ __launch_bounds__(TN_THREADS) void gemm_tn_planes_kernel(TnOp A, TnOp B, float* __restrict__ C, long ldc, int M, int N, int Mr, int Nr, int K,
+                                                                   int k_chunk, int gx, int gy, EpiParams ep) {
+    __shared__ __attribute__((aligned(16))) __bf16 img[TnLds<TERMS>::IMG_ELEMS];
+    __shared__ float csum_s[TN_COLS];
     const int swz = tn_swizzle(blockIdx.x, gridDim.x);
-    tn_block<TERMS>(Ap, lda, Bp, ldb, C, ldc, M, N, Mr, Nr, K, k_chunk, swz % gx, (swz / gx) % gy, swz / (gx * gy), ep);
-}
-
-template <int TERMS>
+    tn_block<TERMS, APL, BPL>(A, B, C, ldc, M, N, Mr, Nr, K, k_chunk, swz % gx, (swz / gx) % gy, swz / (gx * gy), ep, img, csum_s);
+}
+
+template <int TERMS, bool PL = false>
 __global__ __launch_bounds__(TN_THREADS) void gemm_tn_grouped_kernel(const oe_tn_problem* __restrict__ tab, int n_problems) {
+    __shared__ __attribute__((aligned(16))) __bf16 img[TnLds<TERMS>::IMG_ELEMS];
+    __shared__ float csum_s[TN_COLS];
     const int swz = tn_swizzle(blockIdx.x, gridDim.x);
     int p = 0;
     while (p + 1 < n_problems && tab[p + 1].block_start <= swz) ++p;
@@ -251,8 +310,19 @@
     const int local = swz - pr.block_start;
     EpiParams ep{};
     ep.alpha = pr.alpha; ep.alpha_dev = pr.alpha_dev; ep.beta = 1.f; ep.atomic = 1; ep.a_colsum = pr.a_colsum;
-    tn_block<TERMS>(pr.a, pr.lda, pr.b, pr.ldb, pr.c, pr.ldc, pr.m, pr.n, (pr.m + 3) / 4 * 4, (pr.n + 3) / 4 * 4, pr.k, pr.k_chunk,
-                    local % pr.gx, (local / pr.gx) % pr.gy, local / (pr.gx * pr.gy), ep);
+    const int Mr = (pr.m + 3) / 4 * 4, Nr = (pr.n + 3) / 4 * 4;
+    const int tx = local % pr.gx, ty = (local / pr.gx) % pr.gy, tz = local / (pr.gx * pr.gy);
+    if constexpr (PL) {
+        const TnOp A{pr.a_planes ? nullptr : pr.a, (const __bf16*)pr.a_planes, pr.lda, pr.a_plane_stride};
+        const TnOp B{pr.b_planes ? nullptr : pr.b, (const __bf16*)pr.b_planes, pr.ldb, pr.b_plane_stride};
+        if (pr.a_planes && pr.b_planes) tn_block<TERMS, true, true>(A, B, pr.c, pr.ldc, pr.m, pr.n, Mr, Nr, pr.k, pr.k_chunk, tx, ty, tz, ep, img, csum_s);
+        else if (pr.a_planes) tn_block<TERMS, true, false>(A, B, pr.c, pr.ldc, pr.m, pr.n, Mr, Nr, pr.k, pr.k_chunk, tx, ty, tz, ep, img, csum_s);
+        else if (pr.b_planes) tn_block<TERMS, false, true>(A, B, pr.c, pr.ldc, pr.m, pr.n, Mr, Nr, pr.k, pr.k_chunk, tx, ty, tz, ep, img, csum_s);
+        else tn_block<TERMS, false, false>(A, B, pr.c, pr.ldc, pr.m, pr.n, Mr, Nr, pr.k, pr.k_chunk, tx, ty, tz, ep, img, csum_s);
+    } else {
+        const TnOp A{pr.a, nullptr, pr.lda, 0}, B{pr.b, nullptr, pr.ldb, 0};
+        tn_block<TERMS, false, false>(A, B, pr.c, pr.ldc, pr.m, pr.n, Mr, Nr, pr.k, pr.k_chunk, tx, ty, tz, ep, img, csum_s);
+    }
 }
 
 extern "C" int oe_gemm_tn_grouped_plan(oe_tn_problem* problems, int n, int target_blocks) {
@@ -260,10 +330,14 @@
     long tiles = 0;
     for (int i = 0; i < n; ++i) {
         oe_tn_problem& p = problems[i];
-        OE_REQUIRE(p.a && p.b && p.c && p.m >= 4 && p.n >= 4 && p.k >= 1, "oe_gemm_tn_grouped_plan: problem %d: bad shape / null pointer", i);
-        OE_REQUIRE((((uintptr_t)p.a | (uintptr_t)p.b) & 15) == 0 && p.lda % 4 == 0 && p.ldb % 4 == 0 && p.lda >= (p.m + 3) / 4 * 4 &&
-                       p.ldb >= (p.n + 3) / 4 * 4 && p.ldc >= p.n,
-                   "oe_gemm_tn_grouped_plan: problem %d: operands not 16-byte aligned / leading dimensions too short", i);
+        OE_REQUIRE((p.a || p.a_planes) && (p.b || p.b_planes) && p.c && p.m >= 4 && p.n >= 4 && p.k >= 1,
+                   "oe_gemm_tn_grouped_plan: problem %d: bad shape / null pointer", i);
+        const bool a_ok = p.a_planes ? ((((uintptr_t)p.a_planes) & 15) == 0 && p.m % 8 == 0 && p.lda % 8 == 0 && p.lda >= p.m && p.a_plane_stride % 8 == 0)
+                                     : ((((uintptr_t)p.a) & 15) == 0 && p.lda % 4 == 0 && p.lda >= (p.m + 3) / 4 * 4);
+        const bool b_ok = p.b_planes ? ((((uintptr_t)p.b_planes) & 15) == 0 && p.n % 8 == 0 && p.ldb % 8 == 0 && p.ldb >= p.n && p.b_plane_stride % 8 == 0)
+                                     : ((((uintptr_t)p.b) & 15) == 0 && p.ldb % 4 == 0 && p.ldb >= (p.n + 3) / 4 * 4);
+        OE_REQUIRE(a_ok && b_ok && p.ldc >= p.n,
+                   "oe_gemm_tn_grouped_plan: problem %d: operands not 16-byte aligned / leading dimensions too short (planes: whole 8-element groups)", i);
         p.gx = oe_cdiv(p.n, TN_COLS);
         p.gy = oe_cdiv(p.m, TN_COLS);
         tiles += (long)p.gx * p.gy;
@@ -294,12 +368,31 @@
     return 0;
 }
 
+extern "C" int oe_gemm_tn_grouped_planes(const oe_tn_problem* problems_dev, int n, int total_blocks, void* stream) {
+    OE_REQUIRE(problems_dev && n > 0 && total_blocks > 0, "oe_gemm_tn_grouped_planes: bad arguments");
+    hipLaunchKernelGGL((gemm_tn_grouped_kernel<6, true>), dim3(total_blocks), dim3(TN_THREADS), 0, (hipStream_t)stream, problems_dev, n);
+    OE_LAUNCH_CHECK("oe_gemm_tn_grouped_planes");
+    return 0;
+}
+
 int oe_gemm_tn_planes_try(const OperandDesc& A, const OperandDesc& B, float* C, long ldc, int M, int N, int K, int sk, const EpiParams& ep,
-                          int terms, hipStream_t st) {
-    static const int mode = getenv("OE_GEMM_TN_PLANES") ? atoi(getenv("OE_GEMM_TN_PLANES")) : 1;
+                          int terms, hipStream_t st, const void* apl, long a_ps, const void* bpl, long b_ps) {
+    static const int mode_env = getenv("OE_GEMM_TN_PLANES") ? atoi(getenv("OE_GEMM_TN_PLANES")) : 1;
+    const bool pl = apl || bpl;
+    const int mode = pl ? 2 : mode_env;
     if (!mode) return 1;
+    if (pl) {
+        OE_REQUIRE(terms == 6, "oe_gemm (planes operand of a weight gradient): precision 6 only");
+        OE_REQUIRE((apl || A.vec_ok) && (bpl || B.vec_ok) && K >= 1 &&
+                       (!apl || (M % 8 == 0 && M >= 8 && A.ld % 8 == 0 && A.ld >= M && a_ps % 8 == 0 && ((uintptr_t)apl & 15) == 0)) &&
+                       (!bpl || (N % 8 == 0 && N >= 8 && B.ld % 8 == 0 && B.ld >= N && b_ps % 8 == 0 && ((uintptr_t)bpl & 15) == 0)) &&
+                       (apl || (A.ld >= (M + 3) / 4 * 4 && M >= 4)) && (bpl || (B.ld >= (N + 3) / 4 * 4 && N >= 4)),
+                   "oe_gemm (planes operand of a weight gradient): 16-byte aligned operands, row lengths and strides of whole 8-element groups");
+        OE_REQUIRE(!(ep.bias || ep.act || ep.preact_out || ep.actgrad_in || ep.residual || ep.rowmask || ep.drop_p > 0.f || ep.beta != 1.f || ep.scatter) &&
+                       !(sk > 1 && !ep.atomic), "oe_gemm (planes operand of a weight gradient): alpha / column-sum epilogues only");
+    }
     const int Mr = (M + 3) / 4 * 4, Nr = (N + 3) / 4 * 4;
-    if (!A.vec_ok || !B.vec_ok || A.ld < Mr || B.ld < Nr || M < 4 || N < 4 || K < 1) return 1;
+    if (!pl && (!A.vec_ok || !B.vec_ok || A.ld < Mr || B.ld < Nr || M < 4 || N < 4 || K < 1)) return 1;
     if (ep.bias || ep.act || ep.preact_out || ep.actgrad_in || ep.residual || ep.rowmask || ep.drop_p > 0.f || ep.beta != 1.f || ep.scatter) return 1;
     if (sk > 1 && !ep.atomic) return 1;
     const int gx = oe_cdiv(N, TN_COLS), gy = oe_cdiv(M, TN_COLS);
@@ -312,12 +405,14 @@
     }
     int kc = oe_cdiv(oe_cdiv(K, nz), TN_KROWS) * TN_KROWS;
     nz = oe_cdiv(K, kc);
-    if (terms == 6)
-        hipLaunchKernelGGL((gemm_tn_planes_kernel<6>), dim3(gx * gy * nz), dim3(TN_THREADS), 0, st, A.p, A.ld, B.p, B.ld, C, ldc, M, N, Mr, Nr, K, kc, gx, gy, ep);
-    else if (terms == 3)
-        hipLaunchKernelGGL((gemm_tn_planes_kernel<3>), dim3(gx * gy * nz), dim3(TN_THREADS), 0, st, A.p, A.ld, B.p, B.ld, C, ldc, M, N, Mr, Nr, K, kc, gx, gy, ep);
-    else
-        hipLaunchKernelGGL((gemm_tn_planes_kernel<1>), dim3(gx * gy * nz), dim3(TN_THREADS), 0, st, A.p, A.ld, B.p, B.ld, C, ldc, M, N, Mr, Nr, K, kc, gx, gy, ep);
+    const TnOp Ao{apl ? nullptr : A.p, (const __bf16*)apl, A.ld, a_ps}, Bo{bpl ? nullptr : B.p, (const __bf16*)bpl, B.ld, b_ps};
+    const dim3 grid(gx * gy * nz), block(TN_THREADS);
+    if (apl && bpl) hipLaunchKernelGGL((gemm_tn_planes_kernel<6, true, true>), grid, block, 0, st, Ao, Bo, C, ldc, M, N, Mr, Nr, K, kc, gx, gy, ep);
+    else if (apl) hipLaunchKernelGGL((gemm_tn_planes_kernel<6, true, false>), grid, block, 0, st, Ao, Bo, C, ldc, M, N, Mr, Nr, K, kc, gx, gy, ep);
+    else if (bpl) hipLaunchKernelGGL((gemm_tn_planes_kernel<6, false, true>), grid, block, 0, st, Ao, Bo, C, ldc, M, N, Mr, Nr, K, kc, gx, gy, ep);
+    else if (terms == 6) hipLaunchKernelGGL((gemm_tn_planes_kernel<6>), grid, block, 0, st, Ao, Bo, C, ldc, M, N, Mr, Nr, K, kc, gx, gy, ep);
+    else if (terms == 3) hipLaunchKernelGGL((gemm_tn_planes_kernel<3>), grid, block, 0, st, Ao, Bo, C, ldc, M, N, Mr, Nr, K, kc, gx, gy, ep);
+    else hipLaunchKernelGGL((gemm_tn_planes_kernel<1>), grid, block, 0, st, Ao, Bo, C, ldc, M, N, Mr, Nr, K, kc, gx, gy, ep);
     OE_LAUNCH_CHECK("oe_gemm (bf16 mfma, k-major planes)");
     return 0;
 }
diff --git a/openeat_amd/hip.py b/openeat_amd/hip.py
--- a/openeat_amd/hip.py
+++ b/openeat_amd/hip.py
@@ -107,6 +107,7 @@
         ("drop_in", C.c_float), ("seed_in", C.c_ulonglong), ("drop_out", C.c_float), ("seed_out", C.c_ulonglong),
         ("seed_dev", c_fp),
         ("pre_out", c_fp), ("act_out", c_fp),
+        ("act_planes", c_fp), ("act_plane_stride", C.c_long),
         ("residual", c_fp), ("ldr", C.c_long), ("beta", C.c_float),
         ("y", c_fp), ("ldy", C.c_long),
         ("ln", LnPrologue), ("lnf", LnfPrologue),
@@ -151,7 +152,8 @@
     _fields_ = [("a", C.c_void_p), ("b", C.c_void_p), ("c", C.c_void_p), ("a_colsum", C.c_void_p), ("alpha_dev", C.c_void_p),
                 ("lda", C.c_long), ("ldb", C.c_long), ("ldc", C.c_long), ("m", C.c_int), ("n", C.c_int), ("k", C.c_int),
                 ("alpha", C.c_float), ("k_chunk", C.c_int), ("gx", C.c_int), ("gy", C.c_int), ("nz", C.c_int),
-                ("block_start", C.c_int), ("reserved", C.c_int)]
+                ("block_start", C.c_int), ("reserved", C.c_int),
+                ("a_planes", C.c_void_p), ("a_plane_stride", C.c_long), ("b_planes", C.c_void_p), ("b_plane_stride", C.c_long)]
 
 
 I, L, F, P, U64, SZ = C.c_int, C.c_long, C.c_float, c_fp, C.c_ulonglong, C.c_size_t
@@ -168,8 +170,10 @@
     "oe_gemm_pl_hybrid": (I, [I]),
     "oe_gemm_tn_grouped_plan": (I, [C.POINTER(TnProblem), I, I]),
     "oe_gemm_tn_grouped": (I, [P, I, I, I, P]),
+    "oe_gemm_tn_grouped_planes": (I, [P, I, I, P]),
     "oe_ffn_packed_bytes": (SZ, [I, I, I]),
     "oe_ffn_supported": (I, [I, I, I, I]),
+    "oe_ffn_planes_out_supported": (I, [I, I, I]),
     "oe_ffn_pack_weights": (I, [P, P, I, I, I, P, P, P]),
     "oe_ffn_pack_weights_bwd": (I, [P, P, I, I, I, P, P, P]),
     "oe_ffn_pack_weights_table": (I, [P, I, I, I, I, P]),
@@ -317,7 +321,16 @@
     g.a_colsum = None if (a_colsum is None or g.precision == 0) else a_colsum.data_ptr()
     g.conv_kh = conv_kh
     g.conv_korder = conv_korder
-    if g.precision == 6:
+    if g.precision == 6 and a_kmajor and b_kmajor and any(getattr(q, "pad32", False) for q in (a_planes, b_planes)):
+        for q in (a_planes, b_planes):
+            if q is not None and not q.pad32:
+                raise ValueError("gemm: a weight gradient takes planes of the 32-row padded kind (planes.alloc32) on both sides, or fp32")
+        if a_planes is not None:
+            g.a_planes, g.a_plane_stride = a_planes.ptr, a_planes.stride
+        if b_planes is not None:
+            g.b_planes, g.b_plane_stride = b_planes.ptr, b_planes.stride
+        g.planes_k_padded = 2
+    elif g.precision == 6:
         if a_planes is not None and b_planes is not None:
             g.a_planes, g.a_plane_stride = a_planes.ptr, a_planes.stride
             g.b_planes, g.b_plane_stride = b_planes.ptr, b_planes.stride
@@ -349,16 +362,32 @@
     for i, q in enumerate(problems):
         dy, x, out = q["dy"], q["x"], q["out"]
         p = arr[i]
-        p.a, p.b, p.c, p.a_colsum, p.alpha_dev = dy.data_ptr(), x.data_ptr(), out.data_ptr(), dp(q.get("bias_out")), dp(q.get("alpha_dev"))
-        p.lda, p.ldb, p.ldc = dy.stride(0), x.stride(0), out.stride(0)
-        p.m, p.n, p.k, p.alpha = dy.shape[1], x.shape[1], dy.shape[0], float(q.get("alpha", 1.0))
+        p.a, p.b, p.c, p.a_colsum, p.alpha_dev = dp(dy), dp(x), out.data_ptr(), dp(q.get("bias_out")), dp(q.get("alpha_dev"))
+        ap, bp = q.get("dy_planes"), q.get("x_planes")
+        if ap is not None:
+            p.a_planes, p.a_plane_stride = ap.ptr, ap.stride
+        if bp is not None:
+            p.b_planes, p.b_plane_stride = bp.ptr, bp.stride
+        p.lda, p.ldb, p.ldc = (ap.ld if ap is not None else dy.stride(0)), (bp.ld if bp is not None else x.stride(0)), out.stride(0)
+        p.m, p.n = (ap.cols if ap is not None else dy.shape[1]), (bp.cols if bp is not None else x.shape[1])
+        p.k, p.alpha = (ap.rows if ap is not None else bp.rows if dy is None else dy.shape[0]), float(q.get("alpha", 1.0))
     total = lib().oe_gemm_tn_grouped_plan(arr, n, int(target_blocks))
     if total < 0:
         return None
     return bytes(arr), total
 
 
-def tn_grouped_launch(table_dev: torch.Tensor, n: int, total_blocks: int, precision=None, flops: float = 0.0):
+def tn_grouped_launch(table_dev: torch.Tensor, n: int, total_blocks: int, precision=None, flops: float = 0.0, planes: bool = False):
+    if planes:
+        e0 = e1 = None
+        if PROFILE is not None:
+            e0, e1 = torch.cuda.Event(enable_timing=True), torch.cuda.Event(enable_timing=True)
+            e0.record()
+        check(lib().oe_gemm_tn_grouped_planes(C.c_void_p(table_dev.data_ptr()), n, total_blocks, stream()), "oe_gemm_tn_grouped_planes")
+        if PROFILE is not None:
+            e1.record()
+            PROFILE.append((e0, e1, flops, ("tn_grouped", n, total_blocks, 0, 1, 1, 0)))
+        return
     if PROFILE is not None:
         e0, e1 = torch.cuda.Event(enable_timing=True), torch.cuda.Event(enable_timing=True)
         e0.record()
@@ -372,7 +401,7 @@
 
 
 def ffn_fwd(x2, w1p, b1, w2p, b2, rows, d, ff, act, *, drop_in=0.0, seed_in=0, drop_out=0.0, seed_out=0, seed_dev=None, pre_out=None,
-            act_out=None, residual=None, ldr=0, beta=1.0, y=None, precision=None, lnf=None):
+            act_out=None, residual=None, ldr=0, beta=1.0, y=None, precision=None, lnf=None, act_planes=None):
     a = FfnArgs()
     dp = lambda t: None if t is None else t.data_ptr()
     a.x, a.ldx = x2.data_ptr(), x2.stride(0)
@@ -383,6 +412,8 @@
     a.precision = GEMM_PRECISION if precision is None else precision
     a.drop_in, a.seed_in, a.drop_out, a.seed_out, a.seed_dev = drop_in, seed_in, drop_out, seed_out, dp(seed_dev)
     a.pre_out, a.act_out, a.residual, a.ldr, a.beta = dp(pre_out), dp(act_out), dp(residual), ldr, beta
+    if act_planes is not None:
+        a.act_planes, a.act_plane_stride = act_planes.ptr, act_planes.stride
     a.y, a.ldy = y.data_ptr(), y.stride(0)
     if PROFILE is not None:
         e0, e1 = torch.cuda.Event(enable_timing=True), torch.cuda.Event(enable_timing=True)
@@ -394,7 +425,8 @@
     check(lib().oe_ffn_fwd(C.byref(a), stream()), "oe_ffn_fwd")
 
 
-def ffn_bwd(dy2, w2tp, w1tp, rows, d, ff, act, *, drop_in=0.0, seed_in=0, seed_dev=None, pre=None, dh=None, dx=None, precision=None, ln=None):
+def ffn_bwd(dy2, w2tp, w1tp, rows, d, ff, act, *, drop_in=0.0, seed_in=0, seed_dev=None, pre=None, dh=None, dx=None, precision=None, ln=None,
+            dh_planes=None):
     a = FfnArgs()
     dp = lambda t: None if t is None else t.data_ptr()
     a.x, a.ldx = dy2.data_ptr(), dy2.stride(0)
@@ -404,7 +436,9 @@
     a.rows, a.d, a.ff, a.act = rows, d, ff, act
     a.precision = GEMM_PRECISION if precision is None else precision
     a.drop_in, a.seed_in, a.drop_out, a.seed_out, a.seed_dev = drop_in, seed_in, 0.0, 0, dp(seed_dev)
-    a.pre_out, a.act_out, a.residual, a.ldr, a.beta = pre.data_ptr(), dh.data_ptr(), None, 0, 1.0
+    a.pre_out, a.act_out, a.residual, a.ldr, a.beta = pre.data_ptr(), dp(dh), None, 0, 1.0
+    if dh_planes is not None:
+        a.act_planes, a.act_plane_stride = dh_planes.ptr, dh_planes.stride
     a.y, a.ldy = dx.data_ptr(), dx.stride(0)
     if PROFILE is not None:
         e0, e1 = torch.cuda.Event(enable_timing=True), torch.cuda.Event(enable_timing=True)
diff --git a/openeat_amd/ops.py b/openeat_amd/ops.py
--- a/openeat_amd/ops.py
+++ b/openeat_amd/ops.py
@@ -544,6 +544,18 @@
 _TN_TABLES = []
 
 
+def _tn_table(host: bytes, device) -> torch.Tensor:
+    table = torch.empty(len(host), dtype=torch.uint8, device=device)
+    if LN_TABLE is not None and not LN_TABLE.eager:
+        LN_TABLE.uploads.append((table, host))
+    else:
+        pinned = torch.frombuffer(bytearray(host), dtype=torch.uint8).pin_memory()
+        table.copy_(pinned, non_blocking=True)
+        _TN_TABLES.append((table, pinned))
+        del _TN_TABLES[:-64]
+    return table
+
+
 def _group_wgrads(descs):
     if hip.GEMM_PRECISION == 0:
         return set()
@@ -565,14 +577,7 @@
     if plan is None:
         return set()
     host, total = plan
-    table = torch.empty(len(host), dtype=torch.uint8, device=descs[idx[0]]["dy"].device)
-    if LN_TABLE is not None and not LN_TABLE.eager:
-        LN_TABLE.uploads.append((table, host))
-    else:
-        pinned = torch.frombuffer(bytearray(host), dtype=torch.uint8).pin_memory()
-        table.copy_(pinned, non_blocking=True)
-        _TN_TABLES.append((table, pinned))
-        del _TN_TABLES[:-64]
+    table = _tn_table(host, descs[idx[0]]["dy"].device)
     hip.tn_grouped_launch(table, len(idx), total,
                           flops=sum(2.0 * descs[i]["dy"].shape[0] * descs[i]["dy"].shape[1] * descs[i]["x"].shape[1] for i in idx))
     return set(idx)
@@ -652,6 +657,66 @@
                lambda: gemm_tn(dy, x, out=ow, alpha=alpha, alpha_dev=alpha_dev, bias_out=ob, planes=pl),
                desc=dict(dy=dy, x=x, out=ow, alpha=alpha, alpha_dev=alpha_dev, bias_out=ob))
     return (None if tw is not None else ow.view(w.shape)), (None if tb is not None else ob)
+
+
+def wgrad_bias_planes(w, b, dy, x, dy_pl=None, x_pl=None):
+    rows = dy_pl.rows if dy_pl is not None else dy.shape[0]
+    N = dy_pl.cols if dy_pl is not None else dy.shape[1]
+    K = x_pl.cols if x_pl is not None else x.shape[1]
+    like = dy if dy is not None else x if x is not None else dy_pl.t
+    tw, tb = _arena.grad_target(w), (_arena.grad_target(b) if b is not None else None)
+    ow = tw.view(N, K) if tw is not None else torch.zeros(N, K, device=like.device, dtype=torch.float32)
+    ob = None if b is None else (tb if tb is not None else torch.zeros(N, device=like.device, dtype=torch.float32))
+
+    def launch():
+        global FFN_WGRAD_PLANES_LAUNCHES
+        hip.gemm(dy, x, ow, N, K, rows, lda=dy_pl.ld if dy_pl is not None else dy.stride(0), ldb=x_pl.ld if x_pl is not None else x.stride(0),
+                 ldc=ow.stride(0), a_kmajor=True, b_kmajor=True, split_k=_split_k(N, K, rows), atomic_out=True, a_colsum=ob,
+                 a_planes=dy_pl, b_planes=x_pl)
+        FFN_WGRAD_PLANES_LAUNCHES += 1
+
+    _run_wgrad(tw is not None and (b is None or tb is not None), (dy, x) + _pl_tensors((dy_pl, x_pl)), launch)
+    return (None if tw is not None else ow.view(w.shape)), (None if (b is None or tb is not None) else ob)
+
+
+_CU_COUNT = {}
+
+
+def _cu_count(device) -> int:
+    i = torch.device(device).index
+    i = torch.cuda.current_device() if i is None else i
+    if i not in _CU_COUNT:
+        _CU_COUNT[i] = torch.cuda.get_device_properties(i).multi_processor_count
+    return _CU_COUNT[i]
+
+
+def wgrad_bias_planes_pair(first, second):
+    descs, outs, tensors, to_arena = [], [], [], True
+    for w, b, dy, x, dy_pl, x_pl in (first, second):
+        N = dy_pl.cols if dy_pl is not None else dy.shape[1]
+        K = x_pl.cols if x_pl is not None else x.shape[1]
+        like = dy if dy is not None else x if x is not None else dy_pl.t
+        tw, tb = _arena.grad_target(w), (_arena.grad_target(b) if b is not None else None)
+        ow = tw.view(N, K) if tw is not None else torch.zeros(N, K, device=like.device, dtype=torch.float32)
+        ob = None if b is None else (tb if tb is not None else torch.zeros(N, device=like.device, dtype=torch.float32))
+        to_arena = to_arena and tw is not None and (b is None or tb is not None)
+        descs.append(dict(dy=dy, x=x, out=ow, alpha=1.0, alpha_dev=None, bias_out=ob, dy_planes=dy_pl, x_planes=x_pl))
+        outs.append(((None if tw is not None else ow.view(w.shape)), (None if (b is None or tb is not None) else ob)))
+        tensors += [dy, x] + list(_pl_tensors((dy_pl, x_pl)))
+    device = descs[0]["out"].device
+
+    def launch():
+        global FFN_WGRAD_PLANES_LAUNCHES
+        plan = hip.tn_grouped_plan(descs, _cu_count(device))
+        if plan is None:
+            raise RuntimeError("wgrad_bias_planes_pair: " + hip.lib().oe_last_error().decode("utf-8", "replace"))
+        host, total = plan
+        hip.tn_grouped_launch(_tn_table(host, device), len(descs), total, planes=True,
+                              flops=sum(2.0 * q["out"].shape[0] * q["out"].shape[1] * (q["dy_planes"] or q["x_planes"]).rows for q in descs))
+        FFN_WGRAD_PLANES_LAUNCHES += len(descs)
+
+    _run_wgrad(to_arena, tuple(tensors), launch)
+    return outs[0], outs[1]
 
 
 def bgrad(param, dy, alpha=1.0, alpha_dev=None, n=None):
@@ -1197,6 +1262,14 @@
 FFN_PACK_TABLE = os.environ.get("OE_FFN_PACK_TABLE", "1") == "1"
 FFN_FWD_FUSED_LAUNCHES = 0
 FFN_BWD_FUSED_LAUNCHES = 0
+FFN_WGRAD_PLANES = os.environ.get("OE_FFN_WGRAD_PLANES", "1") == "1"
+FFN_WGRAD_PLANES_LAUNCHES = 0
+FFN_WGRAD_PAIR = os.environ.get("OE_FFN_WGRAD_PAIR", "1") == "1"
+
+
+def _ffn_wgrad_planes(d, ff) -> bool:
+    return (FFN_WGRAD_PLANES and hip.GEMM_PRECISION == 6 and _ffn_bwd_fused() and d % 8 == 0 and
+            bool(hip.lib().oe_ffn_planes_out_supported(d, ff, 6)))
 
 
 def _ffn_dead(key, ent):
@@ -1284,23 +1357,26 @@
         if fused_now:
             need = any(ctx.needs_input_grad)
             pre = _new(M, ff, like=x) if need else None
-            a = _new(M, ff, like=x) if need else None
+            a_pl = _planes.alloc32(M, ff, x.device) if (need and _ffn_wgrad_planes(d, ff)) else None
+            a = _new(M, ff, like=x) if (need and a_pl is None) else None
             w1p, w2p = _ffn_packed(w1, w2, d, ff)
             y = _new(M, d, like=x)
             hip.ffn_fwd(x2, w1p, b1, w2p, b2, M, d, ff, act, drop_in=p_in, seed_in=s_in, drop_out=p_out, seed_out=s_out,
                         seed_dev=_seed_dev, pre_out=pre, act_out=a, residual=res2, ldr=0 if res2 is None else res2.stride(0),
-                        beta=out_scale, y=y, lnf=lnf)
+                        beta=out_scale, y=y, lnf=lnf, act_planes=a_pl)
             global FFN_FWD_FUSED_LAUNCHES
             FFN_FWD_FUSED_LAUNCHES += 1
             if lnf is not None:
                 lnf_p.fused()
-            ctx.save_for_backward(x2, w1, w2, pre, a)
+            ctx.save_for_backward(x2, w1, w2, pre, a if a_pl is None else a_pl.t)
             ctx.biases = (b1, b2)
             ctx.cfg = (act, p_in, s_in, out_scale, p_out, s_out, residual is not None, x.shape)
             ctx.fused = True
+            ctx.a_planes = a_pl is not None
             ln_fuse = LN_BWD_FUSE and FUSE_OUT_DROP and _ln_rows_fusable(M, d) and _ffn_bwd_fused() and _ffn6_takes_ln(d, ff)
             return _tag_out_drop(y.view(*x.shape[:-1], w2.shape[0]), out_scale, p_out, s_out, ln_fuse=ln_fuse)
         ctx.fused = False
+        ctx.a_planes = False
         pre = _new(M, ff, like=x)
         if act in GEMM_FUSED_ACTS:
             a = gemm_nt(x2, w1, b1, act=act, preact_out=pre, ld_aux=ff, drop_p=p_in, seed=s_in, seed_dev=_seed_dev, out_planes=True)
@@ -1326,26 +1402,37 @@
         g2 = dy2 if (p_out == 0 and out_scale == 1.0) else _out_drop_grad(dy2, out_scale, p_out, s_out)
         b1, b2 = ctx.biases
         pend = _PENDING_LN.take(g2)
+        a_pl = _planes.view32(a, x2.shape[0]) if ctx.a_planes else None
         if ctx.fused and _ffn_bwd_fused() and g2.stride(0) % 4 == 0:
             M, d, ff = g2.shape[0], w2.shape[0], w1.shape[0]
             w2tp, w1tp = _ffn_packed(w1, w2, d, ff, bwd=True)
-            dh, dx = _new(M, ff, like=g2), _new(M, d, like=g2)
+            dh_pl = _planes.alloc32(M, ff, g2.device) if a_pl is not None else None
+            dh, dx = (_new(M, ff, like=g2) if dh_pl is None else None), _new(M, d, like=g2)
             ln = None
             if pend is not None and not pend.done:
                 if _ffn6_takes_ln(d, ff) and g2.is_contiguous() and g2.data_ptr() == pend.g.data_ptr() and M == pend.rows:
                     ln = pend.prologue()
                 else:
                     pend.resolve()
-            hip.ffn_bwd(g2, w2tp, w1tp, M, d, ff, act, drop_in=p_in, seed_in=s_in, seed_dev=_seed_dev, pre=pre, dh=dh, dx=dx, ln=ln)
+            hip.ffn_bwd(g2, w2tp, w1tp, M, d, ff, act, drop_in=p_in, seed_in=s_in, seed_dev=_seed_dev, pre=pre, dh=dh, dx=dx, ln=ln,
+                        dh_planes=dh_pl)
             global FFN_BWD_FUSED_LAUNCHES
             FFN_BWD_FUSED_LAUNCHES += 1
             if ln is not None:
                 pend.fused()
-            dw2, db2 = wgrad_bias(w2, b2, g2, a)
-            dw1, db1 = wgrad_bias(w1, b1, dh, x2)
+            if a_pl is not None and FFN_WGRAD_PAIR:
+                (dw2, db2), (dw1, db1) = wgrad_bias_planes_pair((w2, b2, g2, None, None, a_pl), (w1, b1, None, x2, dh_pl, None))
+            elif a_pl is not None:
+                dw2, db2 = wgrad_bias_planes(w2, b2, g2, None, x_pl=a_pl)
+                dw1, db1 = wgrad_bias_planes(w1, b1, None, x2, dy_pl=dh_pl)
+            else:
+                dw2, db2 = wgrad_bias(w2, b2, g2, a)
+                dw1, db1 = wgrad_bias(w1, b1, dh, x2)
             return dx.view(in_shape), dw1, db1, dw2, db2, None, None, (dy if has_res else None), None, None
         if pend is not None:
             pend.resolve()
+        if a_pl is not None:
+            a = _planes.join32(a_pl)
         dw2, db2 = wgrad_bias(w2, b2, g2, a)
         if act in GEMM_FUSED_ACTS:
             dh = gemm_nn(g2, w2, act=act, actgrad_in=pre, ld_aux=pre.stride(0), drop_p=p_in, seed=s_in, seed_dev=_seed_dev, out_planes=True)
diff --git a/openeat_amd/planes.py b/openeat_amd/planes.py
--- a/openeat_amd/planes.py
+++ b/openeat_amd/planes.py
@@ -50,11 +50,12 @@
 
 
 class Planes:
-    __slots__ = ("t", "ptr", "stride", "ld", "rows", "cols", "kpad")
-
-    def __init__(self, t: torch.Tensor, ptr: int, stride: int, ld: int, rows: int, cols: int, kpad: bool = False):
+    __slots__ = ("t", "ptr", "stride", "ld", "rows", "cols", "kpad", "pad32")
+
+    def __init__(self, t: torch.Tensor, ptr: int, stride: int, ld: int, rows: int, cols: int, kpad: bool = False, pad32: bool = False):
         self.t, self.ptr, self.stride, self.ld, self.rows, self.cols = t, ptr, stride, ld, rows, cols
         self.kpad = kpad
+        self.pad32 = pad32
 
 
 def alloc(rows: int, cols: int, device) -> Planes:
@@ -63,6 +64,21 @@
     if rp != rows:
         t[:, rows:].zero_()
     return Planes(t, t.data_ptr(), rp * cols, cols, rows, cols, kpad=True)
+
+
+def alloc32(rows: int, cols: int, device) -> Planes:
+    rp = (rows + 31) // 32 * 32
+    t = torch.empty(3, rp, cols, dtype=torch.bfloat16, device=device)
+    return Planes(t, t.data_ptr(), rp * cols, cols, rows, cols, kpad=True, pad32=True)
+
+
+def view32(t: torch.Tensor, rows: int) -> Planes:
+    return Planes(t, t.data_ptr(), t.shape[1] * t.shape[2], t.shape[2], rows, t.shape[2], kpad=True, pad32=True)
+
+
+def join32(pl: Planes) -> torch.Tensor:
+    p = pl.t[:, :pl.rows].float()
+    return (p[1] + p[2]) + p[0]
 
 
 import contextlib
```
